# sedaprotocol/bn254

Measured on AMD Instinct MI355X. Metric: BN254 pairings/sec (batch verify), higher is better.
Workload: dtype u32

## Files before the change

### bn254_amd/_native.py

```python
import ctypes
import os
import subprocess

_PKG = os.path.dirname(os.path.abspath(__file__))
_CSRC = os.path.join(_PKG, "csrc")
LIB_PATH = os.environ.get("BN254_LIB", os.path.join(_PKG, "libbn254hip.so"))
import glob


def translation_units():
    return sorted(glob.glob(os.path.join(_CSRC, "*.hip")))


def _dependencies():
    return translation_units() + sorted(glob.glob(os.path.join(_CSRC, "*.h"))) + sorted(glob.glob(os.path.join(_CSRC, "*.inc"))) + [
        os.path.join(_CSRC, "gen_constants.py"), os.path.join(_CSRC, "gen_step_asm.py"), os.path.join(os.path.dirname(_PKG), "include", "bn254_hip.h")]

HIPCC_COMPILE_FLAGS = ["-O3", "--offload-arch=gfx950", "-std=c++17", "-fPIC", "-mllvm", "-amdgpu-sched-strategy=max-ilp"]
HIPCC_LINK_FLAGS = ["--offload-arch=gfx950", "-shared", "-fPIC", "-Wl,--no-undefined"]
HIPCC_FLAGS = HIPCC_COMPILE_FLAGS + ["-shared", "-Wl,--no-undefined"]
_OBJ = os.path.join(_PKG, "build")


def _stale():
    if not os.path.exists(LIB_PATH):
        return True
    t = os.path.getmtime(LIB_PATH)
    return any(os.path.getmtime(p) > t for p in _dependencies())


def build(force=False, verbose=False, jobs=None):
    const_h = os.path.join(_CSRC, "bn254_constants.h")
    gen = os.path.join(_CSRC, "gen_constants.py")
    if not os.path.exists(const_h) or os.path.getmtime(const_h) < os.path.getmtime(gen):
        subprocess.check_call(["python3", gen], stdout=None if verbose else subprocess.DEVNULL)
    asm_h, asm_gen = os.path.join(_CSRC, "bn254_csqr_asm.h"), os.path.join(_CSRC, "gen_step_asm.py")
    if not os.path.exists(asm_h) or os.path.getmtime(asm_h) < os.path.getmtime(asm_gen):
        subprocess.check_call(["python3", asm_gen, "selftest"], stdout=None if verbose else subprocess.DEVNULL)
        with open(asm_h, "w") as f:
            subprocess.check_call(["python3", asm_gen, "header"], stdout=f)
    mul_h = os.path.join(_CSRC, "bn254_mul_asm.h")
    if not os.path.exists(mul_h) or os.path.getmtime(mul_h) < os.path.getmtime(asm_gen):
        subprocess.check_call(["python3", asm_gen, "selftest_mul"], stdout=None if verbose else subprocess.DEVNULL)
        with open(mul_h, "w") as f:
            subprocess.check_call(["python3", asm_gen, "header_mul"], stdout=f)
    if force or _stale():
        import time
        from concurrent.futures import ThreadPoolExecutor
        hipcc = os.environ.get("HIPCC", "hipcc")
        os.makedirs(_OBJ, exist_ok=True)
        units = translation_units()
        objs = [os.path.join(_OBJ, os.path.basename(u)[:-4] + ".o") for u in units]
        t0 = time.time()

        def compile_one(pair):
            cmd = [hipcc] + HIPCC_COMPILE_FLAGS + ["-c", "-o", pair[1], pair[0]]
            if verbose:
                print(" ".join(cmd), flush=True)
            subprocess.check_call(cmd)
        with ThreadPoolExecutor(jobs or min(8, os.cpu_count() or 1)) as ex:
            list(ex.map(compile_one, zip(units, objs)))
        cmd = [hipcc] + HIPCC_LINK_FLAGS + ["-o", LIB_PATH] + objs
        if verbose:
            print(" ".join(cmd), flush=True)
        subprocess.check_call(cmd)
        if verbose:
            print("libbn254hip.so: %d translation units compiled and linked in %.1f s" % (len(units), time.time() - t0), flush=True)
    return LIB_PATH


_lib = None


def load():
    global _lib
    if _lib is not None:
        return _lib
    if not os.path.exists(LIB_PATH):
        raise RuntimeError("libbn254hip.so is not built (run `python -c 'import __graft_entry__ as g; g.build()'`); "
                           "bn254_amd has no CPU fallback")
    L = ctypes.CDLL(LIB_PATH)
    vp, sz, u32, i32 = ctypes.c_void_p, ctypes.c_size_t, ctypes.c_uint32, ctypes.c_int
    L.bn254_version.restype = ctypes.c_char_p
    L.bn254_ctx_create.argtypes = [i32, ctypes.POINTER(vp)]
    L.bn254_ctx_destroy.argtypes = [vp]
    L.bn254_ctx_destroy.restype = None
    L.bn254_ctx_reserve.argtypes = [vp, sz]
    L.bn254_ctx_reserve_host.argtypes = [vp, sz, sz]
    L.bn254_ctx_synchronize.argtypes = [vp]
    L.bn254_ctx_set_profiling.argtypes = [vp, i32]
    L.bn254_ctx_expect_msgs_len.argtypes = [vp, ctypes.c_uint64]
    L.bn254_ctx_last_kernel_ms.argtypes = [vp, ctypes.POINTER(ctypes.c_float)]
    L.bn254_ctx_set_option.argtypes = [vp, i32, i32]
    L.bn254_debug_route_table.argtypes = [vp, ctypes.POINTER(ctypes.c_uint64), ctypes.POINTER(i32), ctypes.POINTER(i32), i32]
    L.bn254_debug_key_dedup_last.argtypes = [vp, ctypes.POINTER(ctypes.c_uint32)]
    L.bn254_debug_agg_rand_last.argtypes = [vp, ctypes.POINTER(ctypes.c_uint64)]
    L.bn254_debug_agg_rand_sums.argtypes = [vp, ctypes.POINTER(ctypes.c_uint64), sz, sz, vp, vp, vp, vp, vp, vp]
    L.bn254_ctx_last_clocks.argtypes = [vp, ctypes.POINTER(ctypes.c_double)]
    L.bn254_batch_verify.argtypes = [vp, vp, vp, vp, vp, sz, u32, vp]
    L.bn254_batch_verify_device.argtypes = [vp, vp, vp, vp, vp, sz, u32, vp, vp]
    L.bn254_ctx_register_keys.argtypes = [vp, vp, sz, u32, vp]
    L.bn254_batch_verify_keyed.argtypes = [vp, vp, vp, vp, vp, sz, u32, vp]
    L.bn254_batch_verify_keyed_device.argtypes = [vp, vp, vp, vp, vp, sz, u32, vp, vp]
    L.bn254_batch_verify_keyed_bitmap.argtypes = [vp, vp, vp, vp, vp, sz, sz, u32, vp]
    L.bn254_batch_verify_keyed_bitmap_device.argtypes = [vp, vp, vp, vp, vp, sz, sz, u32, vp, vp]
    L.bn254_batch_verify_keyed_randomized.argtypes = [vp, vp, vp, vp, vp, sz, u32, vp, vp]
    L.bn254_batch_verify_keyed_randomized_device.argtypes = [vp, vp, vp, vp, vp, sz, u32, vp, vp, vp]
    L.bn254_batch_verify_compressed.argtypes = [vp, vp, vp, vp, vp, sz, vp]
    L.bn254_batch_verify_compressed_device.argtypes = [vp, vp, vp, vp, vp, sz, vp, vp]
    L.bn254_batch_verify_randomized.argtypes = [vp, vp, vp, vp, vp, sz, u32, vp, vp, vp]
    L.bn254_batch_verify_randomized_device.argtypes = [vp, vp, vp, vp, vp, sz, u32, vp, vp, vp, vp]
    L.bn254_batch_hash_to_g1.argtypes = [vp, vp, vp, sz, vp, vp, vp]
    L.bn254_batch_hash_to_g1_device.argtypes = [vp, vp, vp, sz, vp, vp, vp, vp]
    L.bn254_batch_pairing_check.argtypes = [vp, vp, vp, sz, sz, u32, vp]
    L.bn254_batch_pairing.argtypes = [vp, vp, vp, sz, sz, u32, vp, vp]
    L.bn254_batch_pairing_device.argtypes = [vp, vp, vp, sz, sz, u32, vp, vp, vp]
    L.bn254_batch_check_public_keys.argtypes = [vp, vp, vp, sz, u32, vp]
    L.bn254_batch_g1_add.argtypes = [vp, vp, vp, sz, vp, vp]
    L.bn254_batch_g2_add.argtypes = [vp, vp, vp, sz, vp, vp]
    L.bn254_batch_g1_mul.argtypes = [vp, vp, vp, sz, i32, vp, vp]
    L.bn254_batch_g2_mul.argtypes = [vp, vp, vp, sz, i32, vp, vp]
    L.bn254_batch_g1_mul_device.argtypes = [vp, vp, vp, sz, i32, vp, vp, vp]
    L.bn254_batch_g2_mul_device.argtypes = [vp, vp, vp, sz, i32, vp, vp, vp]
    L.bn254_batch_sign.argtypes = [vp, vp, vp, vp, sz, vp, vp]
    L.bn254_batch_sign_device.argtypes = [vp, vp, vp, vp, sz, vp, vp, vp]
    L.bn254_batch_g1_sum.argtypes = [vp, vp, vp, sz, vp, vp]
    L.bn254_batch_g2_sum.argtypes = [vp, vp, vp, sz, vp, vp]
    L.bn254_batch_aggregate_verify.argtypes = [vp, vp, vp, sz, vp, sz, vp, vp, vp, vp, sz, u32, vp]
    L.bn254_batch_aggregate_verify_device.argtypes = [vp, vp, vp, sz, vp, sz, vp, vp, vp, vp, sz, u32, vp, vp]
    L.bn254_ctx_register_pools.argtypes = [vp, vp, vp, sz, vp, sz, vp, u32, sz]
    L.bn254_ctx_register_pools_device.argtypes = [vp, vp, vp, sz, vp, sz, vp, u32, sz, vp]
    L.bn254_batch_aggregate_verify_registered.argtypes = [vp, vp, vp, vp, sz, vp]
    L.bn254_batch_aggregate_verify_registered_device.argtypes = [vp, vp, vp, vp, sz, vp, vp]
    L.bn254_batch_aggregate_verify_distinct.argtypes = [vp, vp, vp, vp, sz, vp, vp, sz, u32, vp]
    L.bn254_batch_aggregate_verify_distinct_device.argtypes = [vp, vp, vp, vp, sz, vp, vp, sz, u32, vp, vp]
    L.bn254_batch_aggregate_verify_distinct_keyed.argtypes = [vp, vp, vp, vp, sz, vp, vp, sz, u32, vp]
    L.bn254_batch_aggregate_verify_distinct_keyed_device.argtypes = [vp, vp, vp, vp, sz, vp, vp, sz, u32, vp, vp]
    L.bn254_batch_aggregate_verify_distinct_keyed_randomized.argtypes = [vp, vp, vp, vp, sz, vp, vp, sz, u32, vp, vp]
    L.bn254_batch_aggregate_verify_distinct_keyed_randomized_device.argtypes = [vp, vp, vp, vp, sz, vp, vp, sz, u32, vp, vp, vp]
    L.bn254_batch_g1_decompress.argtypes = [vp, vp, sz, vp, vp]
    L.bn254_batch_g2_decompress.argtypes = [vp, vp, sz, vp, vp]
    L.bn254_debug_fp_op.argtypes = [vp, i32, vp, vp, sz, vp, vp]
    L.bn254_debug_fp12_op.argtypes = [vp, i32, vp, vp, sz, vp]
    L.bn254_debug_final_exp_limbs.argtypes = [vp, i32, vp, sz, vp, vp]
    L.bn254_debug_miller_loop.argtypes = [vp, vp, vp, sz, vp]
    L.bn254_debug_hash_candidate.argtypes = [vp, vp, sz, vp, vp]
    L.bn254_probe_issue_rate.argtypes = [vp, i32, i32, ctypes.POINTER(ctypes.c_double), ctypes.POINTER(i32)]
    L.bn254_probe_leaf_floor.argtypes = [vp, sz, i32, ctypes.POINTER(ctypes.c_float)]
    L.bn254_probe_fe_program.argtypes = [vp, sz, vp, sz, ctypes.POINTER(ctypes.c_float)]
    pp = ctypes.POINTER(vp)
    L.bn254_mgpu_create.argtypes = [ctypes.POINTER(i32), i32, ctypes.POINTER(vp)]
    L.bn254_mgpu_destroy.argtypes = [vp]
    L.bn254_mgpu_destroy.restype = None
    L.bn254_mgpu_device_count.argtypes = [vp]
    L.bn254_mgpu_ctx.argtypes = [vp, i32]
    L.bn254_mgpu_ctx.restype = vp
    L.bn254_mgpu_shard_len.argtypes = [vp, sz]
    L.bn254_mgpu_shard_len.restype = sz
    L.bn254_mgpu_gathered_len.argtypes = [vp, sz]
    L.bn254_mgpu_gathered_len.restype = sz
    L.bn254_mgpu_shard_range.argtypes = [vp, sz, i32, ctypes.POINTER(sz), ctypes.POINTER(sz)]
    L.bn254_mgpu_reserve.argtypes = [vp, sz, i32]
    L.bn254_mgpu_synchronize.argtypes = [vp]
    L.bn254_mgpu_set_option.argtypes = [vp, i32, i32]
    L.bn254_mgpu_last_timing.argtypes = [vp, ctypes.POINTER(ctypes.c_float), ctypes.POINTER(ctypes.c_float)]
    L.bn254_mgpu_last_error.argtypes = [vp]
    L.bn254_mgpu_last_error.restype = ctypes.c_char_p
    L.bn254_mgpu_batch_verify.argtypes = [vp, vp, vp, vp, vp, sz, u32, vp]
    L.bn254_mgpu_batch_verify_device.argtypes = [vp, pp, pp, pp, pp, sz, u32, pp, pp]
    L.bn254_mgpu_batch_pairing.argtypes = [vp, vp, vp, sz, sz, u32, vp, vp, ctypes.POINTER(ctypes.c_uint64)]
    L.bn254_mgpu_batch_pairing_device.argtypes = [vp, pp, pp, sz, sz, u32, pp, pp, pp, pp]
    L.bn254_mgpu_batch_hash_to_g1.argtypes = [vp, vp, vp, sz, vp, vp, vp]
    L.bn254_mgpu_batch_verify_compressed.argtypes = [vp, vp, vp, vp, vp, sz, vp]
    L.bn254_mgpu_register_keys.argtypes = [vp, vp, sz, u32, vp]
    L.bn254_mgpu_batch_verify_keyed.argtypes = [vp, vp, vp, vp, vp, sz, u32, vp]
    L.bn254_mgpu_batch_aggregate_verify.argtypes = [vp, vp, vp, sz, vp, sz, vp, vp, vp, vp, sz, u32, vp]
    _lib = L
    return L


EXPORTED_SYMBOLS = [
    "bn254_version", "bn254_ctx_create", "bn254_ctx_destroy", "bn254_ctx_reserve", "bn254_ctx_reserve_host", "bn254_ctx_synchronize",
    "bn254_batch_verify", "bn254_batch_verify_device", "bn254_batch_verify_randomized", "bn254_batch_verify_randomized_device", "bn254_batch_verify_compressed", "bn254_batch_verify_compressed_device", "bn254_batch_hash_to_g1", "bn254_batch_hash_to_g1_device",
    "bn254_batch_pairing_check", "bn254_batch_pairing", "bn254_batch_pairing_device", "bn254_batch_check_public_keys",
    "bn254_batch_g1_add", "bn254_batch_g2_add", "bn254_batch_g1_mul", "bn254_batch_g2_mul", "bn254_batch_g1_mul_device",
    "bn254_batch_g2_mul_device", "bn254_batch_sign", "bn254_batch_sign_device", "bn254_batch_g1_sum", "bn254_batch_g2_sum",
    "bn254_batch_aggregate_verify", "bn254_batch_aggregate_verify_device", "bn254_ctx_register_pools", "bn254_ctx_register_pools_device",
    "bn254_batch_aggregate_verify_registered", "bn254_batch_aggregate_verify_registered_device", "bn254_batch_aggregate_verify_distinct", "bn254_batch_aggregate_verify_distinct_device", "bn254_batch_aggregate_verify_distinct_keyed", "bn254_batch_aggregate_verify_distinct_keyed_device", "bn254_batch_aggregate_verify_distinct_keyed_randomized", "bn254_batch_aggregate_verify_distinct_keyed_randomized_device", "bn254_batch_g1_decompress", "bn254_batch_g2_decompress", "bn254_debug_fp_op", "bn254_debug_fp12_op", "bn254_debug_final_exp_limbs", "bn254_debug_miller_loop", "bn254_debug_hash_candidate", "bn254_debug_route_table", "bn254_debug_key_dedup_last", "bn254_debug_agg_rand_last", "bn254_debug_agg_rand_sums", "bn254_probe_issue_rate", "bn254_probe_leaf_floor", "bn254_probe_fe_program", "bn254_ctx_set_profiling", "bn254_ctx_last_kernel_ms", "bn254_ctx_set_option", "bn254_ctx_last_clocks", "bn254_ctx_expect_msgs_len", "bn254_ctx_register_keys", "bn254_batch_verify_keyed", "bn254_batch_verify_keyed_device", "bn254_batch_verify_keyed_randomized", "bn254_batch_verify_keyed_randomized_device",
    "bn254_batch_verify_keyed_bitmap", "bn254_batch_verify_keyed_bitmap_device",
    "bn254_mgpu_create", "bn254_mgpu_destroy", "bn254_mgpu_device_count", "bn254_mgpu_ctx", "bn254_mgpu_shard_len", "bn254_mgpu_shard_range",
    "bn254_mgpu_gathered_len", "bn254_mgpu_reserve", "bn254_mgpu_synchronize", "bn254_mgpu_set_option", "bn254_mgpu_last_timing",
    "bn254_mgpu_last_error", "bn254_mgpu_batch_verify", "bn254_mgpu_batch_verify_device", "bn254_mgpu_batch_pairing",
    "bn254_mgpu_batch_pairing_device", "bn254_mgpu_batch_hash_to_g1", "bn254_mgpu_batch_verify_compressed", "bn254_mgpu_register_keys",
    "bn254_mgpu_batch_verify_keyed", "bn254_mgpu_batch_aggregate_verify",
]
```

### bn254_amd/csrc/bn254_devhooks.hip

```cpp
#include <hip/hip_runtime.h>

#include <cstdio>
#include <cstdlib>
#include <cstring>
#include <new>

#include "../../include/bn254_hip.h"
#include "bn254_hash.h"
#include "bn254_io.h"
#include "bn254_pairing.h"

using namespace bn254;

#include "bn254_ws.h"
#include "bn254_lane.h"
#include "bn254_host.h"

KERNEL_SMALL void k_debug_fp_op(int op, const uint8_t* a, const uint8_t* b, size_t n, uint8_t* out, uint8_t* status) {
  size_t i = (size_t)blockIdx.x * BN_WAVE + threadIdx.x;
  if (i >= n) return;
  uint32_t any = 0;
  Fp x, y, r;
  bool ok = fp_from_be(x, a + 32 * i, any);
  if (b) ok = fp_from_be(y, b + 32 * i, any) && ok; else y = fp_zero();
  uint8_t st = ok ? ST_OK : ST_NOT_MEMBER;
  switch (op) {
    case 0: r = fp_mul(x, y); break;
    case 1: r = fp_add(x, y); break;
    case 2: r = fp_sub(x, y); break;
    case 3: r = fp_inv(x); break;
    case 4: r = fp_sqr(x); break;
    default: if (!fp_sqrt(r, x) && st == ST_OK) st = ST_NOT_MEMBER; break;
  }
  fp_to_be(out + 32 * i, r);
  status[i] = st;
}
KERNEL_SMALL void k_debug_hash_candidate(const uint8_t* h, size_t n, uint8_t* out, uint8_t* status) {
  size_t i = (size_t)blockIdx.x * BN_WAVE + threadIdx.x;
  if (i >= n) return;
  U256 x;
  const uint32_t* w = (const uint32_t*)(h + 32 * i);
#pragma unroll
  for (int k = 0; k < 8; ++k) x.w[7 - k] = __builtin_bswap32(w[k]);
  bool cand = hash_reduce_candidate(x);
  bool filt = false, ok = false;
  G1Affine p;
  g1_set_generator(p);
  if (cand) {
    Fp xm, rhs;
    hash_curve_rhs(xm, rhs, x);
    filt = u256_is_square_mod_q(fp_to_u256(rhs));
    ok = hash_point_from_candidate(p, x);
  }
  if (!ok) p.inf = true;
  encode_g1(out + 64 * i, p);
  status[i] = (uint8_t)((ok ? 0 : 1) | (filt != ok ? 0x80 : 0));
}
__device__ __forceinline__ void decode_fp12(Fp12& f, const uint8_t* b) {
  uint32_t any = 0;
  Fp2* c[6] = {&f.c0.c0, &f.c0.c1, &f.c0.c2, &f.c1.c0, &f.c1.c1, &f.c1.c2};
  for (int k = 0; k < 6; ++k) { fp_from_be(c[k]->c0, b + 64 * k, any); fp_from_be(c[k]->c1, b + 64 * k + 32, any); }
}
KERNEL void k_debug_fp12_op(int op, const uint8_t* a, const uint8_t* b, size_t n, uint8_t* out) {
  size_t i = (size_t)blockIdx.x * BN_WAVE + threadIdx.x;
  if (i >= n) return;
  Fp12 x, y, r;
  decode_fp12(x, a + 384 * i);
  if (b) decode_fp12(y, b + 384 * i); else fp12_set_one(y);
  switch (op) {
    case 0: fp12_mul(r, x, y); break;
    case 1: fp12_sqr(r, x); break;
    case 2: fp12_inv(r, x); break;
    case 3: fp12_conj(r, x); break;
    case 4: fp12_frob(r, x, 1); break;
    case 5: fp12_frob(r, x, 2); break;
    case 6: fp12_frob(r, x, 3); break;
    case 7: fp12_cyclotomic_sqr(r, x); break;
    default: { Fp12 acc; final_exponentiation(r, x, acc); } break;
  }
  encode_fp12(out + 384 * i, r);
}

KERNEL_SMALL void k_debug_load_f(const int32_t* limbs, size_t n, Ws ws) {
  size_t i = (size_t)blockIdx.x * BN_WAVE + threadIdx.x;
  if (i >= n) return;
  for (int e = 0; e < 12; ++e) {
    Fp x;
#pragma unroll
    for (int k = 0; k < BN_LIMBS; ++k) x.v[k] = limbs[(i * 12 + e) * BN_LIMBS + k];
    ws_store_fp(ws, PL_F0 + e, i, x);
  }
  ws_byte(ws, BY_ST_DECODE, i) = ST_OK;
  ws_byte(ws, BY_ST_HASH, i) = ST_OK;
}
KERNEL_SMALL void k_debug_read_p1(Ws ws, size_t base, size_t n, uint8_t* out) {
  size_t i = (size_t)blockIdx.x * BN_WAVE + threadIdx.x;
  if (i >= n) return;
  G1Affine p;
  ws_load_g1(ws, PL_P1X, BY_P1_INF, base + i, p);
  encode_g1(out + 64 * i, p);
}

#define PROBE_ITERS 4096
#define PROBE_CHAINS 16
template <int OP>
__global__ void __launch_bounds__(256) k_issue_probe(uint32_t* out, uint32_t seed, unsigned long long* clk) {
  unsigned long long clk0 = 0, wall0 = 0;
  if (clk && threadIdx.x == 0) { clk0 = clock64(); wall0 = wall_clock64(); }
  uint32_t a = seed + threadIdx.x * 2654435761u, b = seed ^ (threadIdx.x * 40503u + 977u);
  uint64_t acc[PROBE_CHAINS];
#pragma unroll
  for (int j = 0; j < PROBE_CHAINS; ++j) acc[j] = a + j;
  for (int i = 0; i < PROBE_ITERS; ++i) {
#pragma unroll
    for (int j = 0; j < PROBE_CHAINS; ++j) {
      if (OP == 0) {
        asm volatile("v_mad_u64_u32 %0, vcc, %1, %2, %0" : "+v"(acc[j]) : "v"(a), "v"(b) : "vcc");
      } else if (OP == 1) {
        uint32_t lo = (uint32_t)acc[j];
        asm volatile("v_add_u32 %0, %0, %1" : "+v"(lo) : "v"(a));
        acc[j] = lo;
      } else {
        uint32_t lo = (uint32_t)acc[j];
        asm volatile("v_mul_lo_u32 %0, %0, %1" : "+v"(lo) : "v"(b));
        acc[j] = lo;
      }
    }
  }
  uint64_t sum = 0;
#pragma unroll
  for (int j = 0; j < PROBE_CHAINS; ++j) sum += acc[j];
  out[(size_t)blockIdx.x * 256 + threadIdx.x] = (uint32_t)sum ^ (uint32_t)(sum >> 32);
  if (clk && threadIdx.x == 0 && blockIdx.x < BN_CLK_MAX_WG) {
    unsigned long long* p = clk + ((size_t)2 * BN_CLK_MAX_WG + blockIdx.x) * 2;
    p[0] += clock64() - clk0; p[1] += wall_clock64() - wall0;
  }
}


extern "C" {

int bn254_debug_key_dedup_last(bn254_ctx* c, uint32_t out[5]) {
  if (!c || !out) return BN254_E_BAD_ARGUMENT;
  for (int i = 0; i < 5; ++i) out[i] = 0;
  if (!c->kd_last_run || !c->kd_ctl) return 0;
  HIP_TRY(hipSetDevice(c->device));
  HIP_TRY(hipDeviceSynchronize());
  HIP_TRY(hipMemcpy(out + 1, c->kd_ctl, KD_CTL_WORDS * sizeof(uint32_t), hipMemcpyDeviceToHost));
  out[0] = 1;
  return 0;
}
int bn254_debug_agg_rand_last(bn254_ctx* c, uint64_t out[6]) {
  if (!c || !out) return BN254_E_BAD_ARGUMENT;
  for (int i = 0; i < 6; ++i) out[i] = 0;
  if (!c->aggr_last_ran || !c->aggr_stats) return 0;
  HIP_TRY(hipSetDevice(c->device));
  HIP_TRY(hipDeviceSynchronize());
  uint32_t st[5];
  HIP_TRY(hipMemcpy(st, c->aggr_stats, sizeof st, hipMemcpyDeviceToHost));
  out[0] = 1;
  for (int i = 0; i < 5; ++i) out[i + 1] = st[i];
  return 0;
}
int bn254_debug_agg_rand_sums(bn254_ctx* c, uint64_t dims[2], size_t group_cap, size_t pair_cap, uint32_t* nagg, uint8_t* verdict, uint8_t* s_g,
                              uint64_t* first_pair, uint32_t* pair_key, uint8_t* pair_point) {
  if (!c || !dims) return BN254_E_BAD_ARGUMENT;
  dims[0] = dims[1] = 0;
  if (!c->aggr_last_ran || !c->aggr_buf) return 0;
  HIP_TRY(hipSetDevice(c->device));
  HIP_TRY(hipDeviceSynchronize());
  const size_t ng = c->aggr_last.ng, tbase = c->aggr_last.tbase;
  uint64_t end = 0;
  HIP_TRY(hipMemcpy(&end, c->aggr_last.ghi + (ng - 1), sizeof end, hipMemcpyDeviceToHost));
  const size_t n_tp = (size_t)(end - tbase);
  dims[0] = ng;
  dims[1] = n_tp;
  if (group_cap < ng || pair_cap < n_tp) return 0;
  if (!nagg || !verdict || !s_g || !first_pair || (n_tp && (!pair_key || !pair_point))) return BN254_E_BAD_ARGUMENT;
  HIP_TRY(hipMemcpy(nagg, c->aggr_last.nagg, ng * sizeof(uint32_t), hipMemcpyDeviceToHost));
  HIP_TRY(hipMemcpy(verdict, c->aggr_last.gst, ng, hipMemcpyDeviceToHost));
  HIP_TRY(hipMemcpy(first_pair, c->aggr_last.glo, ng * sizeof(uint64_t), hipMemcpyDeviceToHost));
  for (size_t g = 0; g < ng; ++g) first_pair[g] -= tbase;
  first_pair[ng] = n_tp;
  if (n_tp) HIP_TRY(hipMemcpy(pair_key, c->aggr_last.bkey + tbase, n_tp * sizeof(uint32_t), hipMemcpyDeviceToHost));
  int rc;
  if ((rc = stage_reserve(c, 0, 64 * (ng > n_tp ? ng : n_tp)))) return rc;
  k_debug_read_p1<<<grid_for(ng), BN_WAVE, 0, c->stream>>>(c->ws, c->aggr_last.cbase, ng, c->stage[0]);
  HIP_TRY(hipGetLastError());
  HIP_TRY(hipDeviceSynchronize());
  HIP_TRY(hipMemcpy(s_g, c->stage[0], 64 * ng, hipMemcpyDeviceToHost));
  if (n_tp) {
    k_debug_read_p1<<<grid_for(n_tp), BN_WAVE, 0, c->stream>>>(c->ws, tbase, n_tp, c->stage[0]);
    HIP_TRY(hipGetLastError());
    HIP_TRY(hipDeviceSynchronize());
    HIP_TRY(hipMemcpy(pair_point, c->stage[0], 64 * n_tp, hipMemcpyDeviceToHost));
  }
  return 0;
}
int bn254_debug_route_table(bn254_ctx* c, uint64_t* max_n, int* miller, int* fe, int cap) {
  if (!c || !max_n || !miller || !fe || cap < 5) return BN254_E_BAD_ARGUMENT;
  size_t m[5];
  BnRoute r[5];
  const int rows = bn_route_table(route_limits(c), m, r, 5);
  for (int i = 0; i < rows; ++i) { max_n[i] = m[i] == (size_t)-1 ? UINT64_MAX : (uint64_t)m[i]; miller[i] = r[i].miller; fe[i] = r[i].fe; }
  return rows;
}

int bn254_probe_issue_rate(bn254_ctx* c, int op, int waves_per_simd, double* wave_inst_per_s, int* n_simd) {
  if (!c || !wave_inst_per_s || op < 0 || op > 2 || waves_per_simd < 1 || waves_per_simd > 8) return BN254_E_BAD_ARGUMENT;
  HIP_TRY(hipSetDevice(c->device));
  hipDeviceProp_t prop;
  HIP_TRY(hipGetDeviceProperties(&prop, c->device));
  const int n_cu = prop.multiProcessorCount, blocks = n_cu * waves_per_simd;
  int rc;
  if ((rc = stage_reserve(c, 0, sizeof(uint32_t) * 256 * (size_t)blocks))) return rc;
  uint32_t* out = (uint32_t*)c->stage[0];
  ScopedEvents ev;
  HIP_TRY(ev.create());
  hipEvent_t e0 = ev.e0, e1 = ev.e1;
  float best = 0;
  for (int rep = 0; rep < 3; ++rep) {
    HIP_TRY(hipEventRecord(e0, c->stream));
    if (op == 0) k_issue_probe<0><<<blocks, 256, 0, c->stream>>>(out, 12345u, c->ws.clk);
    else if (op == 1) k_issue_probe<1><<<blocks, 256, 0, c->stream>>>(out, 12345u, c->ws.clk);
    else k_issue_probe<2><<<blocks, 256, 0, c->stream>>>(out, 12345u, c->ws.clk);
    HIP_TRY(hipEventRecord(e1, c->stream));
    HIP_TRY(hipEventSynchronize(e1));
    float ms = 0;
    HIP_TRY(hipEventElapsedTime(&ms, e0, e1));
    if (rep > 0 && (best == 0 || ms < best)) best = ms;
  }
  *wave_inst_per_s = (double)PROBE_ITERS * PROBE_CHAINS * 4.0 * blocks / (best * 1e-3);
  if (n_simd) *n_simd = n_cu * 4;
  return 0;
}

int bn254_probe_leaf_floor(bn254_ctx* c, size_t n, int mode, float* ms) {
  if (!c || !ms || n == 0 || n > c->ws.stride || mode < 0 || mode > 7) return BN254_E_BAD_ARGUMENT;
  HIP_TRY(hipSetDevice(c->device));
  ScopedEvents ev;
  HIP_TRY(ev.create());
  hipEvent_t e0 = ev.e0, e1 = ev.e1;
  float best = 0;
  int rc = 0;
  for (int rep = 0; rep < 4 && rc == 0; ++rep) {
    HIP_TRY(hipEventRecord(e0, c->stream));
    rc = bn254_pair_leaf_floor(n, c->ws, c->stream, mode);
    HIP_TRY(hipEventRecord(e1, c->stream));
    HIP_TRY(hipEventSynchronize(e1));
    float t = 0;
    HIP_TRY(hipEventElapsedTime(&t, e0, e1));
    if (rep > 0 && (best == 0 || t < best)) best = t;
  }
  *ms = best;
  return rc;
}

int bn254_probe_fe_program(bn254_ctx* c, size_t n, const uint8_t* prog, size_t n_steps, float* ms) {
  if (!c || !ms || !prog || n == 0 || n > c->ws.stride || n_steps == 0 || n_steps > 4096) return BN254_E_BAD_ARGUMENT;
  for (size_t k = 0; k < n_steps; ++k) {
    const uint8_t op = prog[2 * k], arg = prog[2 * k + 1];
    if (op == 0 || op > 7) return BN254_E_BAD_ARGUMENT;
    if ((op == 1 || op == 2 || op == 4) && arg >= (BN_FE_EXACT_SLOTS > BN_FE_CHECK_SLOTS ? BN_FE_EXACT_SLOTS : BN_FE_CHECK_SLOTS)) return BN254_E_BAD_ARGUMENT;
    if (op == 6 && (arg < 1 || arg > 3)) return BN254_E_BAD_ARGUMENT;
  }
  HIP_TRY(hipSetDevice(c->device));
  int rc;
  if ((rc = stage_reserve(c, 7, 2 * n_steps + 2))) return rc;
  static const uint8_t fe_end[2] = {0, 0};
  HIP_TRY(hipMemcpy(c->stage[7], prog, 2 * n_steps, hipMemcpyHostToDevice));
  HIP_TRY(hipMemcpy(c->stage[7] + 2 * n_steps, fe_end, 2, hipMemcpyHostToDevice));
  ScopedEvents ev;
  HIP_TRY(ev.create());
  hipEvent_t e0 = ev.e0, e1 = ev.e1;
  float best = 0;
  for (int rep = 0; rep < 4 && rc == 0; ++rep) {
    HIP_TRY(hipEventRecord(e0, c->stream));
    rc = bn254_pair_fe_program(n, c->ws, c->stage[7], c->stream);
    HIP_TRY(hipEventRecord(e1, c->stream));
    HIP_TRY(hipEventSynchronize(e1));
    float t = 0;
    HIP_TRY(hipEventElapsedTime(&t, e0, e1));
    if (rep > 0 && (best == 0 || t < best)) best = t;
  }
  *ms = best;
  return rc;
}

int bn254_debug_fp_op(bn254_ctx* c, int op, const uint8_t* a, const uint8_t* b, size_t n, uint8_t* out, uint8_t* status) {
  if (!c || (n && (!a || !out || !status))) return BN254_E_BAD_ARGUMENT;
  if (n == 0) return 0;
  HIP_TRY(hipSetDevice(c->device));
  HostStaging st(c);
  const uint8_t* d_a = st.in(0, a, n * 32);
  const uint8_t* d_b = b ? st.in(1, b, n * 32) : nullptr;
  uint8_t *d_out = st.out(2, n * 32, out), *d_status = st.out(3, n, status);
  if (!st.ok()) return st.rc;
  k_debug_fp_op<<<grid_for(n), BN_WAVE, 0, c->stream>>>(op, d_a, d_b, n, d_out, d_status);
  HIP_TRY(hipGetLastError());
  return st.finish();
}
int bn254_debug_hash_candidate(bn254_ctx* c, const uint8_t* h, size_t n, uint8_t* out, uint8_t* status) {
  if (!c || (n && (!h || !out || !status))) return BN254_E_BAD_ARGUMENT;
  if (n == 0) return 0;
  HIP_TRY(hipSetDevice(c->device));
  HostStaging st(c);
  const uint8_t* d_h = st.in(0, h, n * 32);
  uint8_t *d_out = st.out(2, n * 64, out), *d_status = st.out(3, n, status);
  if (!st.ok()) return st.rc;
  k_debug_hash_candidate<<<grid_for(n), BN_WAVE, 0, c->stream>>>(d_h, n, d_out, d_status);
  HIP_TRY(hipGetLastError());
  return st.finish();
}
int bn254_debug_final_exp_limbs(bn254_ctx* c, int layout, const int32_t* limbs, size_t n, uint8_t* gt, uint8_t* status) {
  if (!c || layout < 0 || layout > 6 || (n && (!limbs || !status)) || (gt && layout > 1)) return BN254_E_BAD_ARGUMENT;
  if (n == 0) return 0;
  if ((layout == 3 && !c->fits_trio) || ((layout == 4 || layout == 6) && !bn254_nonet_fits_device())) return BN254_E_BAD_ARGUMENT;
  HIP_TRY(hipSetDevice(c->device));
  int rc;
  if ((rc = ws_reserve(c, n))) return rc;
  HostStaging st(c);
  const uint8_t* d_limbs = st.in(0, limbs, n * 12 * BN_LIMBS * sizeof(int32_t));
  uint8_t *d_gt = st.out(1, n * 384, gt), *d_status = st.out(2, n, status);
  if (!st.ok()) return st.rc;
  hipStream_t s = c->stream;
  k_debug_load_f<<<grid_for(n), BN_WAVE, 0, s>>>((const int32_t*)d_limbs, n, c->ws);
  switch (layout) {
    case 0: rc = launch_final_exp_lane(c, s, n, 1, 1, 1, 0, d_gt, d_status, 0, 0, nullptr, nullptr); break;
    case 1: rc = bn254_pair_final_exp_product(n, 1, c->ws, d_gt, d_status, 0, s); break;
    case 2: rc = bn254_pair_final_exp(n, c->ws, 0, d_status, nullptr, nullptr, s); break;
    case 3: rc = bn254_trio_final_exp(n, c->ws, 0, d_status, s); break;
    case 4: rc = bn254_nonet_final_exp(n, c->ws, 0, d_status, s); break;
    case 6: rc = bn254_nonet_final_exp(n, c->ws, 0, d_status, s, 1); break;
    default: rc = launch_final_exp_lane(c, s, n, 1, 1, 1, 0, nullptr, d_status, 0, 0, nullptr, nullptr); break;
  }
  if (rc) return rc;
  HIP_TRY(hipGetLastError());
  return st.finish();
}
int bn254_debug_fp12_op(bn254_ctx* c, int op, const uint8_t* a, const uint8_t* b, size_t n, uint8_t* out) {
  if (!c || (n && (!a || !out))) return BN254_E_BAD_ARGUMENT;
  if (n == 0) return 0;
  HIP_TRY(hipSetDevice(c->device));
  HostStaging st(c);
  const uint8_t* d_a = st.in(0, a, n * 384);
  const uint8_t* d_b = b ? st.in(1, b, n * 384) : nullptr;
  uint8_t* d_out = st.out(2, n * 384, out);
  if (!st.ok()) return st.rc;
  k_debug_fp12_op<<<grid_for(n), BN_WAVE, 0, c->stream>>>(op, d_a, d_b, n, d_out);
  HIP_TRY(hipGetLastError());
  return st.finish();
}


}
```

### bn254_amd/csrc/bn254_hip.hip

```cpp
#include <hip/hip_runtime.h>
#include <thread>

#include <cstdio>
#include <cstdlib>
#include <cstring>
#include <new>

#include "../../include/bn254_hip.h"
#include "bn254_hash.h"
#include "bn254_io.h"
#include "bn254_pairing.h"

using namespace bn254;

#include "bn254_ws.h"
#include "bn254_lane.h"
#include "bn254_host.h"

KERNEL_SMALL void k_decode_g1(const uint8_t* pts, size_t n, uint32_t flags, Ws ws, int px, int inf_plane, int accumulate) {
  size_t i = (size_t)blockIdx.x * BN_WAVE + threadIdx.x;
  if (i >= n) return;
  G1Affine p;
  uint8_t st = decode_g1(p, pts + 64 * i, flags);
  if (st != ST_OK) g1_set_generator(p);
  ws_store_g1(ws, px, inf_plane, i, p);
  uint8_t prev = accumulate ? ws_byte(ws, BY_ST_DECODE, i) : (uint8_t)ST_OK;
  ws_byte(ws, BY_ST_DECODE, i) = prev != ST_OK ? prev : st;
}
KERNEL void k_decode_g2(const uint8_t* pts, size_t n, uint32_t flags, Ws ws, int accumulate) {
  size_t i = (size_t)blockIdx.x * BN_WAVE + threadIdx.x;
  if (i >= n) return;
  G2Affine q;
  uint8_t st = decode_g2(q, pts + 128 * i, flags);
  if (st != ST_OK) g2_set_generator(q);
  if (flags & FLAG_G2_SUBGROUP_CHECK) {
    bool in = g2_in_subgroup(q);
    if (st == ST_OK && !in) { st = ST_INVALID_GROUP_POINT; g2_set_generator(q); }
  }
  ws_store_g2(ws, i, q);
  uint8_t prev = accumulate ? ws_byte(ws, BY_ST_DECODE, i) : (uint8_t)ST_OK;
  ws_byte(ws, BY_ST_DECODE, i) = prev != ST_OK ? prev : st;
}

__device__ __forceinline__ bool msg_span(const uint64_t* off, size_t i, uint64_t msgs_len, uint64_t& lo, uint64_t& len) {
  lo = off[i];
  const uint64_t hi = off[i + 1];
  const bool ok = lo <= hi && hi <= msgs_len;
  len = ok ? hi - lo : 0;
  if (!ok) lo = 0;
  return ok;
}
KERNEL_SMALL void k_hash_init(size_t n, Ws ws) {
  size_t i = (size_t)blockIdx.x * BN_WAVE + threadIdx.x;
  if (i < n) { ws.h_best[i] = HASH_NONE; ws.h_next[i] = 0; }
  if (i <= HASH_MAX_ROUNDS) ws.h_cnt[i] = (i == 0) ? (uint32_t)n : 0u;
}
KERNEL_SMALL void k_hash_round(const uint8_t* msgs, const uint64_t* off, uint64_t msgs_len, Ws ws, int round, uint32_t width, uint32_t max_ctr) {
  const uint32_t n_act = ws.h_cnt[round];
  if (n_act == 0) return;
  const uint32_t* list = round == 0 ? nullptr : ws.h_list + (size_t)(round & 1) * ws.stride;
  const size_t total = (size_t)n_act * width;
  for (size_t w = (size_t)blockIdx.x * BN_WAVE + threadIdx.x; w < total; w += (size_t)gridDim.x * BN_WAVE) {
    uint32_t slot = (uint32_t)(w % n_act), j = (uint32_t)(w / n_act);
    uint32_t i = list ? list[slot] : slot;
    uint32_t ctr = (uint32_t)ws.h_next[i] + j;
    if (ctr >= max_ctr) continue;
    uint64_t lo, len;
    msg_span(off, i, msgs_len, lo, len);
    const uint8_t* msg = msgs + lo;
    HashState hs;
    hash_state_init(hs, msg, len);
    if (hash_try_filter(hs, msg, len, ctr)) atomicMin(&ws.h_best[i], ctr);
  }
}
KERNEL_SMALL void k_hash_resolve(Ws ws, int round, uint32_t width, uint32_t max_ctr) {
  const uint32_t n_act = ws.h_cnt[round];
  if (n_act == 0) return;
  const uint32_t* list = round == 0 ? nullptr : ws.h_list + (size_t)(round & 1) * ws.stride;
  uint32_t* list_out = ws.h_list + (size_t)((round + 1) & 1) * ws.stride;
  const size_t span = (size_t)gridDim.x * BN_WAVE;
  for (size_t base = (size_t)blockIdx.x * BN_WAVE; base < n_act; base += span) {
    const size_t slot = base + threadIdx.x;
    bool survivor = false;
    uint32_t i = 0;
    if (slot < n_act) {
      i = list ? list[slot] : (uint32_t)slot;
      if (ws.h_best[i] == HASH_NONE) {
        const uint32_t next = (uint32_t)ws.h_next[i] + width;
        if (next < max_ctr) { ws.h_next[i] = (uint8_t)next; survivor = true; }
      }
    }
    const uint64_t votes = __ballot(survivor);
    if (votes == 0) continue;
    uint32_t first = 0;
    if (threadIdx.x == 0) first = atomicAdd(&ws.h_cnt[round + 1], (uint32_t)__popcll(votes));
    first = __shfl(first, 0, BN_WAVE);
    if (survivor) list_out[first + (uint32_t)__popcll(votes & ((1ull << threadIdx.x) - 1ull))] = i;
  }
}
#define HASH_RESOLVE_WG 1024
#define HASH_RESOLVE_TILES_MIN ((size_t)1 << 20)
__global__ void __launch_bounds__(HASH_RESOLVE_WG) k_hash_resolve_tiles(Ws ws, int round, uint32_t width, uint32_t max_ctr) {
  const uint32_t n_act = ws.h_cnt[round];
  if (n_act == 0) return;
  const uint32_t* list = round == 0 ? nullptr : ws.h_list + (size_t)(round & 1) * ws.stride;
  uint32_t* list_out = ws.h_list + (size_t)((round + 1) & 1) * ws.stride;
  __shared__ uint32_t wave_cnt[HASH_RESOLVE_WG / BN_WAVE];
  __shared__ uint32_t tile_base;
  const unsigned wave = threadIdx.x / BN_WAVE, lane = threadIdx.x % BN_WAVE;
  const size_t span = (size_t)gridDim.x * HASH_RESOLVE_WG;
  for (size_t base = (size_t)blockIdx.x * HASH_RESOLVE_WG; base < n_act; base += span) {
    const size_t slot = base + threadIdx.x;
    bool survivor = false;
    uint32_t i = 0;
    if (slot < n_act) {
      i = list ? list[slot] : (uint32_t)slot;
      if (ws.h_best[i] == HASH_NONE) {
        const uint32_t next = (uint32_t)ws.h_next[i] + width;
        if (next < max_ctr) { ws.h_next[i] = (uint8_t)next; survivor = true; }
      }
    }
    const uint64_t votes = __ballot(survivor);
    if (lane == 0) wave_cnt[wave] = (uint32_t)__popcll(votes);
    __syncthreads();
    if (threadIdx.x == 0) {
      uint32_t total = 0;
      for (unsigned w = 0; w < HASH_RESOLVE_WG / BN_WAVE; ++w) { const uint32_t c = wave_cnt[w]; wave_cnt[w] = total; total += c; }
      tile_base = total ? atomicAdd(&ws.h_cnt[round + 1], total) : 0u;
    }
    __syncthreads();
    if (survivor) list_out[tile_base + wave_cnt[wave] + (uint32_t)__popcll(votes & ((1ull << lane) - 1ull))] = i;
    __syncthreads();
  }
}
KERNEL_SMALL void k_hash_direct(const uint8_t* msgs, const uint64_t* off, uint64_t msgs_len, size_t n, Ws ws, uint32_t width, uint32_t max_ctr, int px,
                                int inf_plane, uint8_t* tries_out) {
  const size_t w = (size_t)blockIdx.x * BN_WAVE + threadIdx.x;
  const size_t i = w / width;
  const uint32_t ctr = (uint32_t)(w % width);
  bool ok = false;
  G1Affine p;
  g1_set_generator(p);
  bool span_ok = true;
  if (i < n && ctr < max_ctr) {
    uint64_t lo, len;
    span_ok = msg_span(off, i, msgs_len, lo, len);
    const uint8_t* msg = msgs + lo;
    HashState hs;
    hash_state_init(hs, msg, len);
    ok = hash_try(p, hs, msg, len, ctr);
  }
  const uint64_t pass = __ballot(ok);
  if (i >= n) return;
  if (!span_ok) {
    if (ctr == 0) {
      g1_set_generator(p);
      ws_store_g1(ws, px, inf_plane, i, p);
      ws_byte(ws, BY_ST_HASH, i) = (uint8_t)ST_INVALID_LENGTH;
      if (tries_out) tries_out[i] = 0;
      ws.h_best[i] = HASH_DONE;
    }
    return;
  }
  const uint32_t group = (uint32_t)(pass >> (threadIdx.x & ~(width - 1u))) & (uint32_t)((1ull << width) - 1u);
  if (group != 0) {
    if (ctr == (uint32_t)__builtin_ctz(group)) {
      ws_store_g1(ws, px, inf_plane, i, p);
      ws_byte(ws, BY_ST_HASH, i) = (uint8_t)ST_OK;
      if (tries_out) tries_out[i] = (uint8_t)(ctr + 1);
      ws.h_best[i] = HASH_DONE;
    }
  } else if (ctr == 0) {
    ws.h_best[i] = HASH_NONE;
    ws.h_next[i] = (uint8_t)width;
    if (width < max_ctr) {
      const uint32_t pos = atomicAdd(&ws.h_cnt[1], 1u);
      (ws.h_list + ws.stride)[pos] = (uint32_t)i;
    }
  }
}
KERNEL_SMALL void k_hash_finish(const uint8_t* msgs, const uint64_t* off, uint64_t msgs_len, size_t n, Ws ws, uint32_t max_ctr, int px, int inf_plane,
                                uint8_t* tries_out) {
  size_t i = (size_t)blockIdx.x * BN_WAVE + threadIdx.x;
  if (i >= n) return;
  const uint32_t best = ws.h_best[i];
  if (best == HASH_DONE) return;
  uint64_t lo, len;
  const bool span_ok = msg_span(off, i, msgs_len, lo, len);
  const uint8_t* msg = msgs + lo;
  HashState hs;
  hash_state_init(hs, msg, len);
  G1Affine p;
  bool ok = span_ok && best != HASH_NONE && hash_try(p, hs, msg, len, best);
  if (!ok) g1_set_generator(p);
  ws_store_g1(ws, px, inf_plane, i, p);
  ws_byte(ws, BY_ST_HASH, i) = ok ? (uint8_t)ST_OK : !span_ok ? (uint8_t)ST_INVALID_LENGTH : (uint8_t)ST_HASH_TO_POINT;
  if (tries_out) tries_out[i] = ok ? (uint8_t)(best + 1) : !span_ok ? (uint8_t)0 : (uint8_t)max_ctr;
}

KERNEL void k_miller_verify(size_t n, Ws ws, const uint32_t* map, const uint32_t* count) {
  size_t i = (size_t)blockIdx.x * BN_WAVE + threadIdx.x;
  if (i >= n) return;
  if (map) { if (i >= *count) return; i = map[i]; }
  G1Affine sig, h;
  G2Affine pk;
  ws_load_g1(ws, PL_P1X, BY_P1_INF, i, sig);
  ws_load_g1(ws, PL_P2X, BY_P2_INF, i, h);
  ws_load_g2(ws, i, pk);
  __shared__ Fp12Slot lds_f[BN_WAVE];
  Fp12& f = lds_f[threadIdx.x].v;
  miller_loop<true, true>(f, h, pk, sig);
  ws_store_f12(ws, i, f);
}
__device__ __noinline__ void miller_role_a(size_t i, Ws ws) {
  G1Affine h, unused_g1;
  G2Affine pk;
  ws_load_g1(ws, PL_P2X, BY_P2_INF, i, h);
  ws_load_g2(ws, i, pk);
  g1_set_generator(unused_g1);
  Fp12 f;
  miller_loop<true, false>(f, h, pk, unused_g1);
  ws_store_f12(ws, i, f);
}
__device__ __noinline__ void miller_role_b(size_t i, size_t f_stride, Ws ws) {
  G1Affine sig, unused_g1;
  G2Affine unused_g2;
  ws_load_g1(ws, PL_P1X, BY_P1_INF, i, sig);
  g1_set_generator(unused_g1);
  g2_set_generator(unused_g2);
  Fp12 f;
  miller_loop<false, true>(f, unused_g1, unused_g2, sig);
  ws_store_f12(ws, f_stride + i, f);
  ws_byte(ws, BY_ST_DECODE, f_stride + i) = ST_OK;
}
KERNEL void k_miller_verify_split(size_t n, size_t f_stride, unsigned nblk, Ws ws) {
  bool role_b = blockIdx.x >= nblk;
  size_t i = (size_t)(blockIdx.x - (role_b ? nblk : 0u)) * BN_WAVE + threadIdx.x;
  if (i >= n) return;
  if (!role_b) miller_role_a(i, ws); else miller_role_b(i, f_stride, ws);
}
KERNEL void k_miller_var(size_t n, Ws ws) {
  size_t i = (size_t)blockIdx.x * BN_WAVE + threadIdx.x;
  if (i >= n) return;
  G1Affine p;
  G2Affine q;
  ws_load_g1(ws, PL_P1X, BY_P1_INF, i, p);
  ws_load_g2(ws, i, q);
  Fp12 f;
  miller_loop<true, false>(f, p, q, p);
  ws_store_f12(ws, i, f);
}
KERNEL void k_miller_cpk(size_t n, Ws ws) {
  size_t i = (size_t)blockIdx.x * BN_WAVE + threadIdx.x;
  if (i >= n) return;
  G1Affine pk1, g;
  G2Affine pk2;
  ws_load_g1(ws, PL_P1X, BY_P1_INF, i, pk1);
  ws_load_g2(ws, i, pk2);
  g1_set_generator(g);
  Fp12 f;
  miller_loop<true, true>(f, g, pk2, pk1);
  ws_store_f12(ws, i, f);
}

KERNEL void k_final_exp(size_t n, size_t k, size_t item_stride, size_t pair_stride, Ws ws, int use_hash, uint8_t* gt_out, uint8_t* status_out,
                        int raw_only, size_t base, const uint32_t* map, const uint32_t* count) {
  size_t i = (size_t)blockIdx.x * BN_WAVE + threadIdx.x;
  if (i >= n) return;
  if (map) { if (i >= *count) return; i = map[i]; }
  Fp12 f, g;
  ws_load_f12(ws, base + i * item_stride, f);
  uint8_t st = ws_byte(ws, BY_ST_DECODE, base + i * item_stride);
  for (size_t j = 1; j < k; ++j) {
    size_t idx = base + i * item_stride + j * pair_stride;
    ws_load_f12(ws, idx, g);
    fp12_mul(f, f, g);
    uint8_t sj = ws_byte(ws, BY_ST_DECODE, idx);
    if (st == ST_OK) st = sj;
  }
  if (st == ST_OK && use_hash) st = ws_byte(ws, BY_ST_HASH, i);
  __shared__ Fp12Slot lds_acc[BN_WAVE];
  if (!raw_only) {
    if (gt_out) final_exponentiation(f, f, lds_acc[threadIdx.x].v);
    else final_exponentiation_check(f, f, lds_acc[threadIdx.x].v);
  }
  if (gt_out) encode_fp12(gt_out + 384 * i, f);
  if (status_out) status_out[i] = st != ST_OK ? st : (fp12_is_one(f) ? (uint8_t)ST_OK : (uint8_t)ST_VERIFICATION_FAILED);
}


KERNEL_SMALL void k_decompress_g1_ws(const uint8_t* in, size_t n, Ws ws) {
  size_t i = (size_t)blockIdx.x * BN_WAVE + threadIdx.x;
  if (i >= n) return;
  G1Affine p;
  uint8_t st = decompress_g1(p, in + 33 * i);
  if (st != ST_OK) g1_set_generator(p);
  ws_store_g1(ws, PL_P1X, BY_P1_INF, i, p);
  ws_byte(ws, BY_ST_DECODE, i) = st;
}
KERNEL void k_decompress_g2_ws(const uint8_t* in, size_t n, Ws ws) {
  size_t i = (size_t)blockIdx.x * BN_WAVE + threadIdx.x;
  if (i >= n) return;
  G2Affine q;
  uint8_t st = decompress_g2(q, in + 65 * i);
  if (st != ST_OK) g2_set_generator(q);
  bool in_sub = g2_in_subgroup(q);
  if (st == ST_OK && !in_sub) { st = ST_NOT_MEMBER; g2_set_generator(q); }
  ws_store_g2(ws, i, q);
  uint8_t prev = ws_byte(ws, BY_ST_DECODE, i);
  ws_byte(ws, BY_ST_DECODE, i) = prev != ST_OK ? prev : st;
}
KERNEL_SMALL void k_encode_g1(size_t n, Ws ws, int px, int inf_plane, uint8_t* out, uint8_t* status_out) {
  size_t i = (size_t)blockIdx.x * BN_WAVE + threadIdx.x;
  if (i >= n) return;
  G1Affine p;
  ws_load_g1(ws, px, inf_plane, i, p);
  uint8_t st = ws_byte(ws, BY_ST_HASH, i);
  if (st != ST_OK) p.inf = true;
  encode_g1(out + 64 * i, p);
  if (status_out) status_out[i] = st;
}



int ctx_quiesce(bn254_ctx* c) {
  HIP_TRY(hipStreamSynchronize(c->stream));
  HIP_TRY(hipStreamSynchronize(c->copy_stream));
  HIP_TRY(hipStreamSynchronize(c->kd_stream));
  if (c->last_done_armed) {
    c->last_done_armed = false;
    HIP_TRY(hipEventSynchronize(c->last_done));
  }
  return 0;
}
int ws_reserve(bn254_ctx* c, size_t n) {
  if (n <= c->ws.stride) return 0;
  size_t cap = (n + 255) & ~(size_t)255;
  HIP_TRY(hipSetDevice(c->device));
  { int rc_ = ctx_quiesce(c); if (rc_) return rc_; }
  if (c->ws.planes) { HIP_TRY(hipFree(c->ws.planes)); c->ws.planes = nullptr; }
  if (c->ws.bytes) { HIP_TRY(hipFree(c->ws.bytes)); c->ws.bytes = nullptr; }
  if (c->ws.h_best) { HIP_TRY(hipFree(c->ws.h_best)); c->ws.h_best = nullptr; }
  if (c->ws.h_next) { HIP_TRY(hipFree(c->ws.h_next)); c->ws.h_next = nullptr; }
  if (c->ws.h_list) { HIP_TRY(hipFree(c->ws.h_list)); c->ws.h_list = nullptr; }
  c->ws.stride = 0;
  HIP_TRY(hipMalloc((void**)&c->ws.planes, (size_t)N_PLANES * BN_LIMBS * sizeof(int32_t) * cap));
  HIP_TRY(hipMalloc((void**)&c->ws.bytes, (size_t)N_BYTE_PLANES * cap));
  HIP_TRY(hipMalloc((void**)&c->ws.h_best, sizeof(uint32_t) * cap));
  HIP_TRY(hipMalloc((void**)&c->ws.h_next, cap));
  HIP_TRY(hipMalloc((void**)&c->ws.h_list, 2 * sizeof(uint32_t) * cap));
  if (!c->ws.h_cnt) HIP_TRY(hipMalloc((void**)&c->ws.h_cnt, sizeof(uint32_t) * (HASH_MAX_ROUNDS + 1)));
  c->ws.stride = cap;
  return 0;
}
#define WS_BYTES_PER_ITEM ((size_t)N_PLANES * BN_LIMBS * sizeof(int32_t) + N_BYTE_PLANES + sizeof(uint32_t) + 1 + 2 * sizeof(uint32_t))
size_t ws_chunk_for(bn254_ctx* c, size_t n, size_t ws_per_item, bool key_dedup) {
  if (c->max_chunk > 0) return n > (size_t)c->max_chunk ? (size_t)c->max_chunk : 0;
  if (n * ws_per_item <= c->ws.stride && (!key_dedup || (n <= c->kd_items_cap && (size_t)c->kd_max_keys <= c->kd_keys_cap))) return 0;
  const size_t per_item = ws_per_item * WS_BYTES_PER_ITEM + (key_dedup ? KD_BYTES_PER_ITEM : 0);
  const size_t fixed = key_dedup ? (size_t)c->kd_max_keys * KD_BYTES_PER_KEY : 0;
  size_t avail;
  if (c->assume_free_mb > 0) avail = (size_t)c->assume_free_mb << 20;
  else {
    size_t fr = 0, total = 0;
    if (hipSetDevice(c->device) != hipSuccess || hipMemGetInfo(&fr, &total) != hipSuccess) { (void)hipGetLastError(); return 0; }
    avail = fr + c->ws.stride * WS_BYTES_PER_ITEM + c->kd_items_cap * KD_BYTES_PER_ITEM + c->kd_keys_cap * KD_BYTES_PER_KEY;
  }
  const size_t need = ((n + 255) & ~(size_t)255) * per_item + fixed;
  if (need <= avail / 10 * 9) return 0;
  const size_t room = avail / 10 * 8 > fixed ? avail / 10 * 8 - fixed : 0;
  size_t chunk = room / per_item;
  chunk &= ~(size_t)65535;
  if (chunk == 0) chunk = room / per_item & ~(size_t)255;
  if (key_dedup && (chunk == 0 || route_for(c, chunk).miller != BN_ML_LANE_PAIRS)) return ws_chunk_for(c, n, ws_per_item, false);
  return chunk && chunk < n ? chunk : 0;
}
#define KD_NO_ROOM 1
static int kd_reserve(bn254_ctx* c, size_t n, KeyDedup& kd) {
  size_t slots = 1;
  while (slots < 2 * n) slots <<= 1;
  const size_t keys = (size_t)c->kd_max_keys;
  if (n > c->kd_items_cap || keys > c->kd_keys_cap) {
    const size_t items_cap = n > c->kd_items_cap ? ((n + 255) & ~(size_t)255) : c->kd_items_cap;
    const size_t keys_cap = keys > c->kd_keys_cap ? keys : c->kd_keys_cap;
    { int rc_ = ctx_quiesce(c); if (rc_) return rc_; }
    if (c->kd_buf) { HIP_TRY(hipFree(c->kd_buf)); c->kd_buf = nullptr; }
    c->kd_items_cap = c->kd_keys_cap = 0;
    c->kd_ctl = nullptr;
    if (hipMalloc((void**)&c->kd_buf, items_cap * KD_BYTES_PER_ITEM + keys_cap * KD_BYTES_PER_KEY + 256) != hipSuccess) {
      (void)hipGetLastError();
      c->kd_buf = nullptr;
      return KD_NO_ROOM;
    }
    c->kd_items_cap = items_cap;
    c->kd_keys_cap = keys_cap;
  }
  size_t slots_cap = 1;
  while (slots_cap < 2 * c->kd_items_cap) slots_cap <<= 1;
  uint8_t* p = c->kd_buf;
  auto take = [&](size_t bytes) { uint8_t* r = p; p += (bytes + 15) & ~(size_t)15; return r; };
  kd.table = (uint32_t*)take(slots_cap * 4);
  kd.slot_id = (uint32_t*)take(slots_cap * 4);
  kd.slot_of = (uint32_t*)take(c->kd_items_cap * 4);
  kd.key_idx = (uint32_t*)take(c->kd_items_cap * 4);
  kd.lines = (int32_t*)take(c->kd_keys_cap * BN_N_FIXED_LINES * BN_KEY_LINE_WORDS * 4);
  kd.c2 = (int32_t*)take(c->kd_keys_cap * BN_N_FIXED_LINES * 2 * BN_LIMBS * 4);
  kd.rep = (uint32_t*)take(c->kd_keys_cap * 4);
  kd.ctl = (uint32_t*)take(KD_CTL_WORDS * 4);
  c->kd_ctl = kd.ctl;
  kd.st = take(c->kd_keys_cap);
  kd.inf = take(c->kd_keys_cap);
  kd.slot_mask = (uint32_t)(slots - 1);
  kd.hash_mask = c->kd_hash_bits > 0 && c->kd_hash_bits < 32 ? (1u << c->kd_hash_bits) - 1 : 0xFFFFFFFFu;
  kd.max_keys = (uint32_t)keys;
  kd.min_mult = (uint32_t)c->kd_min_mult;
  return 0;
}
int scratch_reserve(bn254_ctx* c, uint8_t** buf, size_t* cap, size_t bytes) {
  if (bytes <= *cap) return 0;
  { int rc_ = ctx_quiesce(c); if (rc_) return rc_; }
  if (*buf) { HIP_TRY(hipFree(*buf)); *buf = nullptr; *cap = 0; }
  const size_t grown = (bytes + 4095) & ~(size_t)4095;
  HIP_TRY(hipMalloc((void**)buf, grown));
  *cap = grown;
  return 0;
}
int stage_reserve(bn254_ctx* c, int slot, size_t bytes) {
  if (bytes <= c->stage_cap[slot]) return 0;
  HIP_TRY(hipSetDevice(c->device));
  return scratch_reserve(c, &c->stage[slot], &c->stage_cap[slot], bytes);
}
uint8_t* HostStaging::out(int slot, size_t bytes, void* host) {
  if (!rc) rc = stage_reserve(c, slot, bytes);
  if (rc) return nullptr;
  if (host) copy_back(host, c->stage[slot], bytes);
  return c->stage[slot];
}
uint8_t* HostStaging::in(int slot, const void* host, size_t bytes) {
  uint8_t* d = out(slot, bytes ? bytes : 1);
  if (d && bytes) check(hipMemcpyAsync(d, host, bytes, hipMemcpyHostToDevice, c->stream));
  return rc ? nullptr : d;
}
void HostStaging::copy_back(void* host, const void* dev, size_t bytes) {
  if (!host || !bytes) return;
  if (n_back == (int)(sizeof back / sizeof back[0])) { check(hipErrorInvalidValue); return; }
  back[n_back++] = {host, dev, bytes};
}
hipError_t HostStaging::drain() {
  finished = true;
  const hipError_t e = hipStreamSynchronize(c->stream);
  const hipError_t e_copy = hipStreamSynchronize(c->copy_stream);
  return e != hipSuccess ? e : e_copy;
}
int HostStaging::finish() {
  for (int i = 0; i < n_back && !rc; ++i) check(hipMemcpyAsync(back[i].host, back[i].dev, back[i].bytes, hipMemcpyDeviceToHost, c->stream));
  const hipError_t e = drain();
  return rc ? rc : -(int)e;
}
int pool_reserve_one(bn254_ctx* c, Pool* p, size_t n_fp, size_t entries) {
  if (entries <= p->stride) return 0;
  HIP_TRY(hipSetDevice(c->device));
  { int rc_ = ctx_quiesce(c); if (rc_) return rc_; }
  if (p->planes) { HIP_TRY(hipFree(p->planes)); p->planes = nullptr; }
  if (p->st) { HIP_TRY(hipFree(p->st)); p->st = nullptr; }
  p->stride = 0;
  const size_t cap = (entries + 255) & ~(size_t)255;
  p->g2 = n_fp == 4 ? 1u : 0u;
  HIP_TRY(hipMalloc((void**)&p->planes, (n_fp / 2) * BN_POOL_HALF_WORDS * sizeof(int32_t) * cap));
  HIP_TRY(hipMalloc((void**)&p->st, cap));
  p->stride = cap;
  return 0;
}
int pool_reserve(bn254_ctx* c, int which, size_t n_fp, size_t entries) {
  Pool& p = c->pool[which];
  if (entries <= p.stride && c->pool_fp[which] == n_fp) return 0;
  HIP_TRY(hipSetDevice(c->device));
  { int rc_ = ctx_quiesce(c); if (rc_) return rc_; }
  if (p.planes) { HIP_TRY(hipFree(p.planes)); p.planes = nullptr; }
  if (p.st) { HIP_TRY(hipFree(p.st)); p.st = nullptr; }
  p.stride = 0;
  size_t cap = (entries + 255) & ~(size_t)255;
  p.g2 = n_fp == 4 ? 1u : 0u;
  HIP_TRY(hipMalloc((void**)&p.planes, (n_fp / 2) * BN_POOL_HALF_WORDS * sizeof(int32_t) * cap));
  HIP_TRY(hipMalloc((void**)&p.st, cap));
  p.stride = cap;
  c->pool_fp[which] = n_fp;
  return 0;
}

int launch_decode_g2(bn254_ctx* c, hipStream_t s, const uint8_t* d_pts, size_t n, uint32_t flags, int accumulate) {
  if (c->pair_lanes && (flags & FLAG_G2_SUBGROUP_CHECK)) {
    if (route_lane_machine_helpers(c, n)) {
      k_decode_g2<<<grid_for(n), BN_WAVE, 0, s>>>(d_pts, n, flags & ~(uint32_t)FLAG_G2_SUBGROUP_CHECK, c->ws, accumulate);
      return bn254_lm_g2_subgroup(n, c->ws, s);
    }
    return bn254_pair_decode_g2(d_pts, n, flags, c->ws, accumulate, s);
  }
  k_decode_g2<<<grid_for(n), BN_WAVE, 0, s>>>(d_pts, n, flags, c->ws, accumulate);
  return 0;
}

int launch_hash_rounds(bn254_ctx* c, hipStream_t s, const uint8_t* d_msgs, const uint64_t* d_off, size_t n, int px, int inf_plane,
                              uint8_t* d_tries, int mark_finish) {
  const uint32_t max_ctr = c->hash_max_tries ? (uint32_t)c->hash_max_tries : 255u;
  const uint64_t msgs_len = c->msgs_len_call;
  k_hash_init<<<grid_for(n > HASH_MAX_ROUNDS + 1 ? n : HASH_MAX_ROUNDS + 1), BN_WAVE, 0, s>>>(n, c->ws);
  if (n <= HASH_DIRECT_MAX_N && c->hash_direct_width > 0) {
    const uint32_t width = (uint32_t)c->hash_direct_width;
    k_hash_direct<<<grid_for(n * width), BN_WAVE, 0, s>>>(d_msgs, d_off, msgs_len, n, c->ws, width, max_ctr, px, inf_plane, d_tries);
    if (max_ctr > width)
      k_hash_round<<<grid_for(64 * (max_ctr - width)), BN_WAVE, 0, s>>>(d_msgs, d_off, msgs_len, c->ws, 1, max_ctr - width, max_ctr);
    if (mark_finish >= 0 && c->profiling) HIP_TRY(hipEventRecord(c->ev[mark_finish], s));
    k_hash_finish<<<grid_for(n), BN_WAVE, 0, s>>>(d_msgs, d_off, msgs_len, n, c->ws, max_ctr, px, inf_plane, d_tries);
    HIP_TRY(hipGetLastError());
    return 0;
  }
  double expect = (double)n;
  uint32_t consumed = 0;
  for (int round = 0; round < HASH_MAX_ROUNDS && consumed < max_ctr; ++round) {
    bool last = round == HASH_MAX_ROUNDS - 1;
    double lanes_per_msg = (double)HASH_TARGET_LANES / (expect < 1.0 ? 1.0 : expect);
    uint32_t width = lanes_per_msg < 2.0 ? 1u : (uint32_t)lanes_per_msg;
    if (width > max_ctr - consumed || last) width = max_ctr - consumed;
    double bound = expect * 1.25 + 256.0;
    if (bound > (double)n) bound = (double)n;
    size_t lanes = (size_t)(bound * width);
    if (lanes > HASH_MAX_GRID_LANES) lanes = HASH_MAX_GRID_LANES;
    k_hash_round<<<grid_for(lanes), BN_WAVE, 0, s>>>(d_msgs, d_off, msgs_len, c->ws, round, width, max_ctr);
    if ((size_t)bound > HASH_RESOLVE_TILES_MIN) {
      size_t tiles = ((size_t)bound + HASH_RESOLVE_WG - 1) / HASH_RESOLVE_WG;
      if (tiles > 16384) tiles = 16384;
      k_hash_resolve_tiles<<<(unsigned)tiles, HASH_RESOLVE_WG, 0, s>>>(c->ws, round, width, max_ctr);
    } else {
      k_hash_resolve<<<grid_for((size_t)bound), BN_WAVE, 0, s>>>(c->ws, round, width, max_ctr);
    }
    consumed += width;
    double pf = 1.0;
    for (uint32_t t = 0; t < width && pf > 1e-12; ++t) pf *= 0.5274;
    expect *= pf;
  }
  if (mark_finish >= 0 && c->profiling) HIP_TRY(hipEventRecord(c->ev[mark_finish], s));
  k_hash_finish<<<grid_for(n), BN_WAVE, 0, s>>>(d_msgs, d_off, msgs_len, n, c->ws, max_ctr, px, inf_plane, d_tries);
  HIP_TRY(hipGetLastError());
  return 0;
}

int launch_decode_g1(bn254_ctx* c, hipStream_t s, const uint8_t* d_pts, size_t n, uint32_t flags, int px, int inf_plane, int accumulate) {
  k_decode_g1<<<grid_for(n), BN_WAVE, 0, s>>>(d_pts, n, flags, c->ws, px, inf_plane, accumulate);
  return 0;
}
int launch_miller_var_lane(bn254_ctx* c, hipStream_t s, size_t n) {
  k_miller_var<<<grid_for(n), BN_WAVE, 0, s>>>(n, c->ws);
  return 0;
}
int launch_miller_verify_lane(bn254_ctx* c, hipStream_t s, size_t n, const uint32_t* map, const uint32_t* count) {
  k_miller_verify<<<grid_for(n), BN_WAVE, 0, s>>>(n, c->ws, map, count);
  return 0;
}
int launch_final_exp_lane(bn254_ctx* c, hipStream_t s, size_t n, size_t k, size_t item_stride, size_t pair_stride, int use_hash, uint8_t* gt_out,
                          uint8_t* status_out, int raw_only, size_t base, const uint32_t* map, const uint32_t* count) {
  k_final_exp<<<grid_for(n), BN_WAVE, 0, s>>>(n, k, item_stride, pair_stride, c->ws, use_hash, gt_out, status_out, raw_only, base, map, count);
  return 0;
}
int launch_encode_g1(bn254_ctx* c, hipStream_t s, size_t n, int px, int inf_plane, uint8_t* out, uint8_t* status_out) {
  k_encode_g1<<<grid_for(n), BN_WAVE, 0, s>>>(n, c->ws, px, inf_plane, out, status_out);
  return 0;
}

extern "C" {

const char* bn254_version(void) { return "bn254-mi355x 0.7 (gfx950; 9x29-bit balanced Montgomery limbs; verify on lane pairs, batches <= 16384 on lane octets with wave roles; bn254_mgpu_*: all the GPUs of a node behind one handle)"; }

int bn254_ctx_create(int hip_device, bn254_ctx** out) {
  if (!out) return BN254_E_BAD_ARGUMENT;
  int count = 0;
  hipError_t e = hipGetDeviceCount(&count);
  if (e != hipSuccess || count <= 0) return BN254_E_NO_DEVICE;
  if (hip_device < 0 || hip_device >= count) return BN254_E_BAD_ARGUMENT;
  HIP_TRY(hipSetDevice(hip_device));
  bn254_ctx* c = new (std::nothrow) bn254_ctx();
  if (!c) return BN254_E_BAD_ARGUMENT;
  memset(c, 0, sizeof *c);
  c->pair_lanes = 1;
  c->rand_min_batch = RAND_MIN_BATCH_DEFAULT;
  c->agg_rand_min_pairs = AGG_RAND_MIN_PAIRS_DEFAULT;
  c->agg_rand_group_pairs = AGG_RAND_GROUP_PAIRS_DEFAULT;
  c->trio_max_batch = TRIO_MAX_BATCH_DEFAULT;
  c->hash_direct_width = HASH_DIRECT_WIDTH_DEFAULT;
  c->trio_wave_roles = TRIO_WAVE_ROLES_DEFAULT;
  c->agg_subset_min_tuples = AGG_SUBSET_MIN_TUPLES_DEFAULT;
  c->agg_sort_by_msg = 1;
  c->agg_wide_min_tuples = AGG_WIDE_MIN_TUPLES_DEFAULT;
  c->pinned_staging = PINNED_STAGING_DEFAULT;
  c->fits_w8 = bn254_quad_fits_device(1); c->fits_quad = bn254_quad_fits_device(0); c->fits_trio = bn254_trio_fits_device();
  if (c->trio_wave_roles == 2 && !c->fits_w8) c->trio_wave_roles = 1;
  if (c->trio_wave_roles == 1 && !c->fits_quad) c->trio_wave_roles = 0;
  if (!c->fits_trio) c->trio_max_batch = 0;
  c->nonet_max_batch = bn254_nonet_fits_device() ? NONET_MAX_BATCH_DEFAULT : 0;
  c->lm_max_batch = bn254_lm_fits_device() ? LM_MAX_BATCH_DEFAULT : 0;
  c->nonet_wide = 1;
  c->g2_fixed_base = 1;
  c->key_dedup = 1;
  c->kd_max_keys = KEY_DEDUP_MAX_KEYS_DEFAULT;
  c->kd_min_mult = KEY_DEDUP_MIN_MULT_DEFAULT;
  c->bm_table_max_keys = BITMAP_TABLE_MAX_KEYS_DEFAULT;
  c->device = hip_device;
  hipError_t err = hipStreamCreateWithFlags(&c->stream, hipStreamNonBlocking);
  if (err == hipSuccess) err = hipStreamCreateWithFlags(&c->copy_stream, hipStreamNonBlocking);
  if (err == hipSuccess) err = hipEventCreateWithFlags(&c->copy_done, hipEventDisableTiming);
  if (err == hipSuccess) err = hipEventCreateWithFlags(&c->last_done, hipEventDisableTiming);
  if (err == hipSuccess) err = hipStreamCreateWithFlags(&c->kd_stream, hipStreamNonBlocking);
  if (err == hipSuccess) err = hipEventCreateWithFlags(&c->kd_fork, hipEventDisableTiming);
  if (err == hipSuccess) err = hipEventCreateWithFlags(&c->kd_join, hipEventDisableTiming);
  for (int i = 0; i < 5 && err == hipSuccess; ++i) err = hipEventCreate(&c->ev[i]);
  if (err != hipSuccess) {
    if (c->kd_join) (void)hipEventDestroy(c->kd_join);
    if (c->kd_fork) (void)hipEventDestroy(c->kd_fork);
    if (c->kd_stream) (void)hipStreamDestroy(c->kd_stream);
    if (c->last_done) (void)hipEventDestroy(c->last_done);
    for (int i = 0; i < 5; ++i) if (c->ev[i]) (void)hipEventDestroy(c->ev[i]);
    if (c->copy_done) (void)hipEventDestroy(c->copy_done);
    if (c->copy_stream) (void)hipStreamDestroy(c->copy_stream);
    if (c->stream) (void)hipStreamDestroy(c->stream);
    delete c;
    return -(int)err;
  }
  *out = c;
  return 0;
}
void bn254_ctx_destroy(bn254_ctx* c) {
  if (!c) return;
  (void)hipSetDevice(c->device);
  (void)ctx_quiesce(c);
  if (c->ws.planes) (void)hipFree(c->ws.planes);
  if (c->ws.bytes) (void)hipFree(c->ws.bytes);
  if (c->ws.h_best) (void)hipFree(c->ws.h_best);
  if (c->ws.h_next) (void)hipFree(c->ws.h_next);
  if (c->ws.h_list) (void)hipFree(c->ws.h_list);
  if (c->ws.h_cnt) (void)hipFree(c->ws.h_cnt);
  if (c->ws.clk) (void)hipFree(c->ws.clk);
  if (c->pin) (void)hipHostFree(c->pin);
  for (int i = 0; i < 8; ++i) { if (c->pool[i].planes) (void)hipFree(c->pool[i].planes); if (c->pool[i].st) (void)hipFree(c->pool[i].st); }
  if (c->g2_comb.planes) (void)hipFree(c->g2_comb.planes);
  if (c->g2_comb.st) (void)hipFree(c->g2_comb.st);
  if (c->g1_comb.planes) (void)hipFree(c->g1_comb.planes);
  if (c->g1_comb.st) (void)hipFree(c->g1_comb.st);
  for (int i = 0; i < 8; ++i) if (c->stage[i]) (void)hipFree(c->stage[i]);
  if (c->key_lines) (void)hipFree(c->key_lines);
  if (c->key_xy) (void)hipFree(c->key_xy);
  if (c->key_st) (void)hipFree(c->key_st);
  if (c->key_inf) (void)hipFree(c->key_inf);
  if (c->aggd_buf) (void)hipFree(c->aggd_buf);
  if (c->aggr_buf) (void)hipFree(c->aggr_buf);
  if (c->aggr_stats) (void)hipFree(c->aggr_stats);
  if (c->kd_buf) (void)hipFree(c->kd_buf);
  if (c->bm_bad) (void)hipFree(c->bm_bad);
  if (c->bm_tab) (void)hipFree(c->bm_tab);
  for (int i = 0; i < 5; ++i) (void)hipEventDestroy(c->ev[i]);
  (void)hipEventDestroy(c->kd_fork);
  (void)hipEventDestroy(c->kd_join);
  (void)hipStreamDestroy(c->kd_stream);
  (void)hipEventDestroy(c->copy_done);
  (void)hipEventDestroy(c->last_done);
  (void)hipStreamSynchronize(c->copy_stream);
  (void)hipStreamDestroy(c->copy_stream);
  (void)hipStreamDestroy(c->stream);
  delete c;
}
int bn254_ctx_reserve(bn254_ctx* c, size_t n) { return c ? ws_reserve(c, n) : BN254_E_BAD_ARGUMENT; }
int bn254_ctx_reserve_host(bn254_ctx* c, size_t n, size_t msg_bytes) {
  if (!c) return BN254_E_BAD_ARGUMENT;
  int rc = ws_reserve(c, n);
  const size_t need[5] = {msg_bytes ? msg_bytes : 1, (n + 1) * sizeof(uint64_t), n * 64, n * 128, n ? n : 1};
  for (int slot = 0; slot < 5 && !rc; ++slot) rc = stage_reserve(c, slot, need[slot]);
  return rc;
}
int bn254_ctx_synchronize(bn254_ctx* c) {
  if (!c) return BN254_E_BAD_ARGUMENT;
  HIP_TRY(hipStreamSynchronize(c->stream));
  return 0;
}
int bn254_ctx_expect_msgs_len(bn254_ctx* c, uint64_t msgs_len) {
  if (!c) return BN254_E_BAD_ARGUMENT;
  c->msgs_len_next = msgs_len;
  c->msgs_len_declared = 1;
  return 0;
}
int bn254_ctx_set_profiling(bn254_ctx* c, int enabled) {
  if (!c) return BN254_E_BAD_ARGUMENT;
  c->profiling = enabled;
  c->ev_valid = 0;
  return 0;
}
int bn254_ctx_set_option(bn254_ctx* c, int option, int value) {
  if (!c) return BN254_E_BAD_ARGUMENT;
  if (option == BN254_OPT_SPLIT_MILLER) { c->split_miller = value; return 0; }
  if (option == BN254_OPT_PAIR_LANES) { c->pair_lanes = value != 0; return 0; }
  if (option == BN254_OPT_RAND_MIN_BATCH) { if (value < 0) return BN254_E_BAD_ARGUMENT; c->rand_min_batch = value; return 0; }
  if (option == BN254_OPT_RAND_ITEMS_PER_LANE) { if (value < 0 || value > 2) return BN254_E_BAD_ARGUMENT; c->rand_items_per_lane = value; return 0; }
  if (option == BN254_OPT_AGG_SUBSET_MIN_TUPLES) { if (value < 0) return BN254_E_BAD_ARGUMENT; c->agg_subset_min_tuples = value; return 0; }
  if (option == BN254_OPT_TRIO_MAX_BATCH) {
    if (value < 0 || (value > 0 && !c->fits_trio)) return BN254_E_BAD_ARGUMENT;
    c->trio_max_batch = value;
    return 0;
  }
  if (option == BN254_OPT_TRIO_WAVE_ROLES) {
    if (value < 0 || value > 2 || (value == 2 && !c->fits_w8) || (value == 1 && !c->fits_quad)) return BN254_E_BAD_ARGUMENT;
    c->trio_wave_roles = value;
    return 0;
  }
  if (option == BN254_OPT_HASH_DIRECT_WIDTH) {
    if (value < 0 || value > 32 || (value & (value - 1))) return BN254_E_BAD_ARGUMENT;
    c->hash_direct_width = value;
    return 0;
  }
  if (option == BN254_OPT_NONET_MAX_BATCH) {
    HIP_TRY(hipSetDevice(c->device));
    if (value < 0 || (value > 0 && !bn254_nonet_fits_device())) return BN254_E_BAD_ARGUMENT;
    c->nonet_max_batch = value;
    return 0;
  }
  if (option == BN254_OPT_NONET_WIDE) { c->nonet_wide = value != 0; return 0; }
  if (option == BN254_OPT_LM_MAX_BATCH) {
    HIP_TRY(hipSetDevice(c->device));
    if (value < 0 || (value > 0 && !bn254_lm_fits_device())) return BN254_E_BAD_ARGUMENT;
    c->lm_max_batch = value;
    return 0;
  }
  if (option == BN254_OPT_PINNED_STAGING) { if (value < 0 || value > 16) return BN254_E_BAD_ARGUMENT; c->pinned_staging = value; return 0; }
  if (option == BN254_OPT_AGG_SORT_BY_MSG) { c->agg_sort_by_msg = value != 0; return 0; }
  if (option == BN254_OPT_AGG_WIDE_MIN_TUPLES) { if (value < 0) return BN254_E_BAD_ARGUMENT; c->agg_wide_min_tuples = value; return 0; }
  if (option == BN254_OPT_CLOCK_PROBE) {
    HIP_TRY(hipSetDevice(c->device));
    HIP_TRY(hipDeviceSynchronize());
    if (value && !c->ws.clk) {
      HIP_TRY(hipMalloc((void**)&c->ws.clk, sizeof(unsigned long long) * 3 * BN_CLK_MAX_WG * 2));
      HIP_TRY(hipMemset(c->ws.clk, 0, sizeof(unsigned long long) * 3 * BN_CLK_MAX_WG * 2));
    } else if (!value && c->ws.clk) {
      HIP_TRY(hipFree(c->ws.clk));
      c->ws.clk = nullptr;
    }
    return 0;
  }
  if (option == BN254_OPT_HASH_MAX_TRIES) { if (value < 0 || value > 255) return BN254_E_BAD_ARGUMENT; c->hash_max_tries = value; return 0; }
  if (option == BN254_OPT_G2_FIXED_BASE) { c->g2_fixed_base = value != 0; return 0; }
  if (option == BN254_OPT_MAX_CHUNK) { if (value < 0) return BN254_E_BAD_ARGUMENT; c->max_chunk = value; return 0; }
  if (option == BN254_OPT_ASSUME_FREE_MB) { if (value < 0) return BN254_E_BAD_ARGUMENT; c->assume_free_mb = value; return 0; }
  if (option == BN254_OPT_KEY_DEDUP) { if (value < 0 || value > 1) return BN254_E_BAD_ARGUMENT; c->key_dedup = value; return 0; }
  if (option == BN254_OPT_KEY_DEDUP_MAX_KEYS) { if (value < 0 || value > KEY_DEDUP_MAX_KEYS_LIMIT) return BN254_E_BAD_ARGUMENT; c->kd_max_keys = value; return 0; }
  if (option == BN254_OPT_KEY_DEDUP_MIN_MULT) { if (value < 1) return BN254_E_BAD_ARGUMENT; c->kd_min_mult = value; return 0; }
  if (option == BN254_OPT_KEY_DEDUP_FORCE_GENERIC) { c->kd_force_generic = value != 0; return 0; }
  if (option == BN254_OPT_KEY_DEDUP_HASH_BITS) { if (value < 0 || value > 32) return BN254_E_BAD_ARGUMENT; c->kd_hash_bits = value; return 0; }
  if (option == BN254_OPT_AGGD_KEYED_ROUTE) { if (value < 0 || value > 3) return BN254_E_BAD_ARGUMENT; c->aggd_keyed_route = value; return 0; }
  if (option == BN254_OPT_AGG_RAND_MIN_PAIRS) { if (value < 0) return BN254_E_BAD_ARGUMENT; c->agg_rand_min_pairs = value; return 0; }
  if (option == BN254_OPT_AGG_RAND_GROUP_PAIRS) { if (value < 1) return BN254_E_BAD_ARGUMENT; c->agg_rand_group_pairs = value; return 0; }
  if (option == BN254_OPT_BITMAP_TABLE_MAX_KEYS) { if (value < 0) return BN254_E_BAD_ARGUMENT; c->bm_table_max_keys = value; return 0; }
  if (option == BN254_OPT_BITMAP_ROUTE) { if (value < 0 || value > 2) return BN254_E_BAD_ARGUMENT; c->bm_route = value; return 0; }
  return BN254_E_BAD_ARGUMENT;
}
int bn254_ctx_last_clocks(bn254_ctx* c, double sclk_mhz[3]) {
  if (!c || !sclk_mhz || !c->ws.clk) return BN254_E_BAD_ARGUMENT;
  HIP_TRY(hipSetDevice(c->device));
  int wall_khz = 0;
  HIP_TRY(hipDeviceGetAttribute(&wall_khz, hipDeviceAttributeWallClockRate, c->device));
  const size_t words = (size_t)3 * BN_CLK_MAX_WG * 2;
  unsigned long long* h = (unsigned long long*)malloc(words * sizeof(unsigned long long));
  if (!h) return BN254_E_NO_MEMORY;
  hipError_t e = hipDeviceSynchronize();
  if (e == hipSuccess) e = hipMemcpy(h, c->ws.clk, words * sizeof(unsigned long long), hipMemcpyDeviceToHost);
  if (e == hipSuccess) e = hipMemset(c->ws.clk, 0, words * sizeof(unsigned long long));
  if (e != hipSuccess) { free(h); return -(int)e; }
  for (int k = 0; k < 3; ++k) {
    double cyc = 0, wall = 0;
    for (size_t w = 0; w < BN_CLK_MAX_WG; ++w) {
      const unsigned long long a = h[((size_t)k * BN_CLK_MAX_WG + w) * 2], b = h[((size_t)k * BN_CLK_MAX_WG + w) * 2 + 1];
      if (b) { cyc += (double)a; wall += (double)b; }
    }
    sclk_mhz[k] = wall > 0 ? cyc / wall * (double)wall_khz * 1e-3 : 0.0;
  }
  free(h);
  return 0;
}
int bn254_ctx_last_kernel_ms(bn254_ctx* c, float ms[4]) {
  if (!c || !ms || !c->ev_valid) return BN254_E_BAD_ARGUMENT;
  HIP_TRY(hipEventSynchronize(c->ev[4]));
  for (int i = 0; i < 4; ++i) HIP_TRY(hipEventElapsedTime(&ms[i], c->ev[i], c->ev[i + 1]));
  if (c->ev_hash_first) { float t = ms[0]; ms[0] = ms[1]; ms[1] = t; }
  return 0;
}


}
int launch_final_exp_layout(bn254_ctx* c, hipStream_t s, size_t n, int use_hash, uint8_t* d_status, int fe) {
  switch (fe) {
    case BN_FE_NONET_WIDE: return bn254_nonet_final_exp(n, c->ws, use_hash, d_status, s, 1);
    case BN_FE_NONET: return bn254_nonet_final_exp(n, c->ws, use_hash, d_status, s, 0);
    case BN_FE_OCTET: return bn254_trio_final_exp(n, c->ws, use_hash, d_status, s);
    default: return bn254_pair_final_exp(n, c->ws, use_hash, d_status, nullptr, nullptr, s);
  }
}
int launch_verify_miller_fe(bn254_ctx* c, hipStream_t s, size_t n, int pairs, int use_hash, uint8_t* d_status, bool mark) {
  if (!c->pair_lanes) {
    const unsigned g = grid_for(n);
    if (pairs == BN_PAIRS_CHECK_PKS) k_miller_cpk<<<g, BN_WAVE, 0, s>>>(n, c->ws);
    else k_miller_verify<<<g, BN_WAVE, 0, s>>>(n, c->ws, nullptr, nullptr);
    if (mark) PROF_MARK(3);
    k_final_exp<<<g, BN_WAVE, 0, s>>>(n, 1, 1, 1, c->ws, use_hash, nullptr, d_status, 0, 0, nullptr, nullptr);
    return 0;
  }
  const BnRoute r = route_for(c, n);
  int rc;
  switch (r.miller) {
    case BN_ML_LANE_MACHINE: rc = bn254_lm_miller_verify(n, c->ws, s, pairs); break;
    case BN_ML_WAVE_ROLES:
      rc = c->trio_wave_roles == 2 ? bn254_w8_miller_verify(n, c->ws, s, pairs)
           : c->trio_wave_roles ? bn254_quad_miller_verify(n, c->ws, s, pairs) : bn254_trio_miller_verify(n, c->ws, s, pairs);
      break;
    default: rc = bn254_pair_miller_verify(n, c->ws, nullptr, nullptr, s, pairs); break;
  }
  if (rc) return rc;
  if (mark) PROF_MARK(3);
  return launch_final_exp_layout(c, s, n, use_hash, d_status, r.fe);
}

extern "C" {
static int verify_tail(bn254_ctx* c, hipStream_t s, size_t n, uint8_t* d_status, bool split, const KeyDedup* kd, int hash_first) {
  int rc;
  if (kd) {
    HIP_TRY(hipStreamWaitEvent(s, c->kd_join, 0));
    const KeyTable kt = {kd->lines, kd->st, kd->inf, kd->max_keys};
    if ((rc = bn254_pair_miller_verify_keyed(n, c->ws, kd->key_idx, kt, s, 0, nullptr, kd->ctl + KD_CTL_KEYED_N))) return rc;
    if ((rc = bn254_pair_miller_verify(n, c->ws, nullptr, kd->ctl + KD_CTL_GENERIC_N, s))) return rc;
    PROF_MARK(3);
    if ((rc = bn254_pair_final_exp(n, c->ws, 1, d_status, nullptr, nullptr, s))) return rc;
  } else if (split) {
    const unsigned g = grid_for(n);
    k_miller_verify_split<<<2 * g, BN_WAVE, 0, s>>>(n, c->ws.stride / 2, g, c->ws);
    PROF_MARK(3);
    k_final_exp<<<g, BN_WAVE, 0, s>>>(n, 2, 1, c->ws.stride / 2, c->ws, 1, nullptr, d_status, 0, 0, nullptr, nullptr);
  } else if ((rc = launch_verify_miller_fe(c, s, n, BN_PAIRS_VERIFY, 1, d_status, true))) return rc;
  PROF_MARK(4);
  if (c->profiling) { c->ev_valid = 1; c->ev_hash_first = hash_first; }
  HIP_TRY(hipGetLastError());
  return 0;
}
static int verify_after_decode(bn254_ctx* c, hipStream_t s, const uint8_t* d_msgs, const uint64_t* d_off, size_t n, uint8_t* d_status, bool split,
                               const KeyDedup* kd = nullptr) {
  PROF_MARK(1);
  if (const int rc = launch_hash_rounds(c, s, d_msgs, d_off, n, PL_P2X, BY_P2_INF, nullptr)) return rc;
  PROF_MARK(2);
  return verify_tail(c, s, n, d_status, split, kd, 0);
}

int bn254_batch_verify_device(bn254_ctx* c, const uint8_t* d_msgs, const uint64_t* d_off, const uint8_t* d_sigs, const uint8_t* d_pks,
                              size_t n, uint32_t flags, uint8_t* d_status, void* stream) {
  MsgsLenScope msgs_len_scope(c);
  if (!c || (n && (!d_msgs || !d_off || !d_sigs || !d_pks || !d_status))) return BN254_E_BAD_ARGUMENT;
  if (n == 0) return 0;
  if (misaligned(d_sigs) || misaligned(d_pks) || ((uintptr_t)d_off & 7u)) return BN254_E_MISALIGNED;
  HIP_TRY(hipSetDevice(c->device));
  bool split = c->split_miller && n <= BN_SPLIT_MAX_N;
  bool key_dedup = c->key_dedup && c->kd_max_keys > 0 && c->pair_lanes && !split && n <= 0xFFFFFFFFu &&
                         route_for(c, n).miller == BN_ML_LANE_PAIRS && route_for(c, n).fe == BN_FE_LANE_PAIRS;
  if (const size_t chunk = ws_chunk_for(c, n, split ? 2 : 1, key_dedup))
    return verify_device_sliced(n, chunk, [&](size_t lo, size_t len) {
      return bn254_batch_verify_device(c, d_msgs, d_off + lo, d_sigs + 64 * lo, d_pks + 128 * lo, len, flags, d_status + lo, stream);
    });
  int rc = ws_reserve(c, split ? 2 * n : n);
  if (rc) return rc;
  KeyDedup kd;
  if (key_dedup) {
    rc = kd_reserve(c, n, kd);
    if (rc == KD_NO_ROOM) key_dedup = false;
    else if (rc) return rc;
    rc = 0;
  }
  c->kd_last_run = key_dedup;
  hipStream_t s = stream ? (hipStream_t)stream : c->stream;
  CallDone call_done(c, s);
  PROF_MARK(0);
  if (key_dedup) {
    HIP_TRY(hipEventRecord(c->kd_fork, s));
    HIP_TRY(hipStreamWaitEvent(c->kd_stream, c->kd_fork, 0));
    if ((rc = bn254_kd_enqueue(d_pks, n, flags, kd, c->kd_force_generic, c->kd_stream))) return rc;
    HIP_TRY(hipEventRecord(c->kd_join, c->kd_stream));
  }
  k_decode_g1<<<grid_for(n), BN_WAVE, 0, s>>>(d_sigs, n, flags, c->ws, PL_P1X, BY_P1_INF, 0);
  if ((rc = launch_decode_g2(c, s, d_pks, n, flags, 1))) return rc;
  return verify_after_decode(c, s, d_msgs, d_off, n, d_status, split, key_dedup ? &kd : nullptr);
}

int bn254_batch_verify_compressed_device(bn254_ctx* c, const uint8_t* d_msgs, const uint64_t* d_off, const uint8_t* d_sigs33,
                                         const uint8_t* d_pks65, size_t n, uint8_t* d_status, void* stream) {
  MsgsLenScope msgs_len_scope(c);
  if (!c || (n && (!d_msgs || !d_off || !d_sigs33 || !d_pks65 || !d_status))) return BN254_E_BAD_ARGUMENT;
  if (n == 0) return 0;
  if ((uintptr_t)d_off & 7u) return BN254_E_MISALIGNED;
  HIP_TRY(hipSetDevice(c->device));
  if (const size_t chunk = ws_chunk_for(c, n))
    return verify_device_sliced(n, chunk, [&](size_t lo, size_t len) {
      return bn254_batch_verify_compressed_device(c, d_msgs, d_off + lo, d_sigs33 + 33 * lo, d_pks65 + 65 * lo, len, d_status + lo, stream);
    });
  int rc = ws_reserve(c, n);
  if (rc) return rc;
  hipStream_t s = stream ? (hipStream_t)stream : c->stream;
  CallDone call_done(c, s);
  PROF_MARK(0);
  k_decompress_g1_ws<<<grid_for(n), BN_WAVE, 0, s>>>(d_sigs33, n, c->ws);
  if (route_lane_machine_helpers(c, n)) {
    if ((rc = bn254_pair_decompress_g2(d_pks65, n, c->ws, s, 1))) return rc;
    if ((rc = bn254_lm_g2_subgroup(n, c->ws, s, ST_NOT_MEMBER))) return rc;
  } else if (c->pair_lanes) { if ((rc = bn254_pair_decompress_g2(d_pks65, n, c->ws, s))) return rc; }
  else k_decompress_g2_ws<<<grid_for(n), BN_WAVE, 0, s>>>(d_pks65, n, c->ws);
  return verify_after_decode(c, s, d_msgs, d_off, n, d_status, false);
}
static int verify_host_sliced(bn254_ctx* c, const uint8_t* msgs, const uint64_t* off, const uint8_t* sigs, const uint8_t* pks, size_t n,
                              uint32_t flags, uint8_t* status, size_t chunk, bool compressed) {
  uint64_t* tmp = (uint64_t*)malloc((chunk + 1) * sizeof(uint64_t));
  if (!tmp) return BN254_E_NO_MEMORY;
  const size_t sig_sz = compressed ? 33 : 64, pk_sz = compressed ? 65 : 128;
  int rc = 0;
  for (size_t lo = 0; lo < n && !rc; lo += chunk) {
    const size_t len = n - lo < chunk ? n - lo : chunk;
    for (size_t i = 0; i <= len; ++i) tmp[i] = off[lo + i] - off[lo];
    const uint8_t* m = msgs ? msgs + off[lo] : nullptr;
    rc = compressed ? bn254_batch_verify_compressed(c, m, tmp, sigs + sig_sz * lo, pks + pk_sz * lo, len, status + lo)
                    : bn254_batch_verify(c, m, tmp, sigs + sig_sz * lo, pks + pk_sz * lo, len, flags, status + lo);
  }
  free(tmp);
  return rc;
}
int bn254_batch_verify_compressed(bn254_ctx* c, const uint8_t* msgs, const uint64_t* off, const uint8_t* sigs33, const uint8_t* pks65, size_t n,
                                  uint8_t* status) {
  MsgsLenScope msgs_len_scope(c);
  if (!c || (n && (!off || !sigs33 || !pks65 || !status))) return BN254_E_BAD_ARGUMENT;
  if (n == 0) return 0;
  HIP_TRY(hipSetDevice(c->device));
  if (!msgs_ok(msgs, off, n)) return BN254_E_BAD_ARGUMENT;
  if (const size_t chunk = ws_chunk_for(c, n)) return verify_host_sliced(c, msgs, off, sigs33, pks65, n, 0, status, chunk, true);
  HostStaging st(c);
  const uint8_t *d_msgs = st.in(0, msgs, (size_t)off[n]), *d_off = st.in(1, off, (n + 1) * sizeof(uint64_t));
  const uint8_t *d_sigs = st.in(2, sigs33, n * 33), *d_pks = st.in(3, pks65, n * 65);
  uint8_t* d_status = st.out(4, n, status);
  if (st.ok()) st.rc = bn254_batch_verify_compressed_device(c, d_msgs, (const uint64_t*)d_off, d_sigs, d_pks, n, d_status, nullptr);
  return st.finish();
}

static int pin_reserve(bn254_ctx* c, size_t bytes) {
  if (bytes <= c->pin_cap) return 0;
  { int rc_ = ctx_quiesce(c); if (rc_) return rc_; }
  if (c->pin) { HIP_TRY(hipHostFree(c->pin)); c->pin = nullptr; c->pin_cap = 0; }
  const size_t cap = (bytes + ((size_t)1 << 20) - 1) & ~(((size_t)1 << 20) - 1);
  HIP_TRY(hipHostMalloc((void**)&c->pin, cap, hipHostMallocDefault));
  c->pin_cap = cap;
  return 0;
}
static int pinned_copy_in(bn254_ctx* c, uint8_t* d_dst, uint8_t* pin, const uint8_t* src, size_t bytes, hipStream_t stream, int threads) {
  if (!bytes) return 0;
  const size_t piece = (size_t)1 << 20;
  if (threads > 16) threads = 16;
  if (threads > 1 && bytes < 4 * piece) threads = 1;
  int rcs[16] = {0};
  auto work = [&](int t, int n_threads) {
    if (t && hipSetDevice(c->device) != hipSuccess) { rcs[t] = -1; return; }
    const size_t share = ((bytes + n_threads - 1) / n_threads + 255) & ~(size_t)255, lo = (size_t)t * share, hi = lo + share < bytes ? lo + share : bytes;
    for (size_t o = lo; o < hi; o += piece) {
      const size_t len = o + piece < hi ? piece : hi - o;
      memcpy(pin + o, src + o, len);
      const hipError_t e = hipMemcpyAsync(d_dst + o, pin + o, len, hipMemcpyHostToDevice, stream);
      if (e != hipSuccess) { rcs[t] = -(int)e; return; }
    }
  };
  std::thread helpers[15];
  int started = 0;
  bool fallback = false;
  try {
    for (int t = 1; t < threads; ++t) { helpers[started] = std::thread(work, t, threads); ++started; }
  } catch (...) {
    fallback = true;
  }
  if (!fallback) work(0, threads);
  for (int t = 0; t < started; ++t) helpers[t].join();
  if (fallback) {
    for (int t = 0; t < 16; ++t) rcs[t] = 0;
    work(0, 1);
  }
  for (int t = 0; t < 16; ++t) if (rcs[t]) return rcs[t];
  return 0;
}
static int verify_host_overlapped(bn254_ctx* c, const uint8_t* msgs, const uint64_t* off, const uint8_t* sigs, const uint8_t* pks, size_t n,
                                  uint32_t flags, uint8_t* status) {
  const size_t msg_bytes = (size_t)off[n];
  int rc;
  if ((rc = ws_reserve(c, n))) return rc;
  HostStaging st(c);
  const size_t need[4] = {msg_bytes ? msg_bytes : 1, (n + 1) * sizeof(uint64_t), n * 64, n * 128};
  for (int slot = 0; slot < 4; ++slot) st.out(slot, need[slot]);
  st.out(4, n, status);
  if (!st.ok()) return st.rc;
  hipStream_t s = c->stream;
  const bool pinned = c->pinned_staging > 0 && n >= PINNED_STAGING_MIN_N;
  auto up = [](size_t x) { return (x + 4095) & ~(size_t)4095; };
  const size_t o_off = up(msg_bytes), o_sig = o_off + up((n + 1) * sizeof(uint64_t)), o_pk = o_sig + up(n * 64), pin_bytes = o_pk + up(n * 128);
  if (pinned && (rc = pin_reserve(c, pin_bytes))) return rc;
  PROF_MARK(0);
  if (pinned) {
    if ((rc = pinned_copy_in(c, c->stage[0], c->pin, msgs, msg_bytes, s, c->pinned_staging))) return rc;
    if ((rc = pinned_copy_in(c, c->stage[1], c->pin + o_off, (const uint8_t*)off, (n + 1) * sizeof(uint64_t), s, 1))) return rc;
  } else {
    if (msg_bytes) HIP_TRY(hipMemcpyAsync(c->stage[0], msgs, msg_bytes, hipMemcpyHostToDevice, s));
    HIP_TRY(hipMemcpyAsync(c->stage[1], off, (n + 1) * sizeof(uint64_t), hipMemcpyHostToDevice, s));
  }
  if ((rc = launch_hash_rounds(c, s, c->stage[0], (const uint64_t*)c->stage[1], n, PL_P2X, BY_P2_INF, nullptr))) return rc;
  if (pinned) {
    if ((rc = pinned_copy_in(c, c->stage[2], c->pin + o_sig, sigs, n * 64, c->copy_stream, c->pinned_staging))) return rc;
    if ((rc = pinned_copy_in(c, c->stage[3], c->pin + o_pk, pks, n * 128, c->copy_stream, c->pinned_staging))) return rc;
  } else {
    HIP_TRY(hipMemcpyAsync(c->stage[2], sigs, n * 64, hipMemcpyHostToDevice, c->copy_stream));
// ... 148 lines not shown
```

### bn254_amd/csrc/bn254_host.h

```cpp
#pragma once
#include <hip/hip_runtime.h>

#include <cstdint>
#include <cstdlib>
#include <cstring>
#include <new>

#include "../../include/bn254_hip.h"

#define BN_HIDDEN __attribute__((visibility("hidden")))

struct AggTables { int valid; size_t n_msgs, n_signers, n_groups, groups4, built_for; int wide2, wide1; };

struct bn254_ctx {
  int device;
  hipStream_t stream;
  Ws ws;
  uint8_t* stage[8];
  size_t stage_cap[8];
  int profiling;
  int split_miller;
  Pool pool[8];
  size_t pool_fp[8];
  int agg_wide_min_tuples;
  int agg_subset_min_tuples;
  int agg_sort_by_msg;
  int pair_lanes;
  int rand_min_batch;
  int rand_items_per_lane;
  int hash_max_tries;
  int trio_wave_roles;
  int hash_direct_width;
  int trio_max_batch;
  int lm_max_batch;
  int nonet_wide;
  int nonet_max_batch;
  hipEvent_t ev[5];
  int ev_valid;
  int ev_hash_first;
  hipStream_t copy_stream;
  uint8_t* pin;
  size_t pin_cap;
  int pinned_staging;
  hipEvent_t copy_done;
  uint64_t msgs_len_next;
  int msgs_len_declared;
  uint64_t msgs_len_call;
  int entry_depth;
  int32_t* key_lines;
  int32_t* key_xy;
  uint8_t* key_st;
  uint8_t* key_inf;
  size_t n_keys, key_cap;
  hipEvent_t last_done;
  bool last_done_armed;
  Pool g2_comb;
  int g2_comb_ready;
  Pool g1_comb;
  int g1_comb_ready;
  int g2_fixed_base;
  AggTables reg_pools;
  int max_chunk;
  int assume_free_mb;
  bool fits_w8, fits_quad, fits_trio;
  uint8_t* aggd_buf;
  size_t aggd_cap;
  int key_dedup;
  int kd_max_keys;
  int kd_min_mult;
  int kd_force_generic;
  int kd_hash_bits;
  hipStream_t kd_stream;
  hipEvent_t kd_fork, kd_join;
  uint8_t* kd_buf;
  size_t kd_items_cap, kd_keys_cap;
  uint32_t* kd_ctl;
  int kd_last_run;
  int aggd_keyed_route;
  int agg_rand_min_pairs;
  int agg_rand_group_pairs;
  uint8_t* aggr_buf;
  size_t aggr_cap;
  uint32_t* aggr_stats;
  int aggr_last_ran;
  struct { size_t ng, cbase, tbase; const uint32_t *nagg, *bkey; const uint64_t *glo, *ghi; const uint8_t* gst; } aggr_last;
  uint8_t* bm_bad;
  size_t bm_bad_cap;
  uint8_t* bm_tab;
  size_t bm_tab_cap;
  bool bm_bad_valid, bm_tab_valid;
  int bm_table_max_keys;
  int bm_route;
};

struct ScopedEvents {
  hipEvent_t e0 = nullptr, e1 = nullptr;
  hipError_t create() {
    hipError_t e = hipEventCreate(&e0);
    return e == hipSuccess ? hipEventCreate(&e1) : e;
  }
  ~ScopedEvents() { if (e0) (void)hipEventDestroy(e0); if (e1) (void)hipEventDestroy(e1); }
  ScopedEvents() = default;
  ScopedEvents(const ScopedEvents&) = delete;
  ScopedEvents& operator=(const ScopedEvents&) = delete;
};
static inline BnRouteLimits route_limits(const bn254_ctx* c) {
  BnRouteLimits L;
  L.small_max = c->pair_lanes && c->trio_max_batch > 0 ? (size_t)c->trio_max_batch : 0;
  L.lm_max = c->lm_max_batch > 0 ? (size_t)c->lm_max_batch : 0;
  L.nonet_max = c->nonet_max_batch > 0 ? (size_t)c->nonet_max_batch : 0;
  L.nonet_wide_max = c->nonet_wide ? (size_t)NONET_WIDE_MAX_BATCH : 0;
  return L;
}
static inline BnRoute route_for(const bn254_ctx* c, size_t n) { return bn_route(route_limits(c), n); }
static inline bool route_lane_machine_helpers(const bn254_ctx* c, size_t n) { return c->pair_lanes && c->lm_max_batch > 0 && n <= (size_t)c->lm_max_batch; }
static inline unsigned grid_for(size_t n) { return (unsigned)((n + BN_WAVE - 1) / BN_WAVE); }

BN_HIDDEN int ctx_quiesce(bn254_ctx* c);
struct CallDone {
  bn254_ctx* c;
  hipStream_t s;
  CallDone(bn254_ctx* ctx, hipStream_t stream) : c(ctx), s(stream) {}
  ~CallDone() {
    if (s == c->stream) return;
    if (hipEventRecord(c->last_done, s) == hipSuccess) c->last_done_armed = true;
    else (void)hipGetLastError();
  }
  CallDone(const CallDone&) = delete;
  CallDone& operator=(const CallDone&) = delete;
};
BN_HIDDEN int ws_reserve(bn254_ctx* c, size_t n);
BN_HIDDEN size_t ws_chunk_for(bn254_ctx* c, size_t n, size_t ws_per_item = 1, bool key_dedup = false);
template <class Slice> static inline int verify_device_sliced(size_t n, size_t chunk, Slice slice) {
  for (size_t lo = 0; lo < n; lo += chunk)
    if (const int rc = slice(lo, n - lo < chunk ? n - lo : chunk)) return rc;
  return 0;
}
BN_HIDDEN int scratch_reserve(bn254_ctx* c, uint8_t** buf, size_t* cap, size_t bytes);
BN_HIDDEN int stage_reserve(bn254_ctx* c, int slot, size_t bytes);
BN_HIDDEN int pool_reserve(bn254_ctx* c, int which, size_t n_fp, size_t entries);
BN_HIDDEN int pool_reserve_one(bn254_ctx* c, Pool* p, size_t n_fp, size_t entries);
static inline bool misaligned(const void* p) { return ((uintptr_t)p & 3u) != 0; }
static inline bool offsets_ok(const uint64_t* off, size_t n) {
  for (size_t i = 0; i < n; ++i) if (off[i] > off[i + 1]) return false;
  return true;
}
static inline bool msgs_ok(const uint8_t* msgs, const uint64_t* off, size_t n) { return offsets_ok(off, n) && (off[n] == 0 || msgs); }
struct MsgsLenScope {
  bn254_ctx* c;
  explicit MsgsLenScope(bn254_ctx* ctx) : c(ctx) {
    if (c && c->entry_depth++ == 0) {
      c->msgs_len_call = c->msgs_len_declared ? c->msgs_len_next : UINT64_MAX;
      c->msgs_len_declared = 0;
    }
  }
  ~MsgsLenScope() { if (c) --c->entry_depth; }
  MsgsLenScope(const MsgsLenScope&) = delete;
  MsgsLenScope& operator=(const MsgsLenScope&) = delete;
};
struct BN_HIDDEN HostStaging {
  bn254_ctx* c;
  int rc = 0;
  explicit HostStaging(bn254_ctx* ctx) : c(ctx) {}
  ~HostStaging() { if (!finished) (void)drain(); }
  bool ok() const { return rc == 0; }
  void check(hipError_t e) { if (!rc && e != hipSuccess) rc = -(int)e; }
  uint8_t* in(int slot, const void* host, size_t bytes);
  uint8_t* out(int slot, size_t bytes, void* host = nullptr);
  void copy_back(void* host, const void* dev, size_t bytes);
  int finish();
  HostStaging(const HostStaging&) = delete;
  HostStaging& operator=(const HostStaging&) = delete;
 private:
  hipError_t drain();
  struct Back { void* host; const void* dev; size_t bytes; } back[4];
  int n_back = 0;
  bool finished = false;
};


#define PROF_MARK(idx) do { if (c->profiling) HIP_TRY(hipEventRecord(c->ev[idx], s)); } while (0)

BN_HIDDEN int launch_decode_g1(bn254_ctx* c, hipStream_t s, const uint8_t* d_pts, size_t n, uint32_t flags, int px, int inf_plane, int accumulate);
BN_HIDDEN int launch_decode_g2(bn254_ctx* c, hipStream_t s, const uint8_t* d_pts, size_t n, uint32_t flags, int accumulate);
BN_HIDDEN int launch_hash_rounds(bn254_ctx* c, hipStream_t s, const uint8_t* d_msgs, const uint64_t* d_off, size_t n, int px, int inf_plane,
                                 uint8_t* d_tries, int mark_finish = -1);
BN_HIDDEN int launch_final_exp_layout(bn254_ctx* c, hipStream_t s, size_t n, int use_hash, uint8_t* d_status, int fe);
enum BnVerifyPairs { BN_PAIRS_VERIFY = 0, BN_PAIRS_CHECK_PKS = 1 };
BN_HIDDEN int launch_verify_miller_fe(bn254_ctx* c, hipStream_t s, size_t n, int pairs, int use_hash, uint8_t* d_status, bool mark);
BN_HIDDEN int launch_miller_var_lane(bn254_ctx* c, hipStream_t s, size_t n);
BN_HIDDEN int launch_rand_tail_lane(bn254_ctx* c, hipStream_t s, size_t n_groups, size_t gbase);
BN_HIDDEN int launch_miller_verify_lane(bn254_ctx* c, hipStream_t s, size_t n, const uint32_t* map, const uint32_t* count);
BN_HIDDEN int launch_final_exp_lane(bn254_ctx* c, hipStream_t s, size_t n, size_t k, size_t item_stride, size_t pair_stride, int use_hash, uint8_t* gt_out,
                                    uint8_t* status_out, int raw_only, size_t base, const uint32_t* map, const uint32_t* count);
BN_HIDDEN int launch_encode_g1(bn254_ctx* c, hipStream_t s, size_t n, int px, int inf_plane, uint8_t* out, uint8_t* status_out);
```

### bn254_amd/csrc/bn254_keydedup.h

```cpp
#pragma once

namespace bn254 {

template <class Emit>
BN_DEV bool kd_walk_raw_lines(const G2Affine& q, Emit&& emit) {
  G2Proj t;
  LineCoef l;
  t.x = q.x; t.y = q.y; t.z = fp2_one();
  const Fp2 q_yneg = fp2_neg(q.y);
  bool degenerate = false;
  int idx = 0;
  auto line = [&]() {
    const Fp2 c2 = NR(290, l.c2);
    degenerate = fp2_is_zero(c2) || degenerate;
    emit(idx++, NS(292, l.c0), NS(293, l.c1), c2);
  };
#if defined(__HIPCC__)
#pragma clang loop unroll(disable)
#endif
  for (int d = 0; d < 64; ++d) {
    dbl_step(t, l); line();
    const int digit = C_ATE_NAF[d];
    if (digit != 0) { add_step(t, l, q.x, fp2_select(digit > 0, q.y, q_yneg)); line(); }
  }
  add_step(t, l, fp2_mul(fp2_conj(q.x), fp2_load_const(C_TW_FROB_X1)), fp2_mul(fp2_conj(q.y), fp2_load_const(C_TW_FROB_Y1))); line();
  add_step(t, l, fp2_mul(q.x, fp2_load_const(C_TW_FROB_X2)), q.y); line();
  return degenerate;
}
BN_DEV void kd_scale_line(const Fp2& c0, const Fp2& c1, const Fp2& c2, Fp2& r0, Fp2& r1) {
  const Fp2 inv = NS(291, fp2_inv(c2));
  const Fp2 a = fp2_mul(c0, inv), b = fp2_mul(c1, inv);
  BN_FOR_ROLES(k) { r0.c[k] = fp_canon(a.c[k]); r1.c[k] = fp_canon(b.c[k]); }
}

#if defined(__HIPCC__)
BN_DEV bool load_fp_be_checked(Fp& r, const uint8_t* p, uint32_t& any) {
  const uint32_t* w = (const uint32_t*)p;
  U256 t;
#pragma unroll
  for (int k = 0; k < 8; ++k) { t.w[7 - k] = __builtin_bswap32(w[k]); any |= w[k]; }
  bool ok = !u256_geq(t.w, C_Q);
  r = fp_from_u256(t);
  return ok;
}
BN_DEV uint8_t decode_g2_pair_role(G2Affine& q, const uint8_t* b, uint32_t flags) {
  const unsigned role = threadIdx.x & 1u;
  uint32_t any = 0;
  bool ok = load_fp_be_checked(q.x.c[0], b + 32 * role, any);
  ok = load_fp_be_checked(q.y.c[0], b + 64 + 32 * role, any) && ok;
  any |= (uint32_t)bn_partner_word((int32_t)any);
  ok = bn_pair_and(ok);
  q.inf = any == 0;
  uint8_t st = ST_OK;
  if (q.inf) st = (flags & FLAG_REJECT_IDENTITY) ? (uint8_t)ST_INVALID_GROUP_POINT : (uint8_t)ST_OK;
  else if (!ok) st = ST_NOT_MEMBER;
  const bool on_curve = g2_on_curve(q);
  if (st == ST_OK && !q.inf && !on_curve) st = ST_INVALID_GROUP_POINT;
  return st;
}
#endif

}
```

### bn254_amd/csrc/bn254_keydedup.hip

```cpp
#include <hip/hip_runtime.h>

#define BN_SPLIT_FP2 1
#define bn254 bn254_kd
#include "bn254_pairing.h"
#include "bn254_keydedup.h"
#include "bn254_lmachine.h"
#include "bn254_kdlines.h"

using namespace bn254;

#include "bn254_ws.h"

#define KD_WG 256
#define KERNEL_KD_PAIR __global__ __launch_bounds__(KD_WG) __attribute__((amdgpu_waves_per_eu(2, 2)))
#define KERNEL_KD __global__ __launch_bounds__(KD_WG)

__device__ __forceinline__ uint32_t kd_hash(const uint32_t* w, uint32_t hash_mask) {
  uint32_t h = 0x9E3779B9u;
#pragma unroll
  for (int k = 0; k < 32; ++k) {
    h ^= w[k];
    h *= 0x85EBCA6Bu;
    h ^= h >> 13;
  }
  h ^= h >> 16; h *= 0xC2B2AE35u; h ^= h >> 16;
  return h & hash_mask;
}
__device__ __forceinline__ bool kd_same_key(const uint32_t* pks, uint32_t other, const uint32_t* w) {
  const uint32_t* o = pks + (size_t)other * 32;
  bool eq = true;
#pragma unroll
  for (int k = 0; k < 32; ++k) eq = eq && o[k] == w[k];
  return eq;
}
KERNEL_KD void k_kd_insert(const uint8_t* pks8, size_t n, KeyDedup kd) {
  const size_t i = (size_t)blockIdx.x * KD_WG + threadIdx.x;
  if (i >= n) return;
  const uint32_t* pks = (const uint32_t*)pks8;
  uint32_t w[32];
#pragma unroll
  for (int k = 0; k < 32; ++k) w[k] = pks[i * 32 + k];
  const uint32_t h = kd_hash(w, kd.hash_mask);
  for (uint32_t probe = 0; probe < KD_MAX_PROBES; ++probe) {
    const uint32_t s = (h + probe) & kd.slot_mask;
    uint32_t cur = __atomic_load_n(&kd.table[s], __ATOMIC_RELAXED);
    if (cur == KD_EMPTY) {
      cur = atomicCAS(&kd.table[s], KD_EMPTY, (uint32_t)i);
      if (cur == KD_EMPTY) {
        const uint32_t id = atomicAdd(&kd.ctl[KD_CTL_D], 1u);
        kd.slot_id[s] = id;
        if (id < kd.max_keys) kd.rep[id] = (uint32_t)i;
        kd.slot_of[i] = s;
        return;
      }
    }
    if (kd_same_key(pks, cur, w)) { kd.slot_of[i] = s; return; }
  }
  kd.slot_of[i] = KD_EMPTY;
  atomicOr(&kd.ctl[KD_CTL_FLAGS], (uint32_t)KD_OVERFLOW);
}
KERNEL_KD void k_kd_resolve(size_t n, KeyDedup kd) {
  const size_t i = (size_t)blockIdx.x * KD_WG + threadIdx.x;
  if (i >= n) return;
  const uint32_t s = kd.slot_of[i];
  kd.key_idx[i] = s == KD_EMPTY ? 0u : kd.slot_id[s];
}
__device__ __forceinline__ bool kd_viable(const KeyDedup& kd, size_t n) {
  const uint32_t d = kd.ctl[KD_CTL_D];
  return d <= kd.max_keys && (size_t)d * kd.min_mult <= n && (kd.ctl[KD_CTL_FLAGS] & KD_OVERFLOW) == 0;
}

__device__ __forceinline__ void kd_store_own(int32_t* dst, const Fp2& x) {
#pragma unroll
  for (int k = 0; k < BN_LIMBS; ++k) dst[(threadIdx.x & 1u) * BN_LIMBS + k] = x.c[0].v[k];
}
__device__ __forceinline__ Fp2 kd_load_own(const int32_t* src) {
  Fp2 r;
#pragma unroll
  for (int k = 0; k < BN_LIMBS; ++k) r.c[0].v[k] = src[(threadIdx.x & 1u) * BN_LIMBS + k];
  return r;
}
#define KD_LM_PER_WAVE 3
#define KD_LM_LANES 18
#define KD_LM_ROLE_STRIDE (LS_KD_SLOTS * BN_LIMBS + 1)
#define KD_LM_KEY_STRIDE (2 * KD_LM_ROLE_STRIDE)
#define KD_LM_LDS_WORDS (KD_LM_PER_WAVE * KD_LM_KEY_STRIDE)
static_assert(KD_LM_PER_WAVE * KD_LM_LANES <= BN_WAVE, "keys per wave");
#define KERNEL_KD_LM __global__ __launch_bounds__(BN_WAVE) __attribute__((amdgpu_waves_per_eu(1, 1)))
#define KD_LM_FENCE() do { __builtin_amdgcn_fence(__ATOMIC_ACQ_REL, "wavefront"); __builtin_amdgcn_wave_barrier(); } while (0)

extern __shared__ int32_t kd_lds[];

struct KdLdsBox {
  typedef unsigned Ref;
  unsigned base;
  __device__ __forceinline__ Ref slot(uint32_t id) const { return base + id * BN_LIMBS; }
  __device__ __forceinline__ Fp2 get(Ref off) const {
    Fp2 r;
#pragma unroll
    for (int i = 0; i < BN_LIMBS; ++i) r.c[0].v[i] = kd_lds[off + i];
    return r;
  }
  __device__ __forceinline__ void put(Ref off, const Fp2& x) const {
#pragma unroll
    for (int i = 0; i < BN_LIMBS; ++i) kd_lds[off + i] = x.c[0].v[i];
  }
};
struct KdLmDev {
  KdLdsBox bx;
  LmEntry e[KD_LV_N];
  unsigned pair;
  bool writer, live, degenerate;
  int32_t* rows;
  int32_t* c2s;
  __device__ __forceinline__ void level(int lv) {
    const LmEntry& en = e[lv];
    {
      const Fp2 pr = lm_stage_product(en, bx, 0);
      KD_LM_FENCE();
      if (writer && (en.w[1] & 255u) != (uint32_t)LS_DUMMY) bx.put(lm_product_out(en, bx, 0), pr);
      KD_LM_FENCE();
    }
    const Fp2 li = lm_stage_linear(en, bx, 0, false, false);
    KD_LM_FENCE();
    if (writer && (en.w[4] & 255u) != (uint32_t)LS_DUMMY) bx.put(lm_linear_out(en, bx, 0), li);
    KD_LM_FENCE();
  }
  __device__ __forceinline__ void add_point(int qx, int qy) {
    const Fp2 x = bx.get(bx.slot((uint32_t)qx)), y = bx.get(bx.slot((uint32_t)qy));
    if (writer) { bx.put(bx.slot(LS_TQX), x); bx.put(bx.slot(LS_TQY), y); }
    KD_LM_FENCE();
  }
  __device__ __forceinline__ void line(int idx, int kind) {
    degenerate = fp2_is_zero(bx.get(bx.slot((uint32_t)kd_line_slot(kind, 2)))) || degenerate;
    const int c = pair < 3 ? (int)pair : 2;
    const Fp2 v = bx.get(bx.slot((uint32_t)kd_line_slot(kind, c)));
    if (live && pair < 3) kd_store_own(c == 2 ? c2s + (size_t)idx * 2 * BN_LIMBS : rows + (size_t)idx * BN_KEY_LINE_WORDS + (size_t)c * 2 * BN_LIMBS, v);
  }
};
KERNEL_KD_LM void k_kd_lines(const uint8_t* pks, size_t n, uint32_t flags, KeyDedup kd) {
  if (!kd_viable(kd, n)) return;
  const uint32_t d = kd.ctl[KD_CTL_D];
  if ((uint32_t)blockIdx.x * KD_LM_PER_WAVE >= d) return;
  __builtin_amdgcn_s_setprio(3);
  const unsigned l = threadIdx.x, v = l / KD_LM_LANES, role = l & 1u;
  KdLmDev m;
  m.writer = v < KD_LM_PER_WAVE;
  const unsigned vslot = m.writer ? v : KD_LM_PER_WAVE - 1;
  m.pair = (l % KD_LM_LANES) >> 1;
  uint32_t j = (uint32_t)blockIdx.x * KD_LM_PER_WAVE + vslot;
  m.live = m.writer && j < d;
  if (j >= d) j = d - 1;
  m.bx.base = vslot * KD_LM_KEY_STRIDE + role * KD_LM_ROLE_STRIDE;
  G2Affine q;
  const uint8_t st = decode_g2_pair_role(q, pks + 128 * (size_t)kd.rep[j], flags);
  const bool real = st == ST_OK && !q.inf;
  if (!real) { q.x = fp2_load_const(C_G2_GEN[0]); q.y = fp2_load_const(C_G2_GEN[1]); }
  if (m.live && m.pair == 0 && role == 0) { kd.st[j] = st; kd.inf[j] = q.inf; }
  if (m.writer) {
    m.bx.put(m.bx.slot(LS_ZERO), fp2_zero()); m.bx.put(m.bx.slot(LS_DUMMY), fp2_zero());
    kd_builder_init(m.bx, q);
  }
#pragma unroll
  for (int lv = 0; lv < KD_LV_N; ++lv) {
    const LmEntry* t = kd_level_table(lv);
#pragma unroll
    for (int k = 0; k < 5; ++k) m.e[lv].w[k] = t[m.pair].w[k];
  }
  m.rows = kd.lines + (size_t)j * BN_N_FIXED_LINES * BN_KEY_LINE_WORDS;
  m.c2s = kd.c2 + (size_t)j * BN_N_FIXED_LINES * 2 * BN_LIMBS;
  m.degenerate = false;
  KD_LM_FENCE();
  kd_builder_program(m);
  if (m.live && real && m.degenerate && m.pair == 0 && role == 0) atomicOr(&kd.ctl[KD_CTL_FLAGS], (uint32_t)KD_DEGENERATE);
}
KERNEL_KD_PAIR void k_kd_scale(size_t n, KeyDedup kd) {
  if (!kd_viable(kd, n)) return;
  const size_t p = ((size_t)blockIdx.x * KD_WG + threadIdx.x) >> 1;
  const uint32_t j = (uint32_t)(p / BN_N_FIXED_LINES), idx = (uint32_t)(p % BN_N_FIXED_LINES);
  if (j >= kd.ctl[KD_CTL_D]) return;
  int32_t* row = kd.lines + ((size_t)j * BN_N_FIXED_LINES + idx) * BN_KEY_LINE_WORDS;
  Fp2 r0, r1;
  kd_scale_line(kd_load_own(row), kd_load_own(row + 2 * BN_LIMBS), kd_load_own(kd.c2 + ((size_t)j * BN_N_FIXED_LINES + idx) * 2 * BN_LIMBS), r0, r1);
  kd_store_own(row, r0);
  kd_store_own(row + 2 * BN_LIMBS, r1);
}
KERNEL_KD void k_kd_decide(size_t n, KeyDedup kd, int force_generic) {
  if (threadIdx.x != 0) return;
  const bool keyed = !force_generic && kd_viable(kd, n) && (kd.ctl[KD_CTL_FLAGS] & KD_DEGENERATE) == 0;
  kd.ctl[KD_CTL_KEYED_N] = keyed ? (uint32_t)n : 0u;
  kd.ctl[KD_CTL_GENERIC_N] = keyed ? 0u : (uint32_t)n;
}

int bn254_kd_enqueue(const uint8_t* d_pks, size_t n, uint32_t flags, KeyDedup kd, int force_generic, hipStream_t s) {
  HIP_TRY(hipMemsetAsync(kd.table, 0xFF, ((size_t)kd.slot_mask + 1) * sizeof(uint32_t), s));
  HIP_TRY(hipMemsetAsync(kd.ctl, 0, KD_CTL_WORDS * sizeof(uint32_t), s));
  const unsigned g = (unsigned)((n + KD_WG - 1) / KD_WG);
  k_kd_insert<<<g, KD_WG, 0, s>>>(d_pks, n, kd);
  k_kd_resolve<<<g, KD_WG, 0, s>>>(n, kd);
  k_kd_lines<<<(unsigned)((kd.max_keys + KD_LM_PER_WAVE - 1) / KD_LM_PER_WAVE), BN_WAVE, KD_LM_LDS_WORDS * sizeof(int32_t), s>>>(d_pks, n, flags, kd);
  k_kd_scale<<<(unsigned)((2 * (size_t)kd.max_keys * BN_N_FIXED_LINES + KD_WG - 1) / KD_WG), KD_WG, 0, s>>>(n, kd);
  k_kd_decide<<<1, BN_WAVE, 0, s>>>(n, kd, force_generic);
  HIP_TRY(hipGetLastError());
  return 0;
}
```

### bn254_amd/csrc/bn254_ws.h

```cpp
#pragma once
#include <stddef.h>

#define BN_WAVE 64
#define BN_SPLIT_MAX_N ((size_t)98304)
#define TRIO_MAX_BATCH_DEFAULT 16384
#define NONET_WIDE_MAX_BATCH 1024
#define NONET_MAX_BATCH_DEFAULT 3072
#define LM_MAX_BATCH_DEFAULT 1536
enum BnMillerLayout { BN_ML_LANE_MACHINE = 0, BN_ML_WAVE_ROLES = 1, BN_ML_LANE_PAIRS = 2 };
enum BnFeLayout { BN_FE_NONET_WIDE = 0, BN_FE_NONET = 1, BN_FE_OCTET = 2, BN_FE_LANE_PAIRS = 3 };
struct BnRouteLimits { size_t lm_max, nonet_wide_max, nonet_max, small_max; };
struct BnRoute { int miller, fe; };
static inline BnRoute bn_route(const BnRouteLimits& L, size_t n) {
  BnRoute r = {BN_ML_LANE_PAIRS, BN_FE_LANE_PAIRS};
  if (n > L.small_max) return r;
  r.miller = n <= L.lm_max ? BN_ML_LANE_MACHINE : BN_ML_WAVE_ROLES;
  r.fe = n <= L.nonet_max ? (n <= L.nonet_wide_max ? BN_FE_NONET_WIDE : BN_FE_NONET) : BN_FE_OCTET;
  return r;
}
static inline int bn_route_table(const BnRouteLimits& L, size_t* max_n, BnRoute* route, int cap) {
  size_t b[4] = {L.lm_max, L.nonet_wide_max, L.nonet_max, L.small_max};
  for (int i = 0; i < 4; ++i) if (b[i] > L.small_max) b[i] = L.small_max;
  for (int i = 0; i < 4; ++i) for (int j = i + 1; j < 4; ++j) if (b[j] < b[i]) { size_t t = b[i]; b[i] = b[j]; b[j] = t; }
  int rows = 0;
  for (int i = 0; i < 4 && rows < cap - 1; ++i) {
    if (b[i] == 0 || (i && b[i] == b[i - 1])) continue;
    const BnRoute r = bn_route(L, b[i]);
    if (rows && route[rows - 1].miller == r.miller && route[rows - 1].fe == r.fe) { max_n[rows - 1] = b[i]; continue; }
    max_n[rows] = b[i]; route[rows] = r; ++rows;
  }
  max_n[rows] = (size_t)-1; route[rows] = bn_route(L, (size_t)-1); ++rows;
  return rows;
}
#ifndef BN_WS_ROUTE_ONLY
#define TRIO_WAVE_ROLES_DEFAULT 2
#define AGG_SUBSET_MIN_TUPLES_DEFAULT 4096
#define AGG_SUBSET_MAX_SIGNERS ((size_t)2048)
#define AGG_SUBSET_G1_TUPLES_PER_MSG ((size_t)64)
#define AGG_SUBSET_G1_MAX_BYTES ((size_t)8 << 30)
#define AGG_WIDE_MIN_TUPLES_DEFAULT 262144
#define AGG_WIDE_G1_TUPLES_PER_MSG ((size_t)512)
#define AGG_WIDE_G2_MAX_BYTES ((size_t)2 << 30)
#define PINNED_STAGING_DEFAULT 0
#define PINNED_STAGING_MIN_N ((size_t)8192)
#define RAND_MIN_BATCH_DEFAULT 131072
#define RAND_TWO_PER_LANE_MIN_N ((size_t)131072)
#define AGGD_WG_ELEMS 128
#define AGGD_WG_PAIRS 256
#define AGGD_TWO_PER_PAIR_MIN_M 131072
#define AGGD_SEG_NONE 0xFFFFFFFFu
#ifndef BN_WAVES_PER_EU
#define BN_WAVES_PER_EU 1
#endif
#define KERNEL __global__ __launch_bounds__(BN_WAVE) __attribute__((amdgpu_waves_per_eu(BN_WAVES_PER_EU, BN_WAVES_PER_EU)))
#define KERNEL_SMALL __global__ __launch_bounds__(BN_WAVE) __attribute__((amdgpu_waves_per_eu(2, 2)))

struct Ws {
  int32_t* planes;
  uint8_t* bytes;
  size_t stride;
  uint32_t* h_best;
  uint8_t* h_next;
  uint32_t* h_list;
  uint32_t* h_cnt;
  unsigned long long* clk;
};
#define BN_CLK_MAX_WG 4096
#define BN_CLK_BEGIN(ws)                                                                         \
  unsigned long long clk0_ = 0, wall0_ = 0;                                                      \
  if ((ws).clk && threadIdx.x == 0) { clk0_ = clock64(); wall0_ = wall_clock64(); }
#define BN_CLK_END(ws, slot)                                                                     \
  do {                                                                                           \
    if ((ws).clk && threadIdx.x == 0 && blockIdx.x < BN_CLK_MAX_WG) {                            \
      unsigned long long* p_ = (ws).clk + ((size_t)(slot) * BN_CLK_MAX_WG + blockIdx.x) * 2;    \
      p_[0] += clock64() - clk0_; p_[1] += wall_clock64() - wall0_;                              \
    }                                                                                            \
  } while (0)
#define HASH_NONE 0xFFFFFFFFu
#define HASH_DONE 0xFFFFFFFEu
#define HASH_DIRECT_WIDTH_DEFAULT 32
#define HASH_DIRECT_MAX_N ((size_t)4096)
#define HASH_MAX_ROUNDS 64
#define HASH_MAX_GRID_LANES ((size_t)1 << 24)
#ifndef HASH_TARGET_LANES
#define HASH_TARGET_LANES ((size_t)1 << 17)
#endif
enum { PL_P1X = 0, PL_P1Y, PL_QX0, PL_QX1, PL_QY0, PL_QY1, PL_P2X, PL_P2Y, PL_HASHX, PL_HASHY, PL_F0, N_PLANES = PL_F0 + 12 };
enum { BY_ST_DECODE = 0, BY_ST_HASH, BY_P1_INF, BY_Q_INF, BY_P2_INF, BY_A_INF, N_BYTE_PLANES };

__device__ __forceinline__ Fp ws_load_fp(const Ws& ws, int plane, size_t i) {
  Fp r;
#pragma unroll
  for (int k = 0; k < BN_LIMBS; ++k) r.v[k] = ws.planes[((size_t)plane * BN_LIMBS + k) * ws.stride + i];
  return r;
}
__device__ __forceinline__ void ws_store_fp(const Ws& ws, int plane, size_t i, const Fp& a) {
#pragma unroll
  for (int k = 0; k < BN_LIMBS; ++k) ws.planes[((size_t)plane * BN_LIMBS + k) * ws.stride + i] = a.v[k];
}
__device__ __forceinline__ uint8_t& ws_byte(const Ws& ws, int plane, size_t i) { return ws.bytes[(size_t)plane * ws.stride + i]; }

__device__ __forceinline__ void ws_store_g1(const Ws& ws, int px, int inf_plane, size_t i, const G1Affine& p) {
  ws_store_fp(ws, px, i, p.x); ws_store_fp(ws, px + 1, i, p.y); ws_byte(ws, inf_plane, i) = p.inf;
}
__device__ __forceinline__ void ws_load_g1(const Ws& ws, int px, int inf_plane, size_t i, G1Affine& p) {
  p.x = ws_load_fp(ws, px, i); p.y = ws_load_fp(ws, px + 1, i); p.inf = ws_byte(ws, inf_plane, i) != 0;
}

#define BN_POOL_HALF_WORDS 20
struct Pool { int32_t* planes; uint8_t* st; size_t stride; uint32_t g2; };
__device__ __forceinline__ size_t pool_word(const Pool& p, int e, size_t j) {
  return p.g2 ? j * (2 * BN_POOL_HALF_WORDS) + (size_t)((e & 1) * BN_POOL_HALF_WORDS + (e >> 1) * BN_LIMBS) : j * BN_POOL_HALF_WORDS + (size_t)(e * BN_LIMBS);
}
__device__ __forceinline__ Fp pool_load_fp(const Pool& p, int e, size_t j) {
  Fp r;
  const int32_t* w = p.planes + pool_word(p, e, j);
#pragma unroll
  for (int k = 0; k < BN_LIMBS; ++k) r.v[k] = w[k];
  return r;
}
__device__ __forceinline__ void pool_store_fp(const Pool& p, int e, size_t j, const Fp& a) {
  int32_t* w = p.planes + pool_word(p, e, j);
#pragma unroll
  for (int k = 0; k < BN_LIMBS; ++k) w[k] = a.v[k];
}
#define HIP_TRY(expr)                                      \
  do {                                                     \
    hipError_t e_ = (expr);                                \
    if (e_ != hipSuccess) return -(int)e_;                 \
  } while (0)

__attribute__((visibility("hidden"))) int bn254_pair_miller_verify(size_t n, Ws ws, const uint32_t* map, const uint32_t* count, hipStream_t s,
                                                                   int mode = 0);
__attribute__((visibility("hidden"))) int bn254_pair_miller_var(size_t n, Ws ws, hipStream_t s);
__attribute__((visibility("hidden"))) int bn254_pair_leaf_floor(size_t n, Ws ws, hipStream_t s, int mode);
__attribute__((visibility("hidden"))) int bn254_pair_fe_program(size_t n, Ws ws, const unsigned char* prog, hipStream_t s);
__attribute__((visibility("hidden"))) int bn254_pair_final_exp_product(size_t n, size_t k, Ws ws, uint8_t* gt_out, uint8_t* status_out, int raw_only,
                                                                       hipStream_t s);
__attribute__((visibility("hidden"))) int bn254_pair_final_exp(size_t n, Ws ws, int use_hash, uint8_t* status_out, const uint32_t* map,
                                                               const uint32_t* count, hipStream_t s, size_t base = 0);
__attribute__((visibility("hidden"))) int bn254_pair_miller_rand(size_t n, size_t n_groups, int items_per_pair, Ws ws, size_t gbase, hipStream_t s);
__attribute__((visibility("hidden"))) int bn254_pair_rand_tail(size_t n_groups, Ws ws, size_t gbase, hipStream_t s);
struct AggdSlots { const uint32_t* slot_agg; const uint64_t* incl; const uint64_t* lo; const uint64_t* hi; };
__attribute__((visibility("hidden"))) int bn254_pair_aggd_miller(size_t n_slots, Ws ws, AggdSlots sl, size_t gbase, size_t pbase, uint32_t* pseg, int last,
                                                                 hipStream_t s);
__attribute__((visibility("hidden"))) int bn254_pair_aggd_level(size_t n_elems, Ws ws, const uint32_t* seg, size_t ebase, size_t gbase, size_t pbase,
                                                                 uint32_t* pseg, int last, hipStream_t s);
__attribute__((visibility("hidden"))) int bn254_pair_aggd_tail(size_t n, Ws ws, size_t gbase, size_t obase, hipStream_t s);
__attribute__((visibility("hidden"))) int bn254_pair_aggregate(const uint32_t* tuple_msg, const uint64_t* tuple_off, const uint32_t* signer_idx, size_t n,
                                                               size_t n_signers, size_t n_msgs, Pool pk_pool, Pool sig_pool, Pool h_pool, Pool sub_pool,
                                                               size_t n_groups, Pool sub1_pool, size_t groups4, Ws ws, hipStream_t s,
                                                               const uint32_t* perm = nullptr, const Pool* wide2_pool = nullptr,
                                                               const Pool* wide1_pool = nullptr);
__attribute__((visibility("hidden"))) int bn254_pair_g2_mul_fixed(const uint8_t* d_scalars, size_t n, int reduce, Pool comb, uint8_t* d_out, uint8_t* d_status,
                                                                  hipStream_t s);
#define BN_G2_COMB_RECORDS (65 * 8 + 1)
__attribute__((visibility("hidden"))) int bn254_pair_g1_mul_fixed(const uint8_t* d_scalars, size_t n, int reduce, Pool comb, uint8_t* d_out, uint8_t* d_status,
                                                                  hipStream_t s);
#define BN_G1_COMB_RECORDS (65 * 8 + 3)
__attribute__((visibility("hidden"))) int bn254_pair_decode_g2(const uint8_t* pts, size_t n, uint32_t flags, Ws ws, int accumulate, hipStream_t s);
__attribute__((visibility("hidden"))) int bn254_pair_decompress_g2(const uint8_t* in, size_t n, Ws ws, hipStream_t s, int skip_subgroup_test = 0);

#define BN_KEY_LINE_WORDS (2 * 2 * BN_LIMBS)
struct KeyTable { const int32_t* lines; const uint8_t* st; const uint8_t* inf; uint32_t n_keys; };
__attribute__((visibility("hidden"))) int bn254_lm_miller_verify_keyed(size_t n, Ws ws, const uint32_t* key_idx, KeyTable kt, hipStream_t s);
__attribute__((visibility("hidden"))) int bn254_pair_miller_verify_keyed(size_t n, Ws ws, const uint32_t* key_idx, KeyTable kt, hipStream_t s, size_t base = 0,
                                                                         const uint32_t* map = nullptr, const uint32_t* count = nullptr);
#define AGGD_KEYED_W1_MAX_SLOTS 65536
__attribute__((visibility("hidden"))) int bn254_pair_aggd_keyed(size_t n_slots, int width, Ws ws, AggdSlots sl, const uint32_t* key_idx, KeyTable kt,
                                                                size_t gbase, size_t pbase, uint32_t* pseg, int last, hipStream_t s);
__attribute__((visibility("hidden"))) int bn254_pair_aggd_move(size_t n, Ws ws, size_t gbase, hipStream_t s);
#define AGG_RAND_MIN_PAIRS_DEFAULT 65536
#define AGG_RAND_GROUP_PAIRS_DEFAULT 1024
#define AGGR_SUM_WG 256
#define AGGR_PART_WORDS (3 * BN_LIMBS)
struct AggrScale { const uint32_t* pair_agg; const uint32_t* key_idx; const uint8_t* key_inf; const uint64_t* lo; uint32_t* nagg; uint32_t* ebkt;
                   uint64_t* cnt; uint64_t G; uint32_t n_keys; };
struct AggrSum { const uint32_t* perm; const uint64_t* tp; uint32_t* bkey; size_t m, gbase, cbase, tbase; uint32_t n_keys; };
__attribute__((visibility("hidden"))) int bn254_aggr_scale(size_t m, size_t n, Ws ws, size_t gbase, AggrScale a, const uint32_t* seed_be, int mode,
                                                           hipStream_t s);
__attribute__((visibility("hidden"))) int bn254_aggr_scatter(size_t n_entries, const uint32_t* ebkt, uint64_t* start, uint32_t* perm, uint32_t* eseg,
                                                             size_t n_b, uint32_t n_keys, const uint64_t* cnt, uint64_t* tp, hipStream_t s);
__attribute__((visibility("hidden"))) int bn254_aggr_glimits(size_t n_groups, uint32_t n_keys, size_t tbase, const uint64_t* cnt, const uint64_t* tp,
                                                             uint64_t* glo, uint64_t* ghi, Ws ws, size_t cbase, hipStream_t s);
__attribute__((visibility("hidden"))) int bn254_aggr_sum(size_t n_elems, int level0, Ws ws, AggrSum a, const uint32_t* seg_in, const int32_t* part_in,
                                                         uint32_t* pseg_out, int32_t* part_out, int last, hipStream_t s);
__attribute__((visibility("hidden"))) int bn254_aggr_collect(size_t n, Ws ws, size_t gbase, const uint64_t* lo, uint64_t G, const uint32_t* nagg,
                                                             const uint8_t* gst, uint8_t* status, uint8_t* queued, size_t n_groups, const uint64_t* glo,
                                                             const uint64_t* ghi, uint32_t* stats, hipStream_t s);
__attribute__((visibility("hidden"))) int bn254_pair_aggd_keyed_queued(size_t n_slots, int width, Ws ws, AggdSlots sl, const uint32_t* key_idx, KeyTable kt,
                                                                       size_t gbase, size_t pbase, uint32_t* pseg, int last, const uint8_t* queued,
                                                                       hipStream_t s);

#define BITMAP_TABLE_MAX_KEYS_DEFAULT 4096
struct BmKeysArg { const int32_t* xy; const uint8_t* st; const uint8_t* inf; const uint32_t* bad; uint32_t n_keys; };
__attribute__((visibility("hidden"))) int bn254_pair_bitmap_sum(const uint32_t* d_bits, size_t bm_words, size_t n, BmKeysArg keys, const int32_t* rec,
                                                                const uint8_t* rec_inf, Ws ws, hipStream_t s);

#define KEY_DEDUP_MAX_KEYS_DEFAULT 1024
#define KEY_DEDUP_MIN_MULT_DEFAULT 16
#define KEY_DEDUP_MAX_KEYS_LIMIT 16384
#define KD_MAX_PROBES 64u
#define KD_EMPTY 0xFFFFFFFFu
enum { KD_OVERFLOW = 1, KD_DEGENERATE = 2 };
enum { KD_CTL_D = 0, KD_CTL_FLAGS, KD_CTL_KEYED_N, KD_CTL_GENERIC_N, KD_CTL_WORDS = 4 };
struct KeyDedup {
  uint32_t* table;
  uint32_t* slot_id;
  uint32_t* slot_of;
  uint32_t* key_idx;
  uint32_t* rep;
  uint32_t* ctl;
  int32_t* lines;
  int32_t* c2;
  uint8_t* st;
  uint8_t* inf;
  uint32_t slot_mask, hash_mask, max_keys, min_mult;
};
__attribute__((visibility("hidden"))) int bn254_kd_enqueue(const uint8_t* d_pks, size_t n, uint32_t flags, KeyDedup kd, int force_generic, hipStream_t s);
#define KD_BYTES_PER_ITEM ((size_t)(2 * 4 + 2) * sizeof(uint32_t))
#define KD_BYTES_PER_KEY ((size_t)BN_N_FIXED_LINES * (BN_KEY_LINE_WORDS + 2 * BN_LIMBS) * sizeof(int32_t) + sizeof(uint32_t) + 2)

__attribute__((visibility("hidden"))) int bn254_trio_miller_verify(size_t n, Ws ws, hipStream_t s, int mode = 0);
__attribute__((visibility("hidden"))) int bn254_quad_miller_verify(size_t n, Ws ws, hipStream_t s, int mode = 0);
__attribute__((visibility("hidden"))) int bn254_w8_miller_verify(size_t n, Ws ws, hipStream_t s, int mode = 0);
__attribute__((visibility("hidden"))) bool bn254_trio_fits_device();
__attribute__((visibility("hidden"))) bool bn254_quad_fits_device(int eight_waves);
__attribute__((visibility("hidden"))) int bn254_trio_final_exp(size_t n, Ws ws, int use_hash, uint8_t* status_out, hipStream_t s);
__attribute__((visibility("hidden"))) bool bn254_lm_fits_device();
__attribute__((visibility("hidden"))) int bn254_lm_miller_verify(size_t n, Ws ws, hipStream_t s, int mode = 0);
__attribute__((visibility("hidden"))) int bn254_lm_g2_subgroup(size_t n, Ws ws, hipStream_t s, int fail_status = 4 );
__attribute__((visibility("hidden"))) bool bn254_nonet_fits_device();
__attribute__((visibility("hidden"))) int bn254_nonet_final_exp(size_t n, Ws ws, int use_hash, uint8_t* status_out, hipStream_t s, int wide = 0);
__attribute__((visibility("hidden"))) int bn254_nonet_final_exp_product(size_t n, size_t k, Ws ws, uint8_t* gt_out, uint8_t* status_out, hipStream_t s);
#endif
```

### bn254_amd/engine.py

```python
import ctypes

from . import _native

G1_BYTES, G2_BYTES, GT_BYTES, SCALAR_BYTES = 64, 128, 384, 32
FLAG_G2_SUBGROUP_CHECK = 1
FLAG_REJECT_IDENTITY = 2
FLAG_RAND64 = 0x100
FLAG_RAND_GLV = 0x200
OPT_SPLIT_MILLER = 1
OPT_HASH_MAX_TRIES = 2
OPT_RAND_ITEMS_PER_LANE = 3
OPT_PAIR_LANES = 4
OPT_RAND_MIN_BATCH = 5
OPT_TRIO_MAX_BATCH = 6
OPT_HASH_DIRECT_WIDTH = 7
OPT_TRIO_WAVE_ROLES = 8
OPT_AGG_SUBSET_MIN_TUPLES = 9
OPT_CLOCK_PROBE = 10
OPT_AGG_SORT_BY_MSG = 11
OPT_PINNED_STAGING = 12
OPT_NONET_MAX_BATCH = 13
OPT_LM_MAX_BATCH = 15
OPT_NONET_WIDE = 16
OPT_AGG_WIDE_MIN_TUPLES = 14
OPT_MAX_CHUNK = 17
OPT_ASSUME_FREE_MB = 18
OPT_G2_FIXED_BASE = 19
OPT_KEY_DEDUP = 20
OPT_KEY_DEDUP_MAX_KEYS = 21
OPT_KEY_DEDUP_MIN_MULT = 22
OPT_KEY_DEDUP_FORCE_GENERIC = 23
OPT_KEY_DEDUP_HASH_BITS = 24
OPT_AGGD_KEYED_ROUTE = 25
OPT_AGG_RAND_MIN_PAIRS = 26
OPT_AGG_RAND_GROUP_PAIRS = 27
OPT_BITMAP_TABLE_MAX_KEYS = 28
OPT_BITMAP_ROUTE = 29


class NativeError(RuntimeError):

    def __init__(self, fn, rc):
        what = "HIP error %d" % (-rc) if -10000 < rc < 0 else {-10001: "bad argument", -10002: "misaligned device pointer",
                                                                -10003: "no HIP device (bn254_amd has no CPU fallback)"}.get(rc, "error")
        super().__init__("%s failed: %s (rc=%d)" % (fn, what, rc))
        self.rc = rc


def _check(fn, rc):
    if rc != 0:
        raise NativeError(fn, rc)


def pack_messages(messages):
    n = len(messages)
    off = (ctypes.c_uint64 * (n + 1))()
    pos = 0
    for i, m in enumerate(messages):
        off[i] = pos
        pos += len(m)
    off[n] = pos
    return b"".join(bytes(m) for m in messages), off


class Engine:
    def __init__(self, device=0):
        self._lib = _native.load()
        h = ctypes.c_void_p()
        _check("bn254_ctx_create", self._lib.bn254_ctx_create(device, ctypes.byref(h)))
        self._h = h
        self.device = device

    def close(self):
        if getattr(self, "_h", None):
            self._lib.bn254_ctx_destroy(self._h)
            self._h = None

    def __del__(self):
        try:
            self.close()
        except Exception:
            pass

    def version(self):
        return self._lib.bn254_version().decode()

    def reserve(self, n):
        _check("bn254_ctx_reserve", self._lib.bn254_ctx_reserve(self._h, n))

    def reserve_host(self, n, msg_bytes):
        _check("bn254_ctx_reserve_host", self._lib.bn254_ctx_reserve_host(self._h, n, msg_bytes))

    def synchronize(self):
        _check("bn254_ctx_synchronize", self._lib.bn254_ctx_synchronize(self._h))

    def set_profiling(self, on):
        _check("bn254_ctx_set_profiling", self._lib.bn254_ctx_set_profiling(self._h, 1 if on else 0))

    def expect_msgs_len(self, msgs_len):
        _check("bn254_ctx_expect_msgs_len", self._lib.bn254_ctx_expect_msgs_len(self._h, int(msgs_len)))

    def set_option(self, option, value):
        _check("bn254_ctx_set_option", self._lib.bn254_ctx_set_option(self._h, option, value))

    def probe_issue_rate(self, op, waves_per_simd=2):
        rate, simds = ctypes.c_double(0), ctypes.c_int(0)
        _check("bn254_probe_issue_rate", self._lib.bn254_probe_issue_rate(self._h, op, waves_per_simd, ctypes.byref(rate), ctypes.byref(simds)))
        return rate.value, simds.value

    def route_table(self):
        m, a, b = (ctypes.c_uint64 * 8)(), (ctypes.c_int * 8)(), (ctypes.c_int * 8)()
        rows = self._lib.bn254_debug_route_table(self._h, m, a, b, 8)
        if rows < 0:
            _check("bn254_debug_route_table", rows)
        return [(int(m[i]), int(a[i]), int(b[i])) for i in range(rows)]

    def debug_key_dedup_last(self):
        o = (ctypes.c_uint32 * 5)()
        _check("bn254_debug_key_dedup_last", self._lib.bn254_debug_key_dedup_last(self._h, o))
        return dict(zip(("ran", "keys", "flags", "keyed_n", "generic_n"), (int(x) for x in o)))

    def debug_agg_rand_last(self):
        o = (ctypes.c_uint64 * 6)()
        _check("bn254_debug_agg_rand_last", self._lib.bn254_debug_agg_rand_last(self._h, o))
        return dict(zip(("ran", "groups", "table_pairs", "failed_groups", "rechecked", "single_groups"), (int(x) for x in o)))

    def debug_agg_rand_sums(self):
        name, f = "bn254_debug_agg_rand_sums", self._lib.bn254_debug_agg_rand_sums
        dims = (ctypes.c_uint64 * 2)()
        _check(name, f(self._h, dims, 0, 0, None, None, None, None, None, None))
        ng, ntp = int(dims[0]), int(dims[1])
        if ng == 0:
            return []
        nagg, verdict, s = (ctypes.c_uint32 * ng)(), ctypes.create_string_buffer(ng), ctypes.create_string_buffer(64 * ng)
        first, keys, pts = (ctypes.c_uint64 * (ng + 1))(), (ctypes.c_uint32 * max(ntp, 1))(), ctypes.create_string_buffer(64 * max(ntp, 1))
        _check(name, f(self._h, dims, ng, ntp, nagg, verdict, s, first, keys, pts))
        assert (int(dims[0]), int(dims[1])) == (ng, ntp)
        return [dict(nagg=int(nagg[g]), verdict=verdict.raw[g], s=s.raw[64 * g:64 * g + 64],
                     pairs=[(int(keys[t]), pts.raw[64 * t:64 * t + 64]) for t in range(int(first[g]), int(first[g + 1]))]) for g in range(ng)]

    def last_kernel_ms(self):
        ms = (ctypes.c_float * 4)()
        _check("bn254_ctx_last_kernel_ms", self._lib.bn254_ctx_last_kernel_ms(self._h, ms))
        return {"decode": ms[0], "hash_to_g1": ms[1], "miller_loop": ms[2], "final_exp": ms[3]}

    def probe_leaf_floor(self, n, mode=0):
        ms = ctypes.c_float()
        _check("bn254_probe_leaf_floor", self._lib.bn254_probe_leaf_floor(self._h, n, mode, ctypes.byref(ms)))
        return ms.value

    def probe_fe_program(self, n, steps):
        prog = bytes(b for st in steps for b in st)
        ms = ctypes.c_float()
        _check("bn254_probe_fe_program", self._lib.bn254_probe_fe_program(self._h, n, prog, len(steps), ctypes.byref(ms)))
        return ms.value

    def last_clocks(self):
        mhz = (ctypes.c_double * 3)()
        _check("bn254_ctx_last_clocks", self._lib.bn254_ctx_last_clocks(self._h, mhz))
        return {"miller_loop": mhz[0], "final_exp": mhz[1], "issue_probe": mhz[2]}

    def batch_verify(self, messages, sigs, pks, flags=0):
        n = len(messages)
        assert len(sigs) == n * G1_BYTES and len(pks) == n * G2_BYTES
        msgs, off = pack_messages(messages)
        status = ctypes.create_string_buffer(max(n, 1))
        _check("bn254_batch_verify", self._lib.bn254_batch_verify(self._h, msgs, off, bytes(sigs), bytes(pks), n, flags, status))
        return status.raw[:n]

    def batch_verify_compressed(self, messages, sigs33, pks65):
        n = len(messages)
        assert len(sigs33) == n * 33 and len(pks65) == n * 65
        msgs, off = pack_messages(messages)
        status = ctypes.create_string_buffer(max(n, 1))
        _check("bn254_batch_verify_compressed",
               self._lib.bn254_batch_verify_compressed(self._h, msgs, off, bytes(sigs33), bytes(pks65), n, status))
        return status.raw[:n]

    def batch_verify_randomized(self, messages, sigs, pks, seed32, flags=0):
        n = len(messages)
        assert len(sigs) == n * G1_BYTES and len(pks) == n * G2_BYTES and len(seed32) == 32
        msgs, off = pack_messages(messages)
        status = ctypes.create_string_buffer(max(n, 1))
        ng = (n + 63) // 64
        groups = ctypes.create_string_buffer(max(ng, 1))
        _check("bn254_batch_verify_randomized",
               self._lib.bn254_batch_verify_randomized(self._h, msgs, off, bytes(sigs), bytes(pks), n, flags, bytes(seed32), status, groups))
        return status.raw[:n], groups.raw[:ng]

    def batch_hash_to_g1(self, messages):
        n = len(messages)
        msgs, off = pack_messages(messages)
        pts = ctypes.create_string_buffer(max(n, 1) * G1_BYTES)
        status = ctypes.create_string_buffer(max(n, 1))
        tries = ctypes.create_string_buffer(max(n, 1))
        _check("bn254_batch_hash_to_g1", self._lib.bn254_batch_hash_to_g1(self._h, msgs, off, n, pts, status, tries))
        return pts.raw[:n * G1_BYTES], status.raw[:n], tries.raw[:n]

    def batch_pairing_check(self, g1s, g2s, n, k, flags=0):
        assert len(g1s) == n * k * G1_BYTES and len(g2s) == n * k * G2_BYTES
        status = ctypes.create_string_buffer(max(n, 1))
        _check("bn254_batch_pairing_check", self._lib.bn254_batch_pairing_check(self._h, bytes(g1s), bytes(g2s), n, k, flags, status))
        return status.raw[:n]

    def batch_pairing(self, g1s, g2s, n, k=1, flags=0):
        assert len(g1s) == n * k * G1_BYTES and len(g2s) == n * k * G2_BYTES
        gt = ctypes.create_string_buffer(max(n, 1) * GT_BYTES)
        status = ctypes.create_string_buffer(max(n, 1))
        _check("bn254_batch_pairing", self._lib.bn254_batch_pairing(self._h, bytes(g1s), bytes(g2s), n, k, flags, gt, status))
        return gt.raw[:n * GT_BYTES], status.raw[:n]

    def batch_check_public_keys(self, pk_g2, pk_g1, n, flags=0):
        status = ctypes.create_string_buffer(max(n, 1))
        _check("bn254_batch_check_public_keys", self._lib.bn254_batch_check_public_keys(self._h, bytes(pk_g2), bytes(pk_g1), n, flags, status))
        return status.raw[:n]

    def _binop(self, name, a, b, n, size):
        out = ctypes.create_string_buffer(max(n, 1) * size)
        status = ctypes.create_string_buffer(max(n, 1))
        _check(name, getattr(self._lib, name)(self._h, bytes(a), bytes(b), n, out, status))
        return out.raw[:n * size], status.raw[:n]

    def batch_g1_add(self, a, b, n):
        return self._binop("bn254_batch_g1_add", a, b, n, G1_BYTES)

    def batch_g2_add(self, a, b, n):
        return self._binop("bn254_batch_g2_add", a, b, n, G2_BYTES)

    def batch_g1_mul(self, points, scalars, n, reduce_scalar=False):
        out = ctypes.create_string_buffer(max(n, 1) * G1_BYTES)
        status = ctypes.create_string_buffer(max(n, 1))
        _check("bn254_batch_g1_mul", self._lib.bn254_batch_g1_mul(self._h, None if points is None else bytes(points), bytes(scalars), n,
                                                               int(reduce_scalar), out, status))
        return out.raw[:n * G1_BYTES], status.raw[:n]

    def batch_g2_mul(self, points, scalars, n, reduce_scalar=False):
        out = ctypes.create_string_buffer(max(n, 1) * G2_BYTES)
        status = ctypes.create_string_buffer(max(n, 1))
        _check("bn254_batch_g2_mul", self._lib.bn254_batch_g2_mul(self._h, None if points is None else bytes(points), bytes(scalars), n,
                                                               int(reduce_scalar), out, status))
        return out.raw[:n * G2_BYTES], status.raw[:n]

    def batch_sign(self, messages, sks):
        n = len(messages)
        msgs, off = pack_messages(messages)
        sigs = ctypes.create_string_buffer(max(n, 1) * G1_BYTES)
        status = ctypes.create_string_buffer(max(n, 1))
        _check("bn254_batch_sign", self._lib.bn254_batch_sign(self._h, msgs, off, bytes(sks), n, sigs, status))
        return sigs.raw[:n * G1_BYTES], status.raw[:n]

    def _sum(self, name, points, seg_off, size):
        n = len(seg_off) - 1
        off = (ctypes.c_uint64 * (n + 1))(*seg_off)
        out = ctypes.create_string_buffer(max(n, 1) * size)
        status = ctypes.create_string_buffer(max(n, 1))
        _check(name, getattr(self._lib, name)(self._h, bytes(points), off, n, out, status))
        return out.raw[:n * size], status.raw[:n]

    def batch_g1_sum(self, points, seg_off):
        return self._sum("bn254_batch_g1_sum", points, seg_off, G1_BYTES)

    def batch_g2_sum(self, points, seg_off):
        return self._sum("bn254_batch_g2_sum", points, seg_off, G2_BYTES)

    def batch_aggregate_verify(self, messages, pk_pool, sig_pool, tuple_msg, signer_lists, flags=0):
        n, n_msgs = len(tuple_msg), len(messages)
        n_signers = len(pk_pool) // G2_BYTES
        assert len(sig_pool) == n_msgs * n_signers * G1_BYTES and len(signer_lists) == n
        msgs, off = pack_messages(messages)
        t_off = (ctypes.c_uint64 * (n + 1))()
        flat = []
        for i, lst in enumerate(signer_lists):
            t_off[i] = len(flat)
            flat.extend(lst)
        t_off[n] = len(flat)
        idx = (ctypes.c_uint32 * max(len(flat), 1))(*flat)
        tm = (ctypes.c_uint32 * max(n, 1))(*tuple_msg)
        status = ctypes.create_string_buffer(max(n, 1))
        _check("bn254_batch_aggregate_verify",
               self._lib.bn254_batch_aggregate_verify(self._h, msgs, off, n_msgs, bytes(pk_pool), n_signers, bytes(sig_pool), tm, t_off, idx, n, flags, status))
        return status.raw[:n]

    def batch_aggregate_verify_distinct(self, messages, pks, agg_sigs, agg_sizes, flags=0):
        m, n = len(messages), len(agg_sizes)
        assert len(pks) == m * G2_BYTES and len(agg_sigs) == n * G1_BYTES and sum(agg_sizes) == m
        msgs, off = pack_messages(messages)
        a_off = (ctypes.c_uint64 * (n + 1))()
        pos = 0
        for i, k in enumerate(agg_sizes):
            a_off[i] = pos
            pos += int(k)
        a_off[n] = pos
        status = ctypes.create_string_buffer(max(n, 1))
        _check("bn254_batch_aggregate_verify_distinct",
               self._lib.bn254_batch_aggregate_verify_distinct(self._h, msgs, off, bytes(pks), m, bytes(agg_sigs), a_off, n, flags, status))
        return status.raw[:n]

    def batch_aggregate_verify_distinct_keyed(self, messages, key_idx, agg_sigs, agg_sizes, flags=0):
        m, n = len(messages), len(agg_sizes)
        assert len(key_idx) == m and len(agg_sigs) == n * G1_BYTES and sum(agg_sizes) == m
        msgs, off = pack_messages(messages)
        idx = (ctypes.c_uint32 * max(m, 1))(*key_idx)
        a_off = (ctypes.c_uint64 * (n + 1))()
        pos = 0
        for i, k in enumerate(agg_sizes):
            a_off[i] = pos
            pos += int(k)
        a_off[n] = pos
        status = ctypes.create_string_buffer(max(n, 1))
        _check("bn254_batch_aggregate_verify_distinct_keyed",
               self._lib.bn254_batch_aggregate_verify_distinct_keyed(self._h, msgs, off, idx, m, bytes(agg_sigs), a_off, n, flags, status))
        return status.raw[:n]

    def batch_aggregate_verify_distinct_keyed_randomized(self, messages, key_idx, agg_sigs, agg_sizes, seed32, flags=0):
        m, n = len(messages), len(agg_sizes)
        assert len(key_idx) == m and len(agg_sigs) == n * G1_BYTES and sum(agg_sizes) == m and len(seed32) == 32
        msgs, off = pack_messages(messages)
        idx = (ctypes.c_uint32 * max(m, 1))(*key_idx)
        a_off = (ctypes.c_uint64 * (n + 1))()
        pos = 0
        for i, k in enumerate(agg_sizes):
            a_off[i] = pos
            pos += int(k)
        a_off[n] = pos
        status = ctypes.create_string_buffer(max(n, 1))
        _check("bn254_batch_aggregate_verify_distinct_keyed_randomized",
               self._lib.bn254_batch_aggregate_verify_distinct_keyed_randomized(self._h, msgs, off, idx, m, bytes(agg_sigs), a_off, n, flags, bytes(seed32),
                                                                                status))
        return status.raw[:n]

    def register_pools(self, messages, pk_pool, sig_pool, expect_tuples, flags=0):
        n_msgs = len(messages)
        n_signers = len(pk_pool) // G2_BYTES
        assert len(sig_pool) == n_msgs * n_signers * G1_BYTES
        msgs, off = pack_messages(messages)
        _check("bn254_ctx_register_pools",
               self._lib.bn254_ctx_register_pools(self._h, msgs, off, n_msgs, bytes(pk_pool), n_signers, bytes(sig_pool), flags, expect_tuples))

    def batch_aggregate_verify_registered(self, tuple_msg, signer_lists):
        n = len(tuple_msg)
        assert len(signer_lists) == n
        t_off = (ctypes.c_uint64 * (n + 1))()
        flat = []
        for i, lst in enumerate(signer_lists):
            t_off[i] = len(flat)
            flat.extend(lst)
        t_off[n] = len(flat)
        idx = (ctypes.c_uint32 * max(len(flat), 1))(*flat)
        tm = (ctypes.c_uint32 * max(n, 1))(*tuple_msg)
        status = ctypes.create_string_buffer(max(n, 1))
        _check("bn254_batch_aggregate_verify_registered", self._lib.bn254_batch_aggregate_verify_registered(self._h, tm, t_off, idx, n, status))
        return status.raw[:n]

    def register_pools_device(self, d_msgs, d_msg_off, n_msgs, d_pk_pool, n_signers, d_sig_pool, expect_tuples, flags=0, stream=None):
        _check("bn254_ctx_register_pools_device",
               self._lib.bn254_ctx_register_pools_device(self._h, d_msgs, d_msg_off, n_msgs, d_pk_pool, n_signers, d_sig_pool, flags, expect_tuples, stream))

    def batch_aggregate_verify_registered_device(self, d_tuple_msg, d_tuple_off, d_signer_idx, n, d_status, stream=None):
        _check("bn254_batch_aggregate_verify_registered_device",
               self._lib.bn254_batch_aggregate_verify_registered_device(self._h, d_tuple_msg, d_tuple_off, d_signer_idx, n, d_status, stream))

    def batch_g1_decompress(self, data, n):
        out = ctypes.create_string_buffer(max(n, 1) * G1_BYTES)
        status = ctypes.create_string_buffer(max(n, 1))
        _check("bn254_batch_g1_decompress", self._lib.bn254_batch_g1_decompress(self._h, bytes(data), n, out, status))
        return out.raw[:n * G1_BYTES], status.raw[:n]

    def batch_g2_decompress(self, data, n):
        out = ctypes.create_string_buffer(max(n, 1) * G2_BYTES)
        status = ctypes.create_string_buffer(max(n, 1))
        _check("bn254_batch_g2_decompress", self._lib.bn254_batch_g2_decompress(self._h, bytes(data), n, out, status))
        return out.raw[:n * G2_BYTES], status.raw[:n]

    def debug_fp_op(self, op, a, b, n):
        out = ctypes.create_string_buffer(max(n, 1) * 32)
        status = ctypes.create_string_buffer(max(n, 1))
        _check("bn254_debug_fp_op", self._lib.bn254_debug_fp_op(self._h, op, bytes(a), None if b is None else bytes(b), n, out, status))
        return out.raw[:n * 32], status.raw[:n]

    def debug_fp12_op(self, op, a, b, n):
        out = ctypes.create_string_buffer(max(n, 1) * GT_BYTES)
        _check("bn254_debug_fp12_op", self._lib.bn254_debug_fp12_op(self._h, op, bytes(a), None if b is None else bytes(b), n, out))
        return out.raw[:n * GT_BYTES]

    def debug_final_exp_limbs(self, layout, limbs, n, want_gt=False):
        assert len(limbs) == n * 108
        arr = (ctypes.c_int32 * max(len(limbs), 1))(*limbs)
        gt = ctypes.create_string_buffer(max(n, 1) * GT_BYTES) if want_gt else None
        status = ctypes.create_string_buffer(max(n, 1))
        _check("bn254_debug_final_exp_limbs", self._lib.bn254_debug_final_exp_limbs(self._h, layout, arr, n, gt, status))
        return (gt.raw[:n * GT_BYTES] if want_gt else None), status.raw[:n]

    def debug_miller_loop(self, g1s, g2s, n):
        out = ctypes.create_string_buffer(max(n, 1) * GT_BYTES)
        _check("bn254_debug_miller_loop", self._lib.bn254_debug_miller_loop(self._h, bytes(g1s), bytes(g2s), n, out))
        return out.raw[:n * GT_BYTES]

    def debug_hash_candidate(self, h, n):
        out = ctypes.create_string_buffer(max(n, 1) * G1_BYTES)
        status = ctypes.create_string_buffer(max(n, 1))
        _check("bn254_debug_hash_candidate", self._lib.bn254_debug_hash_candidate(self._h, bytes(h), n, out, status))
        return out.raw[:n * G1_BYTES], status.raw[:n]

    def register_keys(self, pks, flags=0):
        n = len(pks) // G2_BYTES
        assert len(pks) == n * G2_BYTES
        st = ctypes.create_string_buffer(max(n, 1))
        _check("bn254_ctx_register_keys", self._lib.bn254_ctx_register_keys(self._h, bytes(pks), n, flags, st))
        self.n_registered_keys = n
        return st.raw[:n]

    def batch_verify_keyed(self, messages, sigs, key_idx, flags=0):
        n = len(messages)
        assert len(sigs) == n * G1_BYTES and len(key_idx) == n
        msgs, off = pack_messages(messages)
        idx = (ctypes.c_uint32 * max(n, 1))(*key_idx)
        status = ctypes.create_string_buffer(max(n, 1))
        _check("bn254_batch_verify_keyed", self._lib.bn254_batch_verify_keyed(self._h, msgs, off, bytes(sigs), idx, n, flags, status))
        return status.raw[:n]

    def batch_verify_keyed_bitmap(self, messages, sigs, bitmaps, bm_words, flags=0):
        n = len(messages)
        assert len(sigs) == n * G1_BYTES and len(bitmaps) == n * bm_words
# ... 254 lines not shown
```

### include/bn254_hip.h

```cpp
#ifndef BN254_HIP_H
#define BN254_HIP_H

#include <stddef.h>
#include <stdint.h>

#ifdef __cplusplus
extern "C" {
#endif

typedef struct bn254_ctx bn254_ctx;

#define BN254_FLAG_G2_SUBGROUP_CHECK 1u
#define BN254_FLAG_REJECT_IDENTITY 2u
#define BN254_FLAG_RAND64 0x100u
#define BN254_FLAG_RAND_GLV 0x200u

#define BN254_E_BAD_ARGUMENT (-10001)
#define BN254_E_MISALIGNED (-10002)
#define BN254_E_NO_DEVICE (-10003)
#define BN254_E_RCCL (-10004)
#define BN254_E_NO_MEMORY (-10005)

#define BN254_OK 0
#define BN254_ERR_HASH_TO_POINT 1
#define BN254_ERR_INDEX_OUT_OF_BOUNDS 2
#define BN254_ERR_INVALID_ENCODING 3
#define BN254_ERR_INVALID_GROUP_POINT 4
#define BN254_ERR_INVALID_LENGTH 5
#define BN254_ERR_NOT_MEMBER 6
#define BN254_ERR_TO_AFFINE_CONVERSION 7
#define BN254_ERR_POINT_IN_JACOBIAN 8
#define BN254_ERR_VERIFICATION_FAILED 9
#define BN254_ERR_SERIALIZATION 10
#define BN254_ERR_HEX_DECODE_FAILED 11

const char *bn254_version(void);

int bn254_ctx_create(int hip_device, bn254_ctx **out);
void bn254_ctx_destroy(bn254_ctx *ctx);
int bn254_ctx_reserve(bn254_ctx *ctx, size_t n_items);
int bn254_ctx_reserve_host(bn254_ctx *ctx, size_t n_items, size_t msg_bytes);
int bn254_ctx_synchronize(bn254_ctx *ctx);
int bn254_ctx_expect_msgs_len(bn254_ctx *ctx, uint64_t msgs_len);

int bn254_batch_verify(bn254_ctx *ctx, const uint8_t *msgs, const uint64_t *msg_off , const uint8_t *sigs ,
                       const uint8_t *pks , size_t n, uint32_t flags, uint8_t *status );
int bn254_batch_verify_device(bn254_ctx *ctx, const uint8_t *d_msgs, const uint64_t *d_msg_off, const uint8_t *d_sigs,
                              const uint8_t *d_pks, size_t n, uint32_t flags, uint8_t *d_status, void *stream);

int bn254_batch_verify_compressed(bn254_ctx *ctx, const uint8_t *msgs, const uint64_t *msg_off, const uint8_t *sigs33,
                                  const uint8_t *pks65, size_t n, uint8_t *status);
int bn254_batch_verify_compressed_device(bn254_ctx *ctx, const uint8_t *d_msgs, const uint64_t *d_msg_off,
                                         const uint8_t *d_sigs33, const uint8_t *d_pks65, size_t n, uint8_t *d_status,
                                         void *stream);

int bn254_ctx_register_keys(bn254_ctx *ctx, const uint8_t *pks , size_t n_keys, uint32_t flags, uint8_t *key_status );
int bn254_batch_verify_keyed(bn254_ctx *ctx, const uint8_t *msgs, const uint64_t *msg_off , const uint8_t *sigs ,
                             const uint32_t *key_idx , size_t n, uint32_t flags, uint8_t *status );
int bn254_batch_verify_keyed_device(bn254_ctx *ctx, const uint8_t *d_msgs, const uint64_t *d_msg_off, const uint8_t *d_sigs,
                                    const uint32_t *d_key_idx, size_t n, uint32_t flags, uint8_t *d_status, void *stream);

int bn254_batch_verify_keyed_randomized(bn254_ctx *ctx, const uint8_t *msgs, const uint64_t *msg_off, const uint8_t *sigs,
                                        const uint32_t *key_idx, size_t n, uint32_t flags, const uint8_t *seed32, uint8_t *status);
int bn254_batch_verify_keyed_randomized_device(bn254_ctx *ctx, const uint8_t *d_msgs, const uint64_t *d_msg_off, const uint8_t *d_sigs,
                                               const uint32_t *d_key_idx, size_t n, uint32_t flags, const uint8_t *seed32,
                                               uint8_t *d_status, void *stream);

int bn254_batch_verify_randomized(bn254_ctx *ctx, const uint8_t *msgs, const uint64_t *msg_off, const uint8_t *sigs,
                                  const uint8_t *pks, size_t n, uint32_t flags, const uint8_t *seed32, uint8_t *status,
                                  uint8_t *group_ok);
int bn254_batch_verify_randomized_device(bn254_ctx *ctx, const uint8_t *d_msgs, const uint64_t *d_msg_off,
                                         const uint8_t *d_sigs, const uint8_t *d_pks, size_t n, uint32_t flags,
                                         const uint8_t *seed32 , uint8_t *d_status, uint8_t *d_group_ok,
                                         void *stream);

int bn254_batch_hash_to_g1(bn254_ctx *ctx, const uint8_t *msgs, const uint64_t *msg_off, size_t n, uint8_t *points ,
                           uint8_t *status , uint8_t *tries );
int bn254_batch_hash_to_g1_device(bn254_ctx *ctx, const uint8_t *d_msgs, const uint64_t *d_msg_off, size_t n, uint8_t *d_points,
                                  uint8_t *d_status, uint8_t *d_tries, void *stream);

int bn254_batch_pairing_check(bn254_ctx *ctx, const uint8_t *g1 , const uint8_t *g2 , size_t n, size_t k,
                              uint32_t flags, uint8_t *status );
int bn254_batch_pairing(bn254_ctx *ctx, const uint8_t *g1, const uint8_t *g2, size_t n, size_t k, uint32_t flags,
                        uint8_t *gt , uint8_t *status );
int bn254_batch_pairing_device(bn254_ctx *ctx, const uint8_t *d_g1, const uint8_t *d_g2, size_t n, size_t k, uint32_t flags,
                               uint8_t *d_gt , uint8_t *d_status, void *stream);

int bn254_batch_check_public_keys(bn254_ctx *ctx, const uint8_t *pk_g2 , const uint8_t *pk_g1 , size_t n,
                                  uint32_t flags, uint8_t *status);

int bn254_batch_g1_add(bn254_ctx *ctx, const uint8_t *a , const uint8_t *b , size_t n, uint8_t *out, uint8_t *status);
int bn254_batch_g2_add(bn254_ctx *ctx, const uint8_t *a , const uint8_t *b , size_t n, uint8_t *out, uint8_t *status);
int bn254_batch_g1_mul(bn254_ctx *ctx, const uint8_t *p , const uint8_t *scalars , size_t n, int reduce_scalar,
                       uint8_t *out, uint8_t *status);
int bn254_batch_g2_mul(bn254_ctx *ctx, const uint8_t *p , const uint8_t *scalars , size_t n, int reduce_scalar,
                       uint8_t *out, uint8_t *status);
int bn254_batch_g1_mul_device(bn254_ctx *ctx, const uint8_t *d_p, const uint8_t *d_scalars, size_t n, int reduce_scalar,
                              uint8_t *d_out, uint8_t *d_status, void *stream);
int bn254_batch_g2_mul_device(bn254_ctx *ctx, const uint8_t *d_p, const uint8_t *d_scalars, size_t n, int reduce_scalar,
                              uint8_t *d_out, uint8_t *d_status, void *stream);
int bn254_batch_sign(bn254_ctx *ctx, const uint8_t *msgs, const uint64_t *msg_off, const uint8_t *sks , size_t n,
                     uint8_t *sigs , uint8_t *status);
int bn254_batch_sign_device(bn254_ctx *ctx, const uint8_t *d_msgs, const uint64_t *d_msg_off, const uint8_t *d_sks, size_t n,
                            uint8_t *d_sigs, uint8_t *d_status, void *stream);
int bn254_batch_g1_sum(bn254_ctx *ctx, const uint8_t *points, const uint64_t *seg_off , size_t n, uint8_t *out , uint8_t *status);
int bn254_batch_g2_sum(bn254_ctx *ctx, const uint8_t *points, const uint64_t *seg_off , size_t n, uint8_t *out , uint8_t *status);

int bn254_batch_aggregate_verify(bn254_ctx *ctx, const uint8_t *msgs, const uint64_t *msg_off , size_t n_msgs,
                                 const uint8_t *pk_pool , size_t n_signers, const uint8_t *sig_pool ,
                                 const uint32_t *tuple_msg , const uint64_t *tuple_off , const uint32_t *signer_idx, size_t n,
                                 uint32_t flags, uint8_t *status );
int bn254_batch_aggregate_verify_device(bn254_ctx *ctx, const uint8_t *d_msgs, const uint64_t *d_msg_off, size_t n_msgs, const uint8_t *d_pk_pool,
                                        size_t n_signers, const uint8_t *d_sig_pool, const uint32_t *d_tuple_msg, const uint64_t *d_tuple_off,
                                        const uint32_t *d_signer_idx, size_t n, uint32_t flags, uint8_t *d_status, void *stream);
int bn254_ctx_register_pools(bn254_ctx *ctx, const uint8_t *msgs, const uint64_t *msg_off , size_t n_msgs, const uint8_t *pk_pool ,
                             size_t n_signers, const uint8_t *sig_pool , uint32_t flags, size_t expect_tuples);
int bn254_ctx_register_pools_device(bn254_ctx *ctx, const uint8_t *d_msgs, const uint64_t *d_msg_off, size_t n_msgs, const uint8_t *d_pk_pool, size_t n_signers,
                                    const uint8_t *d_sig_pool, uint32_t flags, size_t expect_tuples, void *stream);
int bn254_batch_aggregate_verify_registered(bn254_ctx *ctx, const uint32_t *tuple_msg , const uint64_t *tuple_off , const uint32_t *signer_idx,
                                            size_t n, uint8_t *status );
int bn254_batch_aggregate_verify_registered_device(bn254_ctx *ctx, const uint32_t *d_tuple_msg, const uint64_t *d_tuple_off, const uint32_t *d_signer_idx,
                                                   size_t n, uint8_t *d_status, void *stream);

int bn254_batch_aggregate_verify_distinct(bn254_ctx *ctx, const uint8_t *msgs, const uint64_t *msg_off , const uint8_t *pks ,
                                          size_t m, const uint8_t *agg_sigs , const uint64_t *agg_off , size_t n, uint32_t flags,
                                          uint8_t *status );
int bn254_batch_aggregate_verify_distinct_device(bn254_ctx *ctx, const uint8_t *d_msgs, const uint64_t *d_msg_off, const uint8_t *d_pks, size_t m,
                                                 const uint8_t *d_agg_sigs, const uint64_t *d_agg_off, size_t n, uint32_t flags, uint8_t *d_status,
                                                 void *stream);

int bn254_batch_aggregate_verify_distinct_keyed(bn254_ctx *ctx, const uint8_t *msgs, const uint64_t *msg_off , const uint32_t *key_idx ,
                                                size_t m, const uint8_t *agg_sigs , const uint64_t *agg_off , size_t n,
                                                uint32_t flags, uint8_t *status );
int bn254_batch_aggregate_verify_distinct_keyed_device(bn254_ctx *ctx, const uint8_t *d_msgs, const uint64_t *d_msg_off, const uint32_t *d_key_idx,
                                                       size_t m, const uint8_t *d_agg_sigs, const uint64_t *d_agg_off, size_t n, uint32_t flags,
                                                       uint8_t *d_status, void *stream);

int bn254_batch_aggregate_verify_distinct_keyed_randomized(bn254_ctx *ctx, const uint8_t *msgs, const uint64_t *msg_off ,
                                                           const uint32_t *key_idx , size_t m, const uint8_t *agg_sigs ,
                                                           const uint64_t *agg_off , size_t n, uint32_t flags, const uint8_t *seed32,
                                                           uint8_t *status );
int bn254_batch_aggregate_verify_distinct_keyed_randomized_device(bn254_ctx *ctx, const uint8_t *d_msgs, const uint64_t *d_msg_off,
                                                                  const uint32_t *d_key_idx, size_t m, const uint8_t *d_agg_sigs,
                                                                  const uint64_t *d_agg_off, size_t n, uint32_t flags,
                                                                  const uint8_t *seed32 , uint8_t *d_status, void *stream);

int bn254_batch_verify_keyed_bitmap(bn254_ctx *ctx, const uint8_t *msgs, const uint64_t *msg_off , const uint8_t *sigs ,
                                    const uint32_t *signer_bits , size_t bm_words, size_t n, uint32_t flags, uint8_t *status );
int bn254_batch_verify_keyed_bitmap_device(bn254_ctx *ctx, const uint8_t *d_msgs, const uint64_t *d_msg_off, const uint8_t *d_sigs,
                                           const uint32_t *d_signer_bits, size_t bm_words, size_t n, uint32_t flags, uint8_t *d_status, void *stream);

int bn254_batch_g1_decompress(bn254_ctx *ctx, const uint8_t *in , size_t n, uint8_t *out , uint8_t *status);
int bn254_batch_g2_decompress(bn254_ctx *ctx, const uint8_t *in , size_t n, uint8_t *out , uint8_t *status);

int bn254_ctx_set_profiling(bn254_ctx *ctx, int enabled);
#define BN254_OPT_TRIO_MAX_BATCH 6
#define BN254_OPT_NONET_MAX_BATCH 13
#define BN254_OPT_LM_MAX_BATCH 15
#define BN254_OPT_RAND_MIN_BATCH 5
#define BN254_OPT_AGG_RAND_MIN_PAIRS 26
#define BN254_OPT_AGG_SUBSET_MIN_TUPLES 9
#define BN254_OPT_AGG_WIDE_MIN_TUPLES 14
#define BN254_OPT_PINNED_STAGING 12
#define BN254_OPT_MAX_CHUNK 17
#define BN254_OPT_KEY_DEDUP 20
#define BN254_OPT_KEY_DEDUP_MAX_KEYS 21
#define BN254_OPT_KEY_DEDUP_MIN_MULT 22
#define BN254_OPT_BITMAP_TABLE_MAX_KEYS 28
int bn254_ctx_set_option(bn254_ctx *ctx, int option, int value);
int bn254_ctx_last_kernel_ms(bn254_ctx *ctx, float ms[4]);
int bn254_ctx_last_clocks(bn254_ctx *ctx, double sclk_mhz[3]);

typedef struct bn254_mgpu bn254_mgpu;

int bn254_mgpu_create(const int *devices, int n_dev , bn254_mgpu **out);
void bn254_mgpu_destroy(bn254_mgpu *mg);
int bn254_mgpu_device_count(const bn254_mgpu *mg);
bn254_ctx *bn254_mgpu_ctx(bn254_mgpu *mg, int g);
size_t bn254_mgpu_shard_len(const bn254_mgpu *mg, size_t n);
int bn254_mgpu_shard_range(const bn254_mgpu *mg, size_t n, int g, size_t *lo, size_t *hi);
size_t bn254_mgpu_gathered_len(const bn254_mgpu *mg, size_t n);
int bn254_mgpu_reserve(bn254_mgpu *mg, size_t n_total, int init_collectives);
int bn254_mgpu_synchronize(bn254_mgpu *mg);
#define BN254_MGPU_OPT_GATHER 1
#define BN254_MGPU_OPT_TIMING 2
int bn254_mgpu_set_option(bn254_mgpu *mg, int option, int value);
int bn254_mgpu_last_timing(bn254_mgpu *mg, float *compute_ms , float *collective_ms );
const char *bn254_mgpu_last_error(const bn254_mgpu *mg);

int bn254_mgpu_batch_verify(bn254_mgpu *mg, const uint8_t *msgs, const uint64_t *msg_off , const uint8_t *sigs ,
                            const uint8_t *pks , size_t n, uint32_t flags, uint8_t *status );
int bn254_mgpu_batch_verify_device(bn254_mgpu *mg, const uint8_t *const *d_msgs, const uint64_t *const *d_msg_off,
                                   const uint8_t *const *d_sigs, const uint8_t *const *d_pks, size_t n , uint32_t flags,
                                   uint8_t *const *d_status_all , void *const *streams );
int bn254_mgpu_batch_verify_compressed(bn254_mgpu *mg, const uint8_t *msgs, const uint64_t *msg_off, const uint8_t *sigs33, const uint8_t *pks65,
                                       size_t n, uint8_t *status);
int bn254_mgpu_register_keys(bn254_mgpu *mg, const uint8_t *pks , size_t n_keys, uint32_t flags, uint8_t *key_status );
int bn254_mgpu_batch_verify_keyed(bn254_mgpu *mg, const uint8_t *msgs, const uint64_t *msg_off, const uint8_t *sigs, const uint32_t *key_idx, size_t n,
                                  uint32_t flags, uint8_t *status);
int bn254_mgpu_batch_aggregate_verify(bn254_mgpu *mg, const uint8_t *msgs, const uint64_t *msg_off, size_t n_msgs, const uint8_t *pk_pool,
                                      size_t n_signers, const uint8_t *sig_pool, const uint32_t *tuple_msg, const uint64_t *tuple_off,
                                      const uint32_t *signer_idx, size_t n, uint32_t flags, uint8_t *status);
int bn254_mgpu_batch_pairing(bn254_mgpu *mg, const uint8_t *g1 , const uint8_t *g2 , size_t n, size_t k,
                             uint32_t flags, uint8_t *gt , uint8_t *status , uint64_t *checksum );
int bn254_mgpu_batch_pairing_device(bn254_mgpu *mg, const uint8_t *const *d_g1, const uint8_t *const *d_g2, size_t n, size_t k,
                                    uint32_t flags, uint8_t *const *d_gt, uint8_t *const *d_status_all, uint64_t *const *d_checksum,
                                    void *const *streams);
int bn254_mgpu_batch_hash_to_g1(bn254_mgpu *mg, const uint8_t *msgs, const uint64_t *msg_off, size_t n, uint8_t *points ,
                                uint8_t *status , uint8_t *tries );

#ifndef BN254_NO_DEV_HOOKS
#define BN254_OPT_SPLIT_MILLER 1
#define BN254_OPT_PAIR_LANES 4
#define BN254_OPT_RAND_ITEMS_PER_LANE 3
#define BN254_OPT_TRIO_WAVE_ROLES 8
#define BN254_OPT_HASH_DIRECT_WIDTH 7
#define BN254_OPT_NONET_WIDE 16
#define BN254_OPT_AGG_SORT_BY_MSG 11
#define BN254_OPT_CLOCK_PROBE 10
#define BN254_OPT_HASH_MAX_TRIES 2
#define BN254_OPT_G2_FIXED_BASE 19
#define BN254_OPT_KEY_DEDUP_FORCE_GENERIC 23
#define BN254_OPT_KEY_DEDUP_HASH_BITS 24
#define BN254_OPT_AGGD_KEYED_ROUTE 25
#define BN254_OPT_AGG_RAND_GROUP_PAIRS 27
#define BN254_OPT_BITMAP_ROUTE 29
#define BN254_OPT_ASSUME_FREE_MB 18
int bn254_debug_route_table(bn254_ctx *ctx, uint64_t *max_n, int *miller, int *fe, int cap);
int bn254_debug_key_dedup_last(bn254_ctx *ctx, uint32_t out[5]);
int bn254_debug_agg_rand_last(bn254_ctx *ctx, uint64_t out[6]);
int bn254_debug_agg_rand_sums(bn254_ctx *ctx, uint64_t dims[2], size_t group_cap, size_t pair_cap, uint32_t *nagg, uint8_t *verdict,
                              uint8_t *s_g , uint64_t *first_pair , uint32_t *pair_key, uint8_t *pair_point );
int bn254_debug_fp_op(bn254_ctx *ctx, int op, const uint8_t *a, const uint8_t *b, size_t n, uint8_t *out, uint8_t *status);
int bn254_debug_fp12_op(bn254_ctx *ctx, int op, const uint8_t *a, const uint8_t *b, size_t n, uint8_t *out);
int bn254_debug_final_exp_limbs(bn254_ctx *ctx, int layout, const int32_t *limbs , size_t n, uint8_t *gt ,
                                uint8_t *status );
int bn254_debug_hash_candidate(bn254_ctx *ctx, const uint8_t *h , size_t n, uint8_t *out , uint8_t *status);
int bn254_debug_miller_loop(bn254_ctx *ctx, const uint8_t *g1, const uint8_t *g2, size_t n, uint8_t *f );

int bn254_probe_issue_rate(bn254_ctx *ctx, int op, int waves_per_simd, double *wave_inst_per_s, int *n_simd);
int bn254_probe_leaf_floor(bn254_ctx *ctx, size_t n, int mode, float *ms);
int bn254_probe_fe_program(bn254_ctx *ctx, size_t n, const uint8_t *prog, size_t n_steps, float *ms);
#endif

#ifdef __cplusplus
}
#endif
#endif
```

Measured before the change: 15.22 million.

## Add wide-first hash schedule with cooperative tail kernel and tree-batched key-line inversion

```diff
diff --git a/bn254_amd/_native.py b/bn254_amd/_native.py
--- a/bn254_amd/_native.py
+++ b/bn254_amd/_native.py
@@ -94,6 +94,8 @@
     L.bn254_ctx_set_option.argtypes = [vp, i32, i32]
     L.bn254_debug_route_table.argtypes = [vp, ctypes.POINTER(ctypes.c_uint64), ctypes.POINTER(i32), ctypes.POINTER(i32), i32]
     L.bn254_debug_key_dedup_last.argtypes = [vp, ctypes.POINTER(ctypes.c_uint32)]
+    if hasattr(L, "bn254_debug_key_tables"):
+        L.bn254_debug_key_tables.argtypes = [vp, i32, sz, sz, vp, vp, vp, vp]
     L.bn254_debug_agg_rand_last.argtypes = [vp, ctypes.POINTER(ctypes.c_uint64)]
     L.bn254_debug_agg_rand_sums.argtypes = [vp, ctypes.POINTER(ctypes.c_uint64), sz, sz, vp, vp, vp, vp, vp, vp]
     L.bn254_ctx_last_clocks.argtypes = [vp, ctypes.POINTER(ctypes.c_double)]
@@ -186,7 +188,7 @@
     "bn254_batch_g1_add", "bn254_batch_g2_add", "bn254_batch_g1_mul", "bn254_batch_g2_mul", "bn254_batch_g1_mul_device",
     "bn254_batch_g2_mul_device", "bn254_batch_sign", "bn254_batch_sign_device", "bn254_batch_g1_sum", "bn254_batch_g2_sum",
     "bn254_batch_aggregate_verify", "bn254_batch_aggregate_verify_device", "bn254_ctx_register_pools", "bn254_ctx_register_pools_device",
-    "bn254_batch_aggregate_verify_registered", "bn254_batch_aggregate_verify_registered_device", "bn254_batch_aggregate_verify_distinct", "bn254_batch_aggregate_verify_distinct_device", "bn254_batch_aggregate_verify_distinct_keyed", "bn254_batch_aggregate_verify_distinct_keyed_device", "bn254_batch_aggregate_verify_distinct_keyed_randomized", "bn254_batch_aggregate_verify_distinct_keyed_randomized_device", "bn254_batch_g1_decompress", "bn254_batch_g2_decompress", "bn254_debug_fp_op", "bn254_debug_fp12_op", "bn254_debug_final_exp_limbs", "bn254_debug_miller_loop", "bn254_debug_hash_candidate", "bn254_debug_route_table", "bn254_debug_key_dedup_last", "bn254_debug_agg_rand_last", "bn254_debug_agg_rand_sums", "bn254_probe_issue_rate", "bn254_probe_leaf_floor", "bn254_probe_fe_program", "bn254_ctx_set_profiling", "bn254_ctx_last_kernel_ms", "bn254_ctx_set_option", "bn254_ctx_last_clocks", "bn254_ctx_expect_msgs_len", "bn254_ctx_register_keys", "bn254_batch_verify_keyed", "bn254_batch_verify_keyed_device", "bn254_batch_verify_keyed_randomized", "bn254_batch_verify_keyed_randomized_device",
+    "bn254_batch_aggregate_verify_registered", "bn254_batch_aggregate_verify_registered_device", "bn254_batch_aggregate_verify_distinct", "bn254_batch_aggregate_verify_distinct_device", "bn254_batch_aggregate_verify_distinct_keyed", "bn254_batch_aggregate_verify_distinct_keyed_device", "bn254_batch_aggregate_verify_distinct_keyed_randomized", "bn254_batch_aggregate_verify_distinct_keyed_randomized_device", "bn254_batch_g1_decompress", "bn254_batch_g2_decompress", "bn254_debug_fp_op", "bn254_debug_fp12_op", "bn254_debug_final_exp_limbs", "bn254_debug_miller_loop", "bn254_debug_hash_candidate", "bn254_debug_route_table", "bn254_debug_key_dedup_last", "bn254_debug_key_tables", "bn254_debug_agg_rand_last", "bn254_debug_agg_rand_sums", "bn254_probe_issue_rate", "bn254_probe_leaf_floor", "bn254_probe_fe_program", "bn254_ctx_set_profiling", "bn254_ctx_last_kernel_ms", "bn254_ctx_set_option", "bn254_ctx_last_clocks", "bn254_ctx_expect_msgs_len", "bn254_ctx_register_keys", "bn254_batch_verify_keyed", "bn254_batch_verify_keyed_device", "bn254_batch_verify_keyed_randomized", "bn254_batch_verify_keyed_randomized_device",
     "bn254_batch_verify_keyed_bitmap", "bn254_batch_verify_keyed_bitmap_device",
     "bn254_mgpu_create", "bn254_mgpu_destroy", "bn254_mgpu_device_count", "bn254_mgpu_ctx", "bn254_mgpu_shard_len", "bn254_mgpu_shard_range",
     "bn254_mgpu_gathered_len", "bn254_mgpu_reserve", "bn254_mgpu_synchronize", "bn254_mgpu_set_option", "bn254_mgpu_last_timing",
diff --git a/bn254_amd/csrc/bn254_devhooks.hip b/bn254_amd/csrc/bn254_devhooks.hip
--- a/bn254_amd/csrc/bn254_devhooks.hip
+++ b/bn254_amd/csrc/bn254_devhooks.hip
@@ -148,6 +148,29 @@
   HIP_TRY(hipDeviceSynchronize());
   HIP_TRY(hipMemcpy(out + 1, c->kd_ctl, KD_CTL_WORDS * sizeof(uint32_t), hipMemcpyDeviceToHost));
   out[0] = 1;
+  return 0;
+}
+int bn254_debug_key_tables(bn254_ctx* c, int which, size_t first, size_t count, int32_t* lines, uint32_t* rep, uint8_t* st, uint8_t* inf) {
+  if (!c || !lines || (which != 0 && which != 1)) return BN254_E_BAD_ARGUMENT;
+  HIP_TRY(hipSetDevice(c->device));
+  HIP_TRY(hipDeviceSynchronize());
+  const size_t per_key = (size_t)BN_N_FIXED_LINES * BN_KEY_LINE_WORDS;
+  const int32_t* src;
+  const uint8_t *src_st, *src_inf;
+  if (which == 0) {
+    uint32_t ctl[KD_CTL_WORDS];
+    if (!c->kd_last_run || !c->kd_ctl || !c->kd_lines_last) return BN254_E_BAD_ARGUMENT;
+    HIP_TRY(hipMemcpy(ctl, c->kd_ctl, sizeof ctl, hipMemcpyDeviceToHost));
+    if (first + count > ctl[KD_CTL_D] || first + count > c->kd_keys_cap) return BN254_E_BAD_ARGUMENT;
+    src = c->kd_lines_last; src_st = c->kd_st_last; src_inf = c->kd_inf_last;
+    if (rep) HIP_TRY(hipMemcpy(rep, c->kd_rep_last + first, count * sizeof(uint32_t), hipMemcpyDeviceToHost));
+  } else {
+    if (!c->key_lines || first + count > c->n_keys) return BN254_E_BAD_ARGUMENT;
+    src = c->key_lines; src_st = c->key_st; src_inf = c->key_inf;
+  }
+  HIP_TRY(hipMemcpy(lines, src + first * per_key, count * per_key * sizeof(int32_t), hipMemcpyDeviceToHost));
+  if (st) HIP_TRY(hipMemcpy(st, src_st + first, count, hipMemcpyDeviceToHost));
+  if (inf) HIP_TRY(hipMemcpy(inf, src_inf + first, count, hipMemcpyDeviceToHost));
   return 0;
 }
 int bn254_debug_agg_rand_last(bn254_ctx* c, uint64_t out[6]) {
diff --git a/bn254_amd/csrc/bn254_hip.hip b/bn254_amd/csrc/bn254_hip.hip
--- a/bn254_amd/csrc/bn254_hip.hip
+++ b/bn254_amd/csrc/bn254_hip.hip
@@ -73,7 +73,7 @@
     if (hash_try_filter(hs, msg, len, ctr)) atomicMin(&ws.h_best[i], ctr);
   }
 }
-KERNEL_SMALL void k_hash_resolve(Ws ws, int round, uint32_t width, uint32_t max_ctr) {
+KERNEL_SMALL void k_hash_resolve(Ws ws, int round, uint32_t width, uint32_t max_ctr, uint32_t mark) {
   const uint32_t n_act = ws.h_cnt[round];
   if (n_act == 0) return;
   const uint32_t* list = round == 0 ? nullptr : ws.h_list + (size_t)(round & 1) * ws.stride;
@@ -87,7 +87,10 @@
       i = list ? list[slot] : (uint32_t)slot;
       if (ws.h_best[i] == HASH_NONE) {
         const uint32_t next = (uint32_t)ws.h_next[i] + width;
-        if (next < max_ctr) { ws.h_next[i] = (uint8_t)next; survivor = true; }
+        if (next < max_ctr) {
+          ws.h_next[i] = (uint8_t)next; survivor = true;
+          if (mark != HASH_NONE) ws.h_best[i] = mark;
+        }
       }
     }
     const uint64_t votes = __ballot(survivor);
@@ -100,7 +103,7 @@
 }
 #define HASH_RESOLVE_WG 1024
 #define HASH_RESOLVE_TILES_MIN ((size_t)1 << 20)
-__global__ void __launch_bounds__(HASH_RESOLVE_WG) k_hash_resolve_tiles(Ws ws, int round, uint32_t width, uint32_t max_ctr) {
+__global__ void __launch_bounds__(HASH_RESOLVE_WG) k_hash_resolve_tiles(Ws ws, int round, uint32_t width, uint32_t max_ctr, uint32_t mark) {
   const uint32_t n_act = ws.h_cnt[round];
   if (n_act == 0) return;
   const uint32_t* list = round == 0 ? nullptr : ws.h_list + (size_t)(round & 1) * ws.stride;
@@ -117,7 +120,10 @@
       i = list ? list[slot] : (uint32_t)slot;
       if (ws.h_best[i] == HASH_NONE) {
         const uint32_t next = (uint32_t)ws.h_next[i] + width;
-        if (next < max_ctr) { ws.h_next[i] = (uint8_t)next; survivor = true; }
+        if (next < max_ctr) {
+          ws.h_next[i] = (uint8_t)next; survivor = true;
+          if (mark != HASH_NONE) ws.h_best[i] = mark;
+        }
       }
     }
     const uint64_t votes = __ballot(survivor);
@@ -179,12 +185,10 @@
     }
   }
 }
-KERNEL_SMALL void k_hash_finish(const uint8_t* msgs, const uint64_t* off, uint64_t msgs_len, size_t n, Ws ws, uint32_t max_ctr, int px, int inf_plane,
-                                uint8_t* tries_out) {
-  size_t i = (size_t)blockIdx.x * BN_WAVE + threadIdx.x;
-  if (i >= n) return;
+__device__ __forceinline__ void hash_finish_item(const uint8_t* msgs, const uint64_t* off, uint64_t msgs_len, size_t i, const Ws& ws, uint32_t max_ctr, int px,
+                                                 int inf_plane, uint8_t* tries_out) {
   const uint32_t best = ws.h_best[i];
-  if (best == HASH_DONE) return;
+  if (best == HASH_DONE || best == HASH_TAIL) return;
   uint64_t lo, len;
   const bool span_ok = msg_span(off, i, msgs_len, lo, len);
   const uint8_t* msg = msgs + lo;
@@ -197,7 +201,63 @@
   ws_byte(ws, BY_ST_HASH, i) = ok ? (uint8_t)ST_OK : !span_ok ? (uint8_t)ST_INVALID_LENGTH : (uint8_t)ST_HASH_TO_POINT;
   if (tries_out) tries_out[i] = ok ? (uint8_t)(best + 1) : !span_ok ? (uint8_t)0 : (uint8_t)max_ctr;
 }
-
+KERNEL_SMALL void k_hash_finish(const uint8_t* msgs, const uint64_t* off, uint64_t msgs_len, size_t n, Ws ws, uint32_t max_ctr, int px, int inf_plane,
+                                uint8_t* tries_out) {
+  size_t i = (size_t)blockIdx.x * BN_WAVE + threadIdx.x;
+  if (i >= n) return;
+  hash_finish_item(msgs, off, msgs_len, i, ws, max_ctr, px, inf_plane, tries_out);
+}
+__device__ __noinline__ bool hash_try_msg(G1Affine& out, const uint8_t* msg, uint64_t len, uint32_t ctr) {
+  HashState hs;
+  hash_state_init(hs, msg, len);
+  return hash_try(out, hs, msg, len, ctr);
+}
+KERNEL_SMALL void k_hash_finish_tail(const uint8_t* msgs, const uint64_t* off, uint64_t msgs_len, size_t n, Ws ws, uint32_t max_ctr, int px, int inf_plane,
+                                     uint8_t* tries_out, unsigned nblk_finish, uint32_t chunk) {
+  if (blockIdx.x < nblk_finish) {
+    const size_t i = (size_t)blockIdx.x * BN_WAVE + threadIdx.x;
+    if (i < n) hash_finish_item(msgs, off, msgs_len, i, ws, max_ctr, px, inf_plane, tries_out);
+    return;
+  }
+  const uint32_t n_tail = ws.h_cnt[1];
+  const uint32_t* list = ws.h_list + ws.stride;
+  const uint32_t per_wave = BN_WAVE / chunk, sub = threadIdx.x / chunk, j = threadIdx.x % chunk;
+  const size_t span = (size_t)(gridDim.x - nblk_finish) * per_wave;
+  for (size_t base = (size_t)(blockIdx.x - nblk_finish) * per_wave; base < n_tail; base += span) {
+    const size_t slot = base + sub;
+    const bool live = slot < n_tail;
+    uint32_t i = 0, first = 0;
+    uint64_t lo = 0, len = 0;
+    bool span_ok = true;
+    if (live) { i = list[slot]; first = ws.h_next[i]; span_ok = msg_span(off, i, msgs_len, lo, len); }
+    const uint8_t* msg = msgs + lo;
+    bool open = live && span_ok;
+    for (uint32_t k = 0;; k += chunk) {
+      const uint32_t ctr = first + k + j;
+      bool ok = false;
+      G1Affine p;
+      if (open && ctr < max_ctr) ok = hash_try_msg(p, msg, len, ctr);
+      const uint64_t pass = __ballot(ok);
+      const uint32_t group = (uint32_t)(pass >> (threadIdx.x & ~(chunk - 1u))) & (uint32_t)((1ull << chunk) - 1u);
+      if (group != 0) {
+        if (ok && j == (uint32_t)__builtin_ctz(group)) {
+          ws_store_g1(ws, px, inf_plane, i, p);
+          ws_byte(ws, BY_ST_HASH, i) = (uint8_t)ST_OK;
+          if (tries_out) tries_out[i] = (uint8_t)(ctr + 1);
+        }
+        open = false;
+      }
+      if (__ballot(open && first + k + chunk < max_ctr) == 0) break;
+    }
+    if (live && j == 0 && (open || !span_ok)) {
+      G1Affine p;
+      g1_set_generator(p);
+      ws_store_g1(ws, px, inf_plane, i, p);
+      ws_byte(ws, BY_ST_HASH, i) = span_ok ? (uint8_t)ST_HASH_TO_POINT : (uint8_t)ST_INVALID_LENGTH;
+      if (tries_out) tries_out[i] = span_ok ? (uint8_t)max_ctr : (uint8_t)0;
+    }
+  }
+}
 KERNEL void k_miller_verify(size_t n, Ws ws, const uint32_t* map, const uint32_t* count) {
   size_t i = (size_t)blockIdx.x * BN_WAVE + threadIdx.x;
   if (i >= n) return;
@@ -387,6 +447,7 @@
     if (c->kd_buf) { HIP_TRY(hipFree(c->kd_buf)); c->kd_buf = nullptr; }
     c->kd_items_cap = c->kd_keys_cap = 0;
     c->kd_ctl = nullptr;
+    c->kd_lines_last = nullptr;
     if (hipMalloc((void**)&c->kd_buf, items_cap * KD_BYTES_PER_ITEM + keys_cap * KD_BYTES_PER_KEY + 256) != hipSuccess) {
       (void)hipGetLastError();
       c->kd_buf = nullptr;
@@ -410,6 +471,7 @@
   c->kd_ctl = kd.ctl;
   kd.st = take(c->kd_keys_cap);
   kd.inf = take(c->kd_keys_cap);
+  c->kd_lines_last = kd.lines; c->kd_rep_last = kd.rep; c->kd_st_last = kd.st; c->kd_inf_last = kd.inf;
   kd.slot_mask = (uint32_t)(slots - 1);
   kd.hash_mask = c->kd_hash_bits > 0 && c->kd_hash_bits < 32 ? (1u << c->kd_hash_bits) - 1 : 0xFFFFFFFFu;
   kd.max_keys = (uint32_t)keys;
@@ -500,6 +562,12 @@
   return 0;
 }
 
+static uint32_t hash_wide_width(size_t n) {
+  double survivors = (double)n * 0.5274 * 0.5274 * 0.5274 * 0.5274;
+  uint32_t w = 4;
+  for (; w < 8 && (double)n / BN_WAVE + survivors * HASH_TAIL_CHUNK_DEFAULT / BN_WAVE > (double)HASH_WIDE_WAVES; ++w) survivors *= 0.5274;
+  return w;
+}
 int launch_hash_rounds(bn254_ctx* c, hipStream_t s, const uint8_t* d_msgs, const uint64_t* d_off, size_t n, int px, int inf_plane,
                               uint8_t* d_tries, int mark_finish) {
   const uint32_t max_ctr = c->hash_max_tries ? (uint32_t)c->hash_max_tries : 255u;
@@ -512,6 +580,32 @@
       k_hash_round<<<grid_for(64 * (max_ctr - width)), BN_WAVE, 0, s>>>(d_msgs, d_off, msgs_len, c->ws, 1, max_ctr - width, max_ctr);
     if (mark_finish >= 0 && c->profiling) HIP_TRY(hipEventRecord(c->ev[mark_finish], s));
     k_hash_finish<<<grid_for(n), BN_WAVE, 0, s>>>(d_msgs, d_off, msgs_len, n, c->ws, max_ctr, px, inf_plane, d_tries);
+    HIP_TRY(hipGetLastError());
+    return 0;
+  }
+  if (n > HASH_DIRECT_MAX_N && (c->hash_schedule == 2 || (c->hash_schedule == 0 && n <= HASH_WIDE_MAX_N))) {
+    uint32_t w0 = c->hash_wide_width ? (uint32_t)c->hash_wide_width : hash_wide_width(n);
+    if (w0 > max_ctr) w0 = max_ctr;
+    size_t lanes = n * w0;
+    if (lanes > HASH_MAX_GRID_LANES) lanes = HASH_MAX_GRID_LANES;
+    k_hash_round<<<grid_for(lanes), BN_WAVE, 0, s>>>(d_msgs, d_off, msgs_len, c->ws, 0, w0, max_ctr);
+    if (n > HASH_RESOLVE_TILES_MIN) {
+      size_t tiles = (n + HASH_RESOLVE_WG - 1) / HASH_RESOLVE_WG;
+      if (tiles > 16384) tiles = 16384;
+      k_hash_resolve_tiles<<<(unsigned)tiles, HASH_RESOLVE_WG, 0, s>>>(c->ws, 0, w0, max_ctr, HASH_TAIL);
+    } else {
+      k_hash_resolve<<<grid_for(n), BN_WAVE, 0, s>>>(c->ws, 0, w0, max_ctr, HASH_TAIL);
+    }
+    double pf = 1.0;
+    for (uint32_t t = 0; t < w0 && pf > 1e-12; ++t) pf *= 0.5274;
+    double bound = (double)n * pf * 1.25 + 256.0;
+    if (bound > (double)n) bound = (double)n;
+    const uint32_t chunk = (uint32_t)c->hash_tail_chunk;
+    size_t tail_blocks = ((size_t)bound * chunk + BN_WAVE - 1) / BN_WAVE;
+    if (tail_blocks > HASH_TAIL_MAX_BLOCKS) tail_blocks = HASH_TAIL_MAX_BLOCKS;
+    if (mark_finish >= 0 && c->profiling) HIP_TRY(hipEventRecord(c->ev[mark_finish], s));
+    const unsigned nblk = grid_for(n);
+    k_hash_finish_tail<<<nblk + (unsigned)tail_blocks, BN_WAVE, 0, s>>>(d_msgs, d_off, msgs_len, n, c->ws, max_ctr, px, inf_plane, d_tries, nblk, chunk);
     HIP_TRY(hipGetLastError());
     return 0;
   }
@@ -530,9 +624,9 @@
     if ((size_t)bound > HASH_RESOLVE_TILES_MIN) {
       size_t tiles = ((size_t)bound + HASH_RESOLVE_WG - 1) / HASH_RESOLVE_WG;
       if (tiles > 16384) tiles = 16384;
-      k_hash_resolve_tiles<<<(unsigned)tiles, HASH_RESOLVE_WG, 0, s>>>(c->ws, round, width, max_ctr);
+      k_hash_resolve_tiles<<<(unsigned)tiles, HASH_RESOLVE_WG, 0, s>>>(c->ws, round, width, max_ctr, HASH_NONE);
     } else {
-      k_hash_resolve<<<grid_for((size_t)bound), BN_WAVE, 0, s>>>(c->ws, round, width, max_ctr);
+      k_hash_resolve<<<grid_for((size_t)bound), BN_WAVE, 0, s>>>(c->ws, round, width, max_ctr, HASH_NONE);
     }
     consumed += width;
     double pf = 1.0;
@@ -587,6 +681,7 @@
   c->agg_rand_group_pairs = AGG_RAND_GROUP_PAIRS_DEFAULT;
   c->trio_max_batch = TRIO_MAX_BATCH_DEFAULT;
   c->hash_direct_width = HASH_DIRECT_WIDTH_DEFAULT;
+  c->hash_tail_chunk = HASH_TAIL_CHUNK_DEFAULT;
   c->trio_wave_roles = TRIO_WAVE_ROLES_DEFAULT;
   c->agg_subset_min_tuples = AGG_SUBSET_MIN_TUPLES_DEFAULT;
   c->agg_sort_by_msg = 1;
@@ -714,6 +809,13 @@
     c->hash_direct_width = value;
     return 0;
   }
+  if (option == BN254_OPT_HASH_SCHEDULE) { if (value < 0 || value > 2) return BN254_E_BAD_ARGUMENT; c->hash_schedule = value; return 0; }
+  if (option == BN254_OPT_HASH_WIDE_WIDTH) { if (value < 0 || value > 64) return BN254_E_BAD_ARGUMENT; c->hash_wide_width = value; return 0; }
+  if (option == BN254_OPT_HASH_TAIL_CHUNK) {
+    if (value < 2 || value > 32 || (value & (value - 1))) return BN254_E_BAD_ARGUMENT;
+    c->hash_tail_chunk = value;
+    return 0;
+  }
   if (option == BN254_OPT_NONET_MAX_BATCH) {
     HIP_TRY(hipSetDevice(c->device));
     if (value < 0 || (value > 0 && !bn254_nonet_fits_device())) return BN254_E_BAD_ARGUMENT;
diff --git a/bn254_amd/csrc/bn254_host.h b/bn254_amd/csrc/bn254_host.h
--- a/bn254_amd/csrc/bn254_host.h
+++ b/bn254_amd/csrc/bn254_host.h
@@ -31,6 +31,9 @@
   int hash_max_tries;
   int trio_wave_roles;
   int hash_direct_width;
+  int hash_schedule;
+  int hash_wide_width;
+  int hash_tail_chunk;
   int trio_max_batch;
   int lm_max_batch;
   int nonet_wide;
@@ -75,6 +78,9 @@
   uint8_t* kd_buf;
   size_t kd_items_cap, kd_keys_cap;
   uint32_t* kd_ctl;
+  const int32_t* kd_lines_last;
+  const uint32_t* kd_rep_last;
+  const uint8_t *kd_st_last, *kd_inf_last;
   int kd_last_run;
   int aggd_keyed_route;
   int agg_rand_min_pairs;
diff --git a/bn254_amd/csrc/bn254_keydedup.h b/bn254_amd/csrc/bn254_keydedup.h
--- a/bn254_amd/csrc/bn254_keydedup.h
+++ b/bn254_amd/csrc/bn254_keydedup.h
@@ -33,6 +33,25 @@
   BN_FOR_ROLES(k) { r0.c[k] = fp_canon(a.c[k]); r1.c[k] = fp_canon(b.c[k]); }
 }
 
+#define KD_TREE_LEAVES 128
+#define KD_TREE_LEVELS 7
+#if !defined(__HIPCC__)
+static inline void kd_scale_tree(const Fp2* c0, const Fp2* c1, const Fp2* c2, Fp2* r0, Fp2* r1) {
+  static_assert(BN_N_FIXED_LINES <= KD_TREE_LEAVES && (1 << KD_TREE_LEVELS) == KD_TREE_LEAVES, "tree shape");
+  Fp2 prod[2 * KD_TREE_LEAVES], inv[2 * KD_TREE_LEAVES];
+  for (int p = 0; p < KD_TREE_LEAVES; ++p) prod[KD_TREE_LEAVES + p] = p < BN_N_FIXED_LINES ? fp2_reduce_weak(c2[p]) : fp2_one();
+  for (int w = KD_TREE_LEAVES / 2; w >= 1; w >>= 1)
+    for (int node = w; node < 2 * w; ++node) prod[node] = fp2_mul(prod[2 * node], prod[2 * node + 1]);
+  inv[1] = fp2_inv(prod[1]);
+  for (int w = 2; w <= KD_TREE_LEAVES; w <<= 1)
+    for (int node = w; node < 2 * w; ++node) inv[node] = fp2_mul(inv[node >> 1], prod[node ^ 1]);
+  for (int p = 0; p < BN_N_FIXED_LINES; ++p) {
+    const Fp2 a = fp2_mul(c0[p], inv[KD_TREE_LEAVES + p]), b = fp2_mul(c1[p], inv[KD_TREE_LEAVES + p]);
+    BN_FOR_ROLES(k) { r0[p].c[k] = fp_canon(a.c[k]); r1[p].c[k] = fp_canon(b.c[k]); }
+  }
+}
+#endif
+
 #if defined(__HIPCC__)
 BN_DEV bool load_fp_be_checked(Fp& r, const uint8_t* p, uint32_t& any) {
   const uint32_t* w = (const uint32_t*)p;
diff --git a/bn254_amd/csrc/bn254_keydedup.hip b/bn254_amd/csrc/bn254_keydedup.hip
--- a/bn254_amd/csrc/bn254_keydedup.hip
+++ b/bn254_amd/csrc/bn254_keydedup.hip
@@ -174,14 +174,47 @@
   kd_builder_program(m);
   if (m.live && real && m.degenerate && m.pair == 0 && role == 0) atomicOr(&kd.ctl[KD_CTL_FLAGS], (uint32_t)KD_DEGENERATE);
 }
+static_assert(BN_N_FIXED_LINES <= KD_TREE_LEAVES && 2 * KD_TREE_LEAVES == KD_WG, "one lane pair per leaf");
+#define KD_NODE_WORDS (2 * BN_LIMBS)
 KERNEL_KD_PAIR void k_kd_scale(size_t n, KeyDedup kd) {
   if (!kd_viable(kd, n)) return;
-  const size_t p = ((size_t)blockIdx.x * KD_WG + threadIdx.x) >> 1;
-  const uint32_t j = (uint32_t)(p / BN_N_FIXED_LINES), idx = (uint32_t)(p % BN_N_FIXED_LINES);
+  const uint32_t j = blockIdx.x;
   if (j >= kd.ctl[KD_CTL_D]) return;
-  int32_t* row = kd.lines + ((size_t)j * BN_N_FIXED_LINES + idx) * BN_KEY_LINE_WORDS;
+  __shared__ int32_t prod[2 * KD_TREE_LEAVES * KD_NODE_WORDS];
+  __shared__ int32_t inv[2 * KD_TREE_LEAVES * KD_NODE_WORDS];
+  const uint32_t p = threadIdx.x >> 1;
+  const bool line = p < BN_N_FIXED_LINES;
+  int32_t* row = kd.lines + ((size_t)j * BN_N_FIXED_LINES + (line ? p : 0u)) * BN_KEY_LINE_WORDS;
+  {
+    Fp2 leaf = fp2_one();
+    if (line) leaf = fp2_reduce_weak(kd_load_own(kd.c2 + ((size_t)j * BN_N_FIXED_LINES + p) * KD_NODE_WORDS));
+    kd_store_own(prod + (KD_TREE_LEAVES + p) * KD_NODE_WORDS, leaf);
+  }
+  __syncthreads();
+  for (uint32_t w = KD_TREE_LEAVES / 2; w >= 1; w >>= 1) {
+    if (p < w) {
+      const uint32_t node = w + p;
+      kd_store_own(prod + node * KD_NODE_WORDS, fp2_mul(kd_load_own(prod + 2 * node * KD_NODE_WORDS), kd_load_own(prod + (2 * node + 1) * KD_NODE_WORDS)));
+    }
+    __syncthreads();
+  }
+  if (threadIdx.x < BN_WAVE) {
+    const Fp2 r = fp2_inv(kd_load_own(prod + KD_NODE_WORDS));
+    if (p == 0) kd_store_own(inv + KD_NODE_WORDS, r);
+  }
+  __syncthreads();
+  for (uint32_t w = 2; w <= KD_TREE_LEAVES; w <<= 1) {
+    if (p < w) {
+      const uint32_t node = w + p;
+      kd_store_own(inv + node * KD_NODE_WORDS, fp2_mul(kd_load_own(inv + (node >> 1) * KD_NODE_WORDS), kd_load_own(prod + (node ^ 1u) * KD_NODE_WORDS)));
+    }
+    __syncthreads();
+  }
+  if (!line) return;
+  const Fp2 c2inv = kd_load_own(inv + (KD_TREE_LEAVES + p) * KD_NODE_WORDS);
+  const Fp2 a = fp2_mul(kd_load_own(row), c2inv), b = fp2_mul(kd_load_own(row + 2 * BN_LIMBS), c2inv);
   Fp2 r0, r1;
-  kd_scale_line(kd_load_own(row), kd_load_own(row + 2 * BN_LIMBS), kd_load_own(kd.c2 + ((size_t)j * BN_N_FIXED_LINES + idx) * 2 * BN_LIMBS), r0, r1);
+  BN_FOR_ROLES(k) { r0.c[k] = fp_canon(a.c[k]); r1.c[k] = fp_canon(b.c[k]); }
   kd_store_own(row, r0);
   kd_store_own(row + 2 * BN_LIMBS, r1);
 }
@@ -199,7 +232,7 @@
   k_kd_insert<<<g, KD_WG, 0, s>>>(d_pks, n, kd);
   k_kd_resolve<<<g, KD_WG, 0, s>>>(n, kd);
   k_kd_lines<<<(unsigned)((kd.max_keys + KD_LM_PER_WAVE - 1) / KD_LM_PER_WAVE), BN_WAVE, KD_LM_LDS_WORDS * sizeof(int32_t), s>>>(d_pks, n, flags, kd);
-  k_kd_scale<<<(unsigned)((2 * (size_t)kd.max_keys * BN_N_FIXED_LINES + KD_WG - 1) / KD_WG), KD_WG, 0, s>>>(n, kd);
+  k_kd_scale<<<kd.max_keys, KD_WG, 0, s>>>(n, kd);
   k_kd_decide<<<1, BN_WAVE, 0, s>>>(n, kd, force_generic);
   HIP_TRY(hipGetLastError());
   return 0;
diff --git a/bn254_amd/csrc/bn254_ws.h b/bn254_amd/csrc/bn254_ws.h
--- a/bn254_amd/csrc/bn254_ws.h
+++ b/bn254_amd/csrc/bn254_ws.h
@@ -78,6 +78,7 @@
   } while (0)
 #define HASH_NONE 0xFFFFFFFFu
 #define HASH_DONE 0xFFFFFFFEu
+#define HASH_TAIL 0xFFFFFFFDu
 #define HASH_DIRECT_WIDTH_DEFAULT 32
 #define HASH_DIRECT_MAX_N ((size_t)4096)
 #define HASH_MAX_ROUNDS 64
@@ -85,6 +86,12 @@
 #ifndef HASH_TARGET_LANES
 #define HASH_TARGET_LANES ((size_t)1 << 17)
 #endif
+#ifndef HASH_WIDE_MAX_N
+#define HASH_WIDE_MAX_N ((size_t)32768)
+#endif
+#define HASH_WIDE_WAVES 1024
+#define HASH_TAIL_CHUNK_DEFAULT 32
+#define HASH_TAIL_MAX_BLOCKS ((size_t)16384)
 enum { PL_P1X = 0, PL_P1Y, PL_QX0, PL_QX1, PL_QY0, PL_QY1, PL_P2X, PL_P2Y, PL_HASHX, PL_HASHY, PL_F0, N_PLANES = PL_F0 + 12 };
 enum { BY_ST_DECODE = 0, BY_ST_HASH, BY_P1_INF, BY_Q_INF, BY_P2_INF, BY_A_INF, N_BYTE_PLANES };
 
diff --git a/bn254_amd/engine.py b/bn254_amd/engine.py
--- a/bn254_amd/engine.py
+++ b/bn254_amd/engine.py
@@ -36,6 +36,9 @@
 OPT_AGG_RAND_GROUP_PAIRS = 27
 OPT_BITMAP_TABLE_MAX_KEYS = 28
 OPT_BITMAP_ROUTE = 29
+OPT_HASH_SCHEDULE = 30
+OPT_HASH_WIDE_WIDTH = 31
+OPT_HASH_TAIL_CHUNK = 32
 
 
 class NativeError(RuntimeError):
@@ -119,6 +122,13 @@
         o = (ctypes.c_uint32 * 5)()
         _check("bn254_debug_key_dedup_last", self._lib.bn254_debug_key_dedup_last(self._h, o))
         return dict(zip(("ran", "keys", "flags", "keyed_n", "generic_n"), (int(x) for x in o)))
+
+    def debug_key_tables(self, which, first, count):
+        words = (ctypes.c_int32 * (count * 87 * 36))()
+        rep = (ctypes.c_uint32 * max(count, 1))()
+        st, inf = ctypes.create_string_buffer(max(count, 1)), ctypes.create_string_buffer(max(count, 1))
+        _check("bn254_debug_key_tables", self._lib.bn254_debug_key_tables(self._h, which, first, count, words, rep, st, inf))
+        return list(words), (list(rep)[:count] if which == 0 else None), st.raw[:count], inf.raw[:count]
 
     def debug_agg_rand_last(self):
         o = (ctypes.c_uint64 * 6)()
diff --git a/include/bn254_hip.h b/include/bn254_hip.h
--- a/include/bn254_hip.h
+++ b/include/bn254_hip.h
@@ -215,6 +215,9 @@
 #define BN254_OPT_RAND_ITEMS_PER_LANE 3
 #define BN254_OPT_TRIO_WAVE_ROLES 8
 #define BN254_OPT_HASH_DIRECT_WIDTH 7
+#define BN254_OPT_HASH_SCHEDULE 30
+#define BN254_OPT_HASH_WIDE_WIDTH 31
+#define BN254_OPT_HASH_TAIL_CHUNK 32
 #define BN254_OPT_NONET_WIDE 16
 #define BN254_OPT_AGG_SORT_BY_MSG 11
 #define BN254_OPT_CLOCK_PROBE 10
@@ -228,6 +231,7 @@
 #define BN254_OPT_ASSUME_FREE_MB 18
 int bn254_debug_route_table(bn254_ctx *ctx, uint64_t *max_n, int *miller, int *fe, int cap);
 int bn254_debug_key_dedup_last(bn254_ctx *ctx, uint32_t out[5]);
+int bn254_debug_key_tables(bn254_ctx *ctx, int which, size_t first, size_t count, int32_t *lines, uint32_t *rep, uint8_t *st, uint8_t *inf);
 int bn254_debug_agg_rand_last(bn254_ctx *ctx, uint64_t out[6]);
 int bn254_debug_agg_rand_sums(bn254_ctx *ctx, uint64_t dims[2], size_t group_cap, size_t pair_cap, uint32_t *nagg, uint8_t *verdict,
                               uint8_t *s_g , uint64_t *first_pair , uint32_t *pair_key, uint8_t *pair_point );
```

New measurement: 15.41 million (median of 6 runs). 1.01x the previous value.
